# pennucci/PulsePortraiture

Hardware: AMD Instinct MI355X
Metric: subint_fits_per_sec (higher is better)
Workload: dtype f64

## Files before the change

pulseportraiture_amd/csrc/pp_common.h:

```cpp
#pragma once
#include <hip/hip_runtime.h>
#include <stdint.h>
#include <type_traits>

namespace pp {

#define PP_DCONST 4149.377593360996
#define PP_TWO_PI 6.283185307179586476925286766559
#define PP_LN10 2.302585092994045684017991454684

typedef double2 cplx;

__device__ __forceinline__ cplx cmul(cplx a, cplx b) {
    return make_double2(fma(a.x, b.x, -a.y * b.y), fma(a.x, b.y, a.y * b.x));
}
__device__ __forceinline__ cplx cmulc(cplx a, cplx b) {
    return make_double2(fma(a.x, b.x, a.y * b.y), fma(a.y, b.x, -a.x * b.y));
}
__device__ __forceinline__ cplx cadd(cplx a, cplx b) { return make_double2(a.x + b.x, a.y + b.y); }
__device__ __forceinline__ cplx csub(cplx a, cplx b) { return make_double2(a.x - b.x, a.y - b.y); }
__device__ __forceinline__ cplx cmul_mi(cplx a) { return make_double2(a.y, -a.x); }
__device__ __forceinline__ double cnorm(cplx a) { return fma(a.x, a.x, a.y * a.y); }

template <typename T>
__device__ __forceinline__ const T* as_global(const T* p) {
    typedef const T __attribute__((address_space(1)))* gp_t;
    return (const T*)(gp_t)(uintptr_t)p;
}

template <typename T>
__device__ __forceinline__ T load_uniform(const T* p) {
    typedef const T __attribute__((address_space(4)))* cp_t;
    return *(cp_t)(uintptr_t)p;
}

__device__ __forceinline__ double rn_pin(double r) { asm volatile("" : "+v"(r)); return r; }
__device__ __forceinline__ double mul_rn(double a, double b) { return rn_pin(a * b); }
__device__ __forceinline__ double add_rn(double a, double b) { return rn_pin(a + b); }
__device__ __forceinline__ double sub_rn(double a, double b) { return rn_pin(a - b); }

__device__ __forceinline__ double recip_ge1(double x) {
    double y = __builtin_amdgcn_rcp(x);
    y = fma(fma(-x, y, 1.0), y, y);
    y = fma(fma(-x, y, 1.0), y, y);
    return (x < 1e300) ? y : 0.0;
}

template <bool SC>
__device__ __forceinline__ double kconst(double v) {
    if (SC) asm volatile("" : "+s"(v));
    return v;
}
template <bool SC = false, bool ISGN = false>
__device__ __forceinline__ void sincos_turns(double t, double* sn, double* cs) {
    const double q = rint(4.0 * t);
    const double y = fma(-0.25, q, t);
    const double u = y * y;
    double ps = kconst<SC>(0x1.aaec32af93359p-4);
    ps = fma(ps, u, kconst<SC>(-0x1.6fadb9f155744p-1));
    ps = fma(ps, u, kconst<SC>(0x1.e8f434d018d63p+1));
    ps = fma(ps, u, kconst<SC>(-0x1.e3074fde8871fp+3));
    ps = fma(ps, u, kconst<SC>(0x1.50783487ee782p+5));
    ps = fma(ps, u, kconst<SC>(-0x1.32d2cce62bd86p+6));
    ps = fma(ps, u, kconst<SC>(0x1.466bc6775aae2p+6));
    ps = fma(ps, u, kconst<SC>(-0x1.4abbce625be53p+5));
    ps = fma(ps, u, kconst<SC>(0x1.921fb54442d18p+2));
    const double s0 = ps * y;
    double pc = kconst<SC>(0x1.20c62c2f2d7f5p-2);
    pc = fma(pc, u, kconst<SC>(-0x1.b6e24f44b128fp+0));
    pc = fma(pc, u, kconst<SC>(0x1.f9d38a3763cc3p+2));
    pc = fma(pc, u, kconst<SC>(-0x1.a6d1f2a204a8cp+4));
    pc = fma(pc, u, kconst<SC>(0x1.e1f506891babbp+5));
    pc = fma(pc, u, kconst<SC>(-0x1.55d3c7e3cbffap+6));
    pc = fma(pc, u, kconst<SC>(0x1.03c1f081b5ac4p+6));
    pc = fma(pc, u, kconst<SC>(-0x1.3bd3cc9be45dep+4));
    const double c0 = fma(pc, u, 1.0);
    const int qi = (int)q;
    const bool odd = qi & 1;
    const double so = odd ? c0 : s0, co = odd ? s0 : c0;
    if (ISGN) {
        const unsigned uq = (unsigned)qi;
        *sn = __hiloint2double((int)((unsigned)__double2hiint(so) + ((uq >> 1) << 31)), __double2loint(so));
        *cs = __hiloint2double((int)((unsigned)__double2hiint(co) + (((uq + 1u) >> 1) << 31)), __double2loint(co));
        return;
    }
    *sn = (qi & 2) ? -so : so;
    *cs = ((qi + 1) & 2) ? -co : co;
}

template <bool SC = false, bool ISGN = false>
__device__ __forceinline__ cplx unit_phasor(double k, double phi) {
    double pfrac = phi - rint(phi);
    double prod = k * pfrac;
    double err = fma(k, pfrac, -prod);
    double r = (prod - rint(prod)) + err;
    double s, c;
    sincos_turns<SC, ISGN>(r, &s, &c);
    return make_double2(c, s);
}

template <int W>
__device__ __forceinline__ double group_sum(double v) {
#pragma unroll
    for (int o = W / 2; o > 0; o >>= 1) v += __shfl_xor(v, o, 64);
    return v;
}
template <int W>
__device__ __forceinline__ double group_max(double v) {
#pragma unroll
    for (int o = W / 2; o > 0; o >>= 1) v = fmax(v, __shfl_xor(v, o, 64));
    return v;
}

__device__ __forceinline__ int wave_reduce16_index(int lane) { return (lane >> 2) & 15; }
template <int NS>
__device__ __forceinline__ double wave_reduce16(const double (&s)[NS], int lane) {
    double t8[8], t4[4], t2[2];
    const bool b5 = lane & 32, b4 = lane & 16, b3 = lane & 8, b2 = lane & 4;
#pragma unroll
    for (int j = 0; j < 8; ++j) {
        const double hi = (j + 8 < NS) ? s[j + 8] : 0.0;
        const double keep = b5 ? hi : s[j], send = b5 ? s[j] : hi;
        t8[j] = keep + __shfl_xor(send, 32, 64);
    }
#pragma unroll
    for (int j = 0; j < 4; ++j) {
        const double keep = b4 ? t8[j + 4] : t8[j], send = b4 ? t8[j] : t8[j + 4];
        t4[j] = keep + __shfl_xor(send, 16, 64);
    }
#pragma unroll
    for (int j = 0; j < 2; ++j) {
        const double keep = b3 ? t4[j + 2] : t4[j], send = b3 ? t4[j] : t4[j + 2];
        t2[j] = keep + __shfl_xor(send, 8, 64);
    }
    const double keep = b2 ? t2[1] : t2[0], send = b2 ? t2[0] : t2[1];
    double v = keep + __shfl_xor(send, 4, 64);
    v += __shfl_xor(v, 2, 64);
    v += __shfl_xor(v, 1, 64);
    return v;
}

template <int X>
__device__ __forceinline__ double quad_xor(double v) {
    static_assert(X == 1 || X == 2, "inside a quad");
    constexpr int ctrl = X == 1 ? 0xB1 : 0x4E;
    int lo = __double2loint(v), hi = __double2hiint(v);
    lo = __builtin_amdgcn_mov_dpp(lo, ctrl, 0xF, 0xF, false);
    hi = __builtin_amdgcn_mov_dpp(hi, ctrl, 0xF, 0xF, false);
    return __hiloint2double(hi, lo);
}
template <int NS, bool LEAN = false>
__device__ __forceinline__ double wave_reduce_lds(const double (&s)[NS], int lane, double* buf) {
    static_assert(NS <= 16, "one value per lane quad");
    const unsigned l = (unsigned)lane & 63u;
    const int wpos = LEAN ? (int)(l + (l >> 4)) : (lane >> 4) * 17 + (lane & 15);
#pragma unroll
    for (int q = 0; q < NS; ++q) buf[q * 68 + wpos] = s[q];
    const int q = min(lane >> 2, NS - 1), part = lane & 3;
    const double* src = LEAN ? buf + 17u * (4u * min(l >> 2, (unsigned)(NS - 1)) + (l & 3u)) : buf + q * 68 + part * 17;
    double v = 0.0;
#pragma unroll
    for (int t = 0; t < 16; ++t) v += src[t];
    if (LEAN) {
        v += quad_xor<1>(v);
        v += quad_xor<2>(v);
    } else {
        v += __shfl_xor(v, 1, 64);
        v += __shfl_xor(v, 2, 64);
    }
    return v;
}
#define PP_WRED_DOUBLES(NS) ((NS) * 68)

template <int NV>
__device__ inline void block_sum(double (&v)[NV], double* scratch) {
    const int lane = threadIdx.x & 63, wid = threadIdx.x >> 6, nw = blockDim.x >> 6;
#pragma unroll
    for (int i = 0; i < NV; ++i) v[i] = group_sum<64>(v[i]);
    __syncthreads();
    if (lane == 0) {
#pragma unroll
        for (int i = 0; i < NV; ++i) scratch[wid * NV + i] = v[i];
    }
    __syncthreads();
#pragma unroll
    for (int i = 0; i < NV; ++i) {
        double s = 0.0;
        for (int w = 0; w < nw; ++w) s += scratch[w * NV + i];
        v[i] = s;
    }
}

template <int NV, int C0>
__device__ __forceinline__ void wave_totals_to(const double (&v)[NV], int lane, double* dst) {
    constexpr int n = (NV - C0) < 16 ? (NV - C0) : 16;
    double part[n];
#pragma unroll
    for (int j = 0; j < n; ++j) part[j] = v[C0 + j];
    const double tot = wave_reduce16<n>(part, lane);
    if ((lane & 3) == 0 && (lane >> 2) < n) dst[C0 + (lane >> 2)] = tot;
    if constexpr (C0 + 16 < NV) wave_totals_to<NV, C0 + 16>(v, lane, dst);
}
#define PP_BSUM_DOUBLES(NW, NVMAX) (2 * (NW) * ((NVMAX) + 1))
template <int NV, int NVMAX>
__device__ __forceinline__ void block_sum_t(double (&v)[NV], double* scratch, int& flip, double* mx = nullptr) {
    static_assert(NV <= NVMAX, "scratch sized for NVMAX values");
    const int lane = threadIdx.x & 63, wid = threadIdx.x >> 6, nw = blockDim.x >> 6;
    double* buf = scratch + flip * nw * (NVMAX + 1);
    flip ^= 1;
    wave_totals_to<NV, 0>(v, lane, buf + wid * (NV + 1));
    if (mx) {
        const double m = group_max<64>(*mx);
        if (lane == 0) buf[wid * (NV + 1) + NV] = m;
    }
    __syncthreads();
#pragma unroll
    for (int i = 0; i < NV; ++i) {
        double s = 0.0;
        for (int w = 0; w < nw; ++w) s += buf[w * (NV + 1) + i];
        v[i] = s;
    }
    if (mx) {
        double m = buf[NV];
        for (int w = 1; w < nw; ++w) m = fmax(m, buf[w * (NV + 1) + NV]);
        *mx = m;
    }
}

struct SubState {
    double x[5];
    double xe[5];
    double f;
    double g[5];
    double H[25];
    double f0, g0[5], H0[25];
    double radius;
    double pred_red;
    int hits_boundary;
    int iter, nfev, status, done, cur;
    int npass;
    double xl[5], fl, gl[5], Hl[25];
    int fresh;
    int recentred;
    int nmodel;
    int model;
    double xprev[5];
    double geo[4];
};

#define PP_NACC 21
constexpr int PP_CHUNK_CHANNELS = 256;
#define PP_NCS 9
#define PP_TJ 10
#define PP_TSTRIDE (PP_TJ + 2)
#define PP_TAY_PAIR_STRIDE 2
__device__ __forceinline__ size_t tay_idx(size_t row, int q) { return row * PP_TSTRIDE + (size_t)q; }

}
```

pulseportraiture_amd/csrc/pp_extra.h:

```cpp
#pragma once
#include "pp_kernels.h"

namespace pp {

__device__ __forceinline__ void philox4x32_10(uint32_t (&c)[4], uint32_t k0, uint32_t k1) {
#pragma unroll
    for (int r = 0; r < 10; ++r) {
        const uint32_t hi0 = __umulhi(0xD2511F53u, c[0]), lo0 = 0xD2511F53u * c[0];
        const uint32_t hi1 = __umulhi(0xCD9E8D57u, c[2]), lo1 = 0xCD9E8D57u * c[2];
        const uint32_t n0 = hi1 ^ c[1] ^ k0, n2 = hi0 ^ c[3] ^ k1;
        c[0] = n0; c[1] = lo1; c[2] = n2; c[3] = lo0;
        k0 += 0x9E3779B9u; k1 += 0xBB67AE85u;
    }
}

__device__ __forceinline__ void normal_pair(uint64_t seed, int64_t sub, int chan, int pair, double& z0, double& z1) {
    uint32_t c[4] = {(uint32_t)pair, (uint32_t)chan, (uint32_t)((uint64_t)sub & 0xffffffffu),
                     (uint32_t)((uint64_t)sub >> 32)};
    philox4x32_10(c, (uint32_t)(seed & 0xffffffffu), (uint32_t)(seed >> 32));
    const uint64_t a = ((uint64_t)c[0] << 32) | c[1], b = ((uint64_t)c[2] << 32) | c[3];
    const double u1 = ((double)(a >> 11) + 0.5) * (1.0 / 9007199254740992.0);
    const double u2 = ((double)(b >> 11) + 0.5) * (1.0 / 9007199254740992.0);
    const double r = sqrt(-2.0 * log(u1));
    double s, co;
// ... 621 lines not shown
    const double* par;
    const double* w;
    const cplx* twB;
    cplx* acc;
    double* totw;
    const int* off;
    const int2* pairs;
    int npol, nchan, nchan_model;
};

__device__ __forceinline__ void align_add_totw(const AlignListArgs& a, int m) {
    double t = a.totw[m];
    for (int q = a.off[m]; q < a.off[m + 1]; ++q) t += a.w[(size_t)a.pairs[q].x * a.nchan + a.pairs[q].y];
    a.totw[m] = t;
}

template <int M, typename Tio>
__global__ __launch_bounds__(FftPlan<M>::T) void k_align_add(AlignListArgs a) {
    constexpr int T = FftPlan<M>::T;
    __shared__ cplx lds[FftPlan<M>::LDS_ELEMS];
    __shared__ cplx zin[M];
    const int tid = threadIdx.x;
    const int ipol = blockIdx.x / a.nchan_model, m = blockIdx.x % a.nchan_model;
    const int q0 = a.off[m], q1 = a.off[m + 1];
    if (q0 == q1) return;
    cplx* arow = a.acc + ((size_t)ipol * a.nchan_model + m) * M;
    for (int k = tid; k < M; k += T) zin[k] = arow[k];
    for (int q = q0; q < q1; ++q) {
        const int i = a.pairs[q].x, n = a.pairs[q].y;
        const double w = a.w[(size_t)i * a.nchan + n];
        const double phin = align_phase(a.par[i * 3], a.par[i * 3 + 1], a.par[i * 3 + 2],
                                        a.freqs[(size_t)i * a.freqs_stride + n], a.P[i]);
        align_add_row<M, Tio>(lds, zin, reinterpret_cast<const Tio*>(a.src) + (((size_t)i * a.npol + ipol) * a.nchan + n) * (2 * M),
                              a.twB, w, phin, tid);
        __syncthreads();
    }
    for (int k = tid; k < M; k += T) arow[k] = zin[k];
    if (ipol == 0 && tid == 0) align_add_totw(a, m);
}

struct ChanChi2Args {
    const void* src;
    const cplx* const* mft; const double* const* mdc; const int* slot;
    const double* freqs; long long freqs_stride;
    const double* P;
    const double* par;
    const double* nuref;
    const double* scales;
    const double* errs;
    const cplx* twB;
    double* out;
    int nsub, nchan;
};

template <int M, typename Tio>
__global__ __launch_bounds__(FftPlan<M>::T) void k_chan_chi2(ChanChi2Args a) {
    constexpr int T = FftPlan<M>::T;
    __shared__ cplx lds[FftPlan<M>::LDS_ELEMS];
    __shared__ double scratch[(T / 64) + 1];
    const int tid = threadIdx.x;
    const long long nrows = (long long)a.nsub * a.nchan;
    for (long long row = blockIdx.x; row < nrows; row += gridDim.x) {
        const int i = (int)(row / a.nchan), n = (int)(row % a.nchan);
        const double nu = a.freqs[(size_t)i * a.freqs_stride + n], P = a.P[i];
        const double* pr = a.par + (size_t)i * 5;
        const double nuDM = a.nuref[i * 3], nuGM = a.nuref[i * 3 + 1], nutau = a.nuref[i * 3 + 2];
        const double a2 = 1.0 / (nu * nu);
        const double iDM = (nuDM == INFINITY) ? 0.0 : 1.0 / (nuDM * nuDM);
        const double iGM = (nuGM == INFINITY) ? 0.0 : 1.0 / (nuGM * nuGM * nuGM * nuGM);
        const double phin = pr[0] + PP_DCONST * pr[1] * (a2 - iDM) / P +
                            PP_DCONST * PP_DCONST * pr[2] * (a2 * a2 - iGM) / P;
        const double taun = (pr[3] != 0.0) ? pr[3] * pow(nu / nutau, pr[4]) : 0.0;
        const int sl = a.slot ? a.slot[i] : 0;
        const cplx* mrow = as_global(a.mft[sl]) + (size_t)n * M;
        const double m0 = as_global(a.mdc[sl])[n];
        const double sc = a.scales[(size_t)i * a.nchan + n], sg = a.errs[(size_t)i * a.nchan + n];
        fft_row<M, Tio>(lds, reinterpret_cast<const Tio*>(a.src) + (size_t)row * (2 * M), a.twB, tid);
        const cplx z0 = lds[0];
        double sum = 0.0;
        for (int k = tid; k <= M; k += T) {
            double wgt = 2.0;
            cplx d, m;
            if (k == 0) { d = make_double2(z0.x + z0.y, 0.0); m = make_double2(m0, 0.0); wgt = 1.0; }
            else {
                d = (k == M) ? make_double2(z0.x - z0.y, 0.0) : rfft_harmonic<M>(lds, a.twB, k);
                d = cmul(d, unit_phasor((double)k, phin));
                m = mrow[k - 1];
                if (taun != 0.0) {
                    const double x = PP_TWO_PI * (double)k * taun, den = 1.0 / (1.0 + x * x);
                    m = cmul(m, make_double2(den, -x * den));
                }
            }
            cplx r = make_double2(d.x - sc * m.x, d.y - sc * m.y);
            if (k == M) { r.y = 0.0; wgt = 1.0; }
            sum = fma(wgt, cnorm(r), sum);
        }
        sum = group_sum<64>(sum);
        if ((tid & 63) == 0) scratch[tid >> 6] = sum;
        __syncthreads();
        if (tid == 0) {
            double tot = 0.0;
            for (int wv = 0; wv < T / 64; ++wv) tot += scratch[wv];
            a.out[row] = tot / (2.0 * M) / (sg * sg) / (double)(2 * M - 2);
        }
        __syncthreads();
    }
}

struct FpsArgs {
    const cplx* spec;
    const double* noise;
    double* out7;
    double lo, hi;
    int Ns, M, nprof;
    int finish;
    const cplx* specm;
    int mstride;
};

__device__ __forceinline__ void fps_sums(const cplx* X, int M, double phi, int tid, int nt, double& s0,
                                         double& s1, double& s2) {
    s0 = s1 = s2 = 0.0;
    if (tid >= M) return;
    cplx e = unit_phasor((double)(tid + 1), phi);
    const cplx w = unit_phasor((double)nt, phi);
    for (int j = tid; j < M; j += nt) {
        const cplx z = cmul(X[j], e);
        const double k = (double)(j + 1);
        s0 += z.x;
        s1 = fma(k, z.y, s1);
        s2 = fma(k * k, z.x, s2);
        e = cmul(e, w);
    }
}

__device__ inline int block_argmin256(double v, int j, double* shv, int* shj) {
#pragma unroll
    for (int o = 32; o > 0; o >>= 1) {
        const double ov = __shfl_xor(v, o, 64);
        const int oj = __shfl_xor(j, o, 64);
        if (ov < v || (ov == v && oj < j)) { v = ov; j = oj; }
    }
    __syncthreads();
    if ((threadIdx.x & 63) == 0) { shv[threadIdx.x >> 6] = v; shj[threadIdx.x >> 6] = j; }
    __syncthreads();
    v = shv[0]; j = shj[0];
    for (int w = 1; w < 4; ++w)
        if (shv[w] < v || (shv[w] == v && shj[w] < j)) { v = shv[w]; j = shj[w]; }
    __syncthreads();
    return j;
}

#define PP_FPS_LDS 2048
template <int NV, int NVW, typename F>
__device__ __forceinline__ void fps_bsum(double (&out)[NV], double* scratch, int tid, F&& part) {
    if constexpr (NVW == 1) {
        part(tid, out);
        block_sum<NV>(out, scratch);
        __syncthreads();
    } else {
        const int lane = tid & 63;
#pragma unroll 1
        for (int vw = 0; vw < NVW; ++vw) {
            double v[NV];
            part(lane + 64 * vw, v);
#pragma unroll
            for (int q = 0; q < NV; ++q) v[q] = group_sum<64>(v[q]);
            if (lane == 0) {
#pragma unroll
                for (int q = 0; q < NV; ++q) scratch[vw * NV + q] = v[q];
            }
        }
        __syncthreads();
#pragma unroll
        for (int q = 0; q < NV; ++q) {
            double t = 0.0;
            for (int w = 0; w < NVW; ++w) t += scratch[w * NV + q];
            out[q] = t;
        }
        __syncthreads();
    }
}

template <typename F>
__device__ __forceinline__ double nelder_mead_1d(const double x0, F&& feval, double& f0, int& fcalls) {
    double sim0 = x0, sim1 = (x0 != 0.0) ? mul_rn(1.05, x0) : 0.00025;
    f0 = feval(sim0);
    double f1 = feval(sim1);
    fcalls = 2;
    int iterations = 1;
    auto order = [&]() {
        if (f1 < f0) { const double t = sim0; sim0 = sim1; sim1 = t; const double u = f0; f0 = f1; f1 = u; }
    };
    order();
    while (fcalls < 200 && iterations < 200) {
        if (fabs(sim1 - sim0) <= 1e-4 && fabs(f0 - f1) <= 1e-4) break;
        const double xbar = sim0;
        const double xr = sub_rn(mul_rn(2.0, xbar), sim1);
        const double fxr = feval(xr); ++fcalls;
        bool shrink = false;
        if (fxr < f0) {
            const double xe = sub_rn(mul_rn(3.0, xbar), mul_rn(2.0, sim1));
            const double fxe = feval(xe); ++fcalls;
            if (fxe < fxr) { sim1 = xe; f1 = fxe; } else { sim1 = xr; f1 = fxr; }
        } else if (fxr < f1) {
            const double xc = sub_rn(mul_rn(1.5, xbar), mul_rn(0.5, sim1));
            const double fxc = feval(xc); ++fcalls;
            if (fxc <= fxr) { sim1 = xc; f1 = fxc; } else shrink = true;
        } else {
            const double xcc = add_rn(mul_rn(0.5, xbar), mul_rn(0.5, sim1));
            const double fxcc = feval(xcc); ++fcalls;
            if (fxcc < f1) { sim1 = xcc; f1 = fxcc; } else shrink = true;
        }
        if (shrink) {
            sim1 = add_rn(sim0, mul_rn(0.5, sub_rn(sim1, sim0)));
            f1 = feval(sim1); ++fcalls;
        }
        ++iterations;
        order();
    }
    return sim0;
}

template <int NVW, typename DF>
__device__ __forceinline__ void fps_body(const FpsArgs& a, const int i, const int tid, const int M, DF&& dspec,
                                         const cplx* m, cplx* X, double* scratch, double* shv, int* shj) {
    constexpr int RT = 256 / NVW;
    const int H = M + 1, kc = (int)(0.75 * H);
    double v[3];
    fps_bsum<3, NVW>(v, scratch, tid, [&](const int vt, double (&u)[3]) __attribute__((always_inline)) {
        u[0] = u[1] = u[2] = 0.0;
        for (int k = 1 + vt; k <= M; k += 256) {
            const cplx dk = dspec(k), mk = m[k];
            X[k - 1] = cmulc(dk, mk);
            const double pd = cnorm(dk);
            u[0] += pd; u[1] += cnorm(mk);
            if (k >= kc) u[2] += pd;
        }
    });
    const double B = 2.0 * M;
    double sig = a.noise ? a.noise[i] : NAN;
    if (!(sig >= 0.0)) sig = sqrt(v[2] / B / (double)(H - kc));
    const double err2 = sig * sig * (0.5 * B);
    const double dd = v[0] / err2, pp_ = v[1] / err2;
    const int Ns = a.Ns;
    double bestv = INFINITY;
    int bestj = 0x7fffffff;
    const double h = (Ns > 1) ? (a.hi - a.lo) / (double)(Ns - 1) : 0.5;
    for (int j = tid; j < Ns; j += RT) {
        const double phi = (Ns > 1) ? add_rn(mul_rn((double)j, h), a.lo) : a.lo;
        double s0, s1, s2;
        fps_sums(X, M, phi, 0, 1, s0, s1, s2);
        const double vv = -s0 / err2;
        if (vv < bestv) { bestv = vv; bestj = j; }
    }
    int best;
    if constexpr (NVW == 1) best = min(block_argmin256(bestv, bestj, shv, shj), Ns - 1);
    else {
#pragma unroll
        for (int o = 32; o > 0; o >>= 1) {
            const double ov = __shfl_xor(bestv, o, 64);
            const int oj = __shfl_xor(bestj, o, 64);
            if (ov < bestv || (ov == bestv && oj < bestj)) { bestv = ov; bestj = oj; }
        }
        best = min(bestj, Ns - 1);
    }
    double phi = (Ns > 1) ? add_rn(mul_rn((double)best, h), a.lo) : a.lo;
    double f = 0.0, f2 = 0.0;
    auto sums_at = [&](double x, double (&s)[3]) __attribute__((always_inline)) {
        fps_bsum<3, NVW>(s, scratch, tid, [&](const int vt, double (&u)[3]) __attribute__((always_inline)) {
            fps_sums(X, M, x, vt, 256, u[0], u[1], u[2]);
        });
    };
    auto feval = [&](double x) -> double {
        double s[3];
        sums_at(x, s);
        return -s[0] / err2;
    };
    if (a.finish == 1) {
        double f0_;
        int fcalls_;
        phi = nelder_mead_1d(phi, feval, f0_, fcalls_);
    } else {
    double lo = phi - h, hi = phi + h;
    for (int it = 0; it < 60; ++it) {
        double s[3];
        sums_at(phi, s);
        f = -s[0] / err2;
        const double f1 = PP_TWO_PI * s[1] / err2;
        f2 = PP_TWO_PI * PP_TWO_PI * s[2] / err2;
        if (f1 > 0.0) hi = phi; else lo = phi;
        double nxt = (f2 > 0.0) ? phi - f1 / f2 : 0.5 * (lo + hi);
        if (!(nxt > lo && nxt < hi)) nxt = 0.5 * (lo + hi);
        const double step = fabs(nxt - phi);
        phi = nxt;
        if (step < 1e-15) break;
    }
    }
    double s[3];
    sums_at(phi, s);
    f = -s[0] / err2;
    f2 = PP_TWO_PI * PP_TWO_PI * s[2] / err2;
    if (tid == 0) {
        const double scale = -f / pp_;
        double* o = a.out7 + (size_t)i * 7;
        o[0] = phi;
        o[1] = 1.0 / sqrt(scale * f2);
        o[2] = scale;
        o[3] = 1.0 / sqrt(pp_);
        o[4] = sqrt(scale * scale * pp_);
        o[5] = (dd - f * f / pp_) / (B - 2.0);
        o[6] = 0.0;
    }
}

__global__ __launch_bounds__(256) void k_fps(FpsArgs a, cplx* xwork) {
    const int i = blockIdx.x, tid = threadIdx.x, M = a.M;
    __shared__ double scratch[4 * 4];
    __shared__ double shv[4];
    __shared__ int shj[4];
    const cplx* d = a.specm ? a.spec + (size_t)i * (M + 1) : a.spec + (size_t)(2 * i) * (M + 1);
    const cplx* m = a.specm ? a.specm + (size_t)i * a.mstride : a.spec + (size_t)(2 * i + 1) * (M + 1);
    __shared__ cplx Xs[PP_FPS_LDS];
    auto dv = [&](const int k) __attribute__((always_inline)) { return d[k]; };
    if (M <= PP_FPS_LDS) fps_body<1>(a, i, tid, M, dv, m, Xs, scratch, shv, shj);
    else fps_body<1>(a, i, tid, M, dv, m, xwork + (size_t)i * M, scratch, shv, shj);
}

__global__ void k_seed_dm_pick(const int* act, int nact, const double* pk, int ntrial, double step,
                               const double* xbase, double* xout) {
    const int j = blockIdx.x * blockDim.x + threadIdx.x;
    if (j >= nact) return;
    const int i = sub_of(act, j);
    const double* p = pk + (size_t)i * ntrial;
    int b = 0;
    for (int t = 1; t < ntrial; ++t) if (p[t] > p[b]) b = t;
    double frac = 0.0;
    if (b > 0 && b < ntrial - 1) {
        const double den = p[b - 1] - 2.0 * p[b] + p[b + 1];
        if (den < 0.0) frac = fmin(0.5, fmax(-0.5, 0.5 * (p[b - 1] - p[b + 1]) / den));
    }
    for (int q = 0; q < 5; ++q) xout[i * 5 + q] = xbase[i * 5 + q];
    xout[i * 5 + 1] = xbase[i * 5 + 1] + ((double)(b - (ntrial - 1) / 2) + frac) * step;
}

__global__ __launch_bounds__(256) void k_list_active(const SubState* st, const double* seedq, double qmin, int nsub,
                                                     int* act, int* count) {
    __shared__ int offs[257];
    const int tid = threadIdx.x;
    const int per = (nsub + 255) / 256, lo = min(nsub, tid * per), hi = min(nsub, lo + per);
    auto want = [&](int i) { return seedq ? !(seedq[i] >= qmin) : (st[i].done == 0); };
    int c = 0;
    for (int i = lo; i < hi; ++i) c += want(i) ? 1 : 0;
    offs[tid + 1] = c;
    if (tid == 0) offs[0] = 0;
    __syncthreads();
    if (tid == 0) for (int t = 1; t <= 256; ++t) offs[t] += offs[t - 1];
    __syncthreads();
    int o = offs[tid];
    for (int i = lo; i < hi; ++i) if (want(i)) act[o++] = i;
    if (tid == 0) *count = offs[256];
}

#define PP_SEED_KPT 16
__global__ __launch_bounds__(256) void k_seed_accum(FitArgs a, cplx* ypart, int Ks, const double* xbase,
                                                    double dm_off) {
    const int jx = blockIdx.x, i = sub_of(a.act, jx), chunk = blockIdx.y, tid = threadIdx.x;
    const int lane = tid & 63, wave = tid >> 6;
    __shared__ cplx ysh[3 * 64 * PP_SEED_KPT / 4];
    const double P = a.P[i];
    const double nuDM = a.nu_fit[i * 3], nuGM = a.nu_fit[i * 3 + 1];
    const double DM = xbase[i * 5 + 1] + dm_off, GM = xbase[i * 5 + 2];
    const double* freqs = a.freqs + (size_t)i * a.freqs_stride;
    const double* wts = a.wts + (size_t)i * a.nchan;
    const int* ktv = a.ktab ? a.ktab[a.slot ? a.slot[i] : 0] : nullptr;
    cplx y[PP_SEED_KPT];
#pragma unroll
    for (int j = 0; j < PP_SEED_KPT; ++j) y[j] = make_double2(0.0, 0.0);
    const int n0 = chunk * a.cpc, n1 = min(n0 + a.cpc, a.nchan_x);
    for (int nn = n0 + wave; nn < n1; nn += 4) {
        const int n = a.coff + nn * a.cstep;
        const double w = wts[n];
        if (w == 0.0) continue;
        double p1, p2;
        phase_geom(freqs[n], P, nuDM, nuGM, p1, p2);
        const double phin = DM * p1 + GM * p2;
        cplx e = unit_phasor((double)(lane + 1), phin);
        const cplx wst = make_double2(__shfl(e.x, 63, 64), __shfl(e.y, 63, 64));
        const cplx* xrow = a.X + ((size_t)jx * a.nchan_x + nn) * a.Xs;
        const int ktn = min(ktv ? ktv[n] : a.Kt, Ks);
        cplx xv[PP_SEED_KPT];
#pragma unroll
        for (int j = 0; j < PP_SEED_KPT; ++j) {
            const int k = lane + 1 + 64 * j;
            xv[j] = (k <= ktn) ? xrow[k - 1] : make_double2(0.0, 0.0);
        }
#pragma unroll
        for (int j = 0; j < PP_SEED_KPT; ++j) {
            if (64 * j < ktn) {
                const cplx z = cmul(xv[j], e);
                y[j].x = fma(w, z.x, y[j].x);
                y[j].y = fma(w, z.y, y[j].y);
                e = cmul(e, wst);
            }
        }
    }
    cplx* yo = ypart + ((size_t)jx * a.nchunk + chunk) * Ks;
#pragma unroll
    for (int q = 0; q < 4; ++q) {
        __syncthreads();
        if (wave > 0) {
#pragma unroll
            for (int j = 0; j < PP_SEED_KPT / 4; ++j)
                ysh[((wave - 1) * (PP_SEED_KPT / 4) + j) * 64 + lane] = y[q * (PP_SEED_KPT / 4) + j];
        }
        __syncthreads();
        if (wave == 0) {
#pragma unroll
            for (int j = 0; j < PP_SEED_KPT / 4; ++j) {
                const int jj = q * (PP_SEED_KPT / 4) + j;
                cplx s = y[jj];
                for (int ww = 0; ww < 3; ++ww) {
                    const cplx v = ysh[(ww * (PP_SEED_KPT / 4) + j) * 64 + lane];
// ... 97 lines not shown
```

pulseportraiture_amd/csrc/pp_fftq.h:

```cpp
#pragma once
#include "pp_fft.h"

namespace pp {

__device__ __forceinline__ void lane_swap32(double& a, double& b) {
    unsigned alo = (unsigned)__double2loint(a), ahi = (unsigned)__double2hiint(a);
    unsigned blo = (unsigned)__double2loint(b), bhi = (unsigned)__double2hiint(b);
    auto r0 = __builtin_amdgcn_permlane32_swap(alo, blo, false, false);
    auto r1 = __builtin_amdgcn_permlane32_swap(ahi, bhi, false, false);
    a = __hiloint2double((int)r1[0], (int)r0[0]);
    b = __hiloint2double((int)r1[1], (int)r0[1]);
}
__device__ __forceinline__ void lane_swap16(double& a, double& b) {
    unsigned alo = (unsigned)__double2loint(a), ahi = (unsigned)__double2hiint(a);
    unsigned blo = (unsigned)__double2loint(b), bhi = (unsigned)__double2hiint(b);
    auto r0 = __builtin_amdgcn_permlane16_swap(alo, blo, false, false);
    auto r1 = __builtin_amdgcn_permlane16_swap(ahi, bhi, false, false);
    a = __hiloint2double((int)r1[0], (int)r0[0]);
    b = __hiloint2double((int)r1[1], (int)r0[1]);
}

__device__ __forceinline__ int fftq_lambda(int t) { return 4 * (t >> 4) + (t & 3) + 16 * ((t >> 2) & 3); }
__device__ __forceinline__ int fftq_lane_of(int lam) { return 16 * ((lam >> 2) & 3) + (lam & 3) + 4 * ((lam >> 4) & 3); }

constexpr int FFTQ_LDS_ELEMS = 4 * 272;

template <int WHEN = 0, bool LEAN = false, typename T1, typename T2, typename Mid>
__device__ __forceinline__ void fftq1024_from(cplx (&v)[16], cplx* lds, T1 get_t1, T2 get_t2, int tid,
                                              double* power, Mid mid) {
    dft16_first(v);
    if (WHEN == 0) mid();
    const cplx t1 = get_t1();
    dft16_second(v);
    {
        cplx wq[16];
        wq[1] = t1;
#pragma unroll
        for (int j = 2; j < 16; ++j) {
            if (j % 2 == 0) {
                const cplx h = wq[j / 2];
                wq[j] = make_double2(fma(h.x, h.x, -h.y * h.y), 2.0 * h.x * h.y);
            } else wq[j] = cmul(wq[j - 1], wq[1]);
        }
#pragma unroll
        for (int j = 1; j < 16; ++j) v[j] = cmul(v[j], wq[j]);
    }
    if (WHEN == 1) mid();
    const cplx t2 = get_t2();
#pragma unroll
    for (int j = 0; j < 8; ++j) {
        lane_swap32(v[j].x, v[j + 8].x);
        lane_swap32(v[j].y, v[j + 8].y);
    }
#pragma unroll
    for (int j = 0; j < 16; ++j) {
        if (j & 4) continue;
        lane_swap16(v[j].x, v[j + 4].x);
        lane_swap16(v[j].y, v[j + 4].y);
    }
    if (WHEN == 2) mid();
    dft16_first(v);
    {
        const cplx w2 = make_double2(fma(t2.x, t2.x, -t2.y * t2.y), 2.0 * t2.x * t2.y);
        const cplx w3 = cmul(w2, t2);
#pragma unroll
        for (int c = 0; c < 4; ++c) {
            v[4 + c] = cmul(v[4 + c], t2);
            v[8 + c] = cmul(v[8 + c], w2);
            v[12 + c] = cmul(v[12 + c], w3);
        }
    }
    {
        cplx* wbase = LEAN ? lds + 17u * ((unsigned)tid & 63u) : lds + (tid >> 4) * 272 + 17 * (tid & 15);
#pragma unroll
        for (int j = 0; j < 16; ++j) wbase[j] = v[j];
        lds_sync<64>();
        const cplx* rbase = LEAN ? wbase - 16u * ((unsigned)tid & 15u) : lds + (tid >> 4) * 272 + (tid & 15);
#pragma unroll
        for (int j = 0; j < 16; ++j) v[j] = rbase[17 * j];
        lds_sync<64>();
    }
    if (WHEN == 3) mid();
    dft_reg<16>(v);
    if (power) {
        double acc = 0.0;
#pragma unroll
        for (int j = 0; j < 16; ++j) {
            if (j == 0 && tid == 0) { const double dM = v[0].x - v[0].y; acc += dM * dM; }
            else acc += cnorm(v[j]);
        }
        *power += acc;
    }
}

template <int WHEN = 0, typename Mid>
__device__ __forceinline__ void fftq1024(cplx (&v)[16], cplx* lds, const cplx t1, const cplx t2, int tid,
                                         double* power, Mid mid) {
    fftq1024_from<WHEN>(v, lds, [&]() { return t1; }, [&]() { return t2; }, tid, power, mid);
}

__device__ __forceinline__ int fftq512_lambda(int t) {
    return 4 * ((t >> 5) & 1) + 2 * ((t >> 4) & 1) + 32 * ((t >> 3) & 1) + 16 * ((t >> 2) & 1) + 8 * ((t >> 1) & 1) + (t & 1);
}
__device__ __forceinline__ int fftq512_lane_of(int lam) {
    return 32 * ((lam >> 2) & 1) + 16 * ((lam >> 1) & 1) + 8 * ((lam >> 5) & 1) + 4 * ((lam >> 4) & 1) + 2 * ((lam >> 3) & 1) + (lam & 1);
}
constexpr int FFTQ512_LDS_ELEMS = 8 * 72;

__device__ __forceinline__ double lane_xor8(double v) {
    int lo = __double2loint(v), hi = __double2hiint(v);
    lo = __builtin_amdgcn_update_dpp(lo, lo, 0x128, 0xF, 0xF, false);
    hi = __builtin_amdgcn_update_dpp(hi, hi, 0x128, 0xF, 0xF, false);
    return __hiloint2double(hi, lo);
}

template <int WHEN = 0, typename Mid>
__device__ __forceinline__ void fftq512(cplx (&v)[8], cplx* lds, const cplx t1, const cplx t2, const cplx t3, int tid,
                                        double* power, Mid mid) {
    dft_reg<8>(v);
    if (WHEN == 0) mid();
    {
        cplx wq[8];
        wq[1] = t1;
#pragma unroll
        for (int j = 2; j < 8; ++j) {
            if (j % 2 == 0) {
                const cplx h = wq[j / 2];
                wq[j] = make_double2(fma(h.x, h.x, -h.y * h.y), 2.0 * h.x * h.y);
            } else wq[j] = cmul(wq[j - 1], wq[1]);
        }
#pragma unroll
        for (int j = 1; j < 8; ++j) v[j] = cmul(v[j], wq[j]);
    }
#pragma unroll
    for (int j = 0; j < 4; ++j) {
        lane_swap32(v[j].x, v[j + 4].x);
        lane_swap32(v[j].y, v[j + 4].y);
    }
#pragma unroll
    for (int j = 0; j < 8; ++j) {
        if (j & 2) continue;
        lane_swap16(v[j].x, v[j + 2].x);
        lane_swap16(v[j].y, v[j + 2].y);
    }
    dft4(v[0], v[2], v[4], v[6]);
    dft4(v[1], v[3], v[5], v[7]);
    {
        const cplx w2 = make_double2(fma(t2.x, t2.x, -t2.y * t2.y), 2.0 * t2.x * t2.y);
        const cplx w3 = cmul(w2, t2);
#pragma unroll
        for (int c = 0; c < 2; ++c) {
            v[2 + c] = cmul(v[2 + c], t2);
            v[4 + c] = cmul(v[4 + c], w2);
            v[6 + c] = cmul(v[6 + c], w3);
        }
    }
    {
        const bool up = (tid & 8) != 0;
        const double sg = up ? -1.0 : 1.0;
        const cplx w = up ? t3 : make_double2(1.0, 0.0);
#pragma unroll
        for (int j = 0; j < 8; ++j) {
            const cplx p = make_double2(lane_xor8(v[j].x), lane_xor8(v[j].y));
            const cplx d = make_double2(fma(sg, v[j].x, p.x), fma(sg, v[j].y, p.y));
            v[j] = cmul(d, w);
        }
    }
    {
        cplx* wbase = lds + (tid >> 3) * 72 + 9 * (tid & 7);
#pragma unroll
        for (int j = 0; j < 8; ++j) wbase[j] = v[j];
        lds_sync<64>();
        const cplx* rbase = lds + (tid >> 3) * 72 + (tid & 7);
#pragma unroll
        for (int j = 0; j < 8; ++j) v[j] = rbase[9 * j];
        lds_sync<64>();
    }
    if (WHEN == 3) mid();
    dft_reg<8>(v);
    if (power) {
        double acc = 0.0;
#pragma unroll
        for (int j = 0; j < 8; ++j) {
            if (j == 0 && tid == 0) { const double dM = v[0].x - v[0].y; acc += dM * dM; }
            else acc += cnorm(v[j]);
        }
        *power += acc;
    }
}

template <int M> struct FftQ;
template <> struct FftQ<1024> {
    static constexpr int R = 16, LDS_ELEMS = FFTQ_LDS_ELEMS;
    static __device__ __forceinline__ int lambda(int t) { return fftq_lambda(t); }
    static __device__ __forceinline__ int lane_of(int lam) { return fftq_lane_of(lam); }
    template <int WHEN, typename Mid>
    static __device__ __forceinline__ void run(cplx (&v)[16], cplx* lds, const cplx* twB, int tid, double* power, Mid mid) {
        const cplx t1 = twB[2 * tid], t2 = twB[32 * (tid & 15)];
// ... 83 lines not shown
```

pulseportraiture_amd/csrc/pp_kernels.h:

```cpp
#pragma once
#include "pp_fft.h"

namespace pp {

struct ModelFftArgs {
    const void* port;
    cplx* mft;
    double* msum;
    double* mmax;
    double* mdc;
    double* msq;
    const cplx* twB;
    int nchan;
};

struct TailArgs;
#define PP_TAIL_LDS_DOUBLES 2176
#define PP_TAIL_CACHE ((PP_TAIL_LDS_DOUBLES - 536) / 4)
__device__ void tail_work(const TailArgs* t, double* lds, int nlds, int tid, int max_tickets);

struct XspecArgs {
    const void* data;
    const cplx* const* mft;
    const cplx* mft0;
    const int* const* ktab;
    const int* kt0;
    const int* slot;
    cplx* X;
    double* sdraw;
    double* noise;
    const cplx* twB;
    int nsub, nchan, Kt;
    int Xs;
    const double* x0;
    const double* P;
    const double* nu_fit;
    const double* freqs; long long freqs_stride;
    double* csum0;
    double* tay;
    const double* ph0;
    const int* act;
    int cstep, coff, nchan_full;
    unsigned* ticket;
    unsigned ticket_base;
    int x_f32;
    const unsigned* mwords;
    const TailArgs* tail;
    int tail_nsub;
};

__device__ __forceinline__ void store_x(const XspecArgs& a, size_t row, int k, const cplx& x) {
    if (a.x_f32) reinterpret_cast<float2*>(a.X)[row * a.Xs + (k - 1)] = make_float2((float)x.x, (float)x.y);
    else a.X[row * a.Xs + (k - 1)] = x;
}

struct FitArgs {
    int nsub, nchan, nbin, M, Kt;
    int Xs;
    int flags[5];
    int log10_tau, option, is_toa, max_iter, scat;
    int method;
    const cplx* X;
    const cplx* const* mft;
    const double* const* msq;
    const double* const* msum;
    const int* const* ktab;
    const int* slot;
    const double* freqs; long long freqs_stride;
    const double* wts;
    const double* sdraw;
    const double* P;
    const double* nu_fit;
    const double* nu_out;
    const double* x0;
    SubState* st;
    double* csum;
    int ncs;
    double* tay;
    double* partial;
    int nchunk, cpc;
    int* nactive;
    double* o_params; double* o_errs; double* o_nu; double* o_cov;
    double* o_chi2; double* o_rchi2; double* o_snr; int* o_nfev; int* o_rc; int* o_npass;
    double* o_scales; double* o_scale_errs; double* o_csnr;
    double* o_f0; double* o_g0; double* o_H0;
    double* o_rec;
    const int* act;
    int nact, nchan_x, cstep, coff;
    double* mdl;
    int use_model;
    double model_tol;
    int model_bet;
    int recentre;
    double* x0w;
    int x_f32;
    const double* xstart;
    int nfev_shadow;
    int solve_cache;
    int tail_fused;
    int x_full;
};

__device__ __forceinline__ int sub_of(const int* act, int j) { return act ? act[j] : j; }

template <typename P>
__device__ __forceinline__ const P* uniform_ptr(const P* p) {
    const unsigned long long u = reinterpret_cast<unsigned long long>(p);
    const unsigned lo = (unsigned)__builtin_amdgcn_readfirstlane((int)(unsigned)u);
    const unsigned hi = (unsigned)__builtin_amdgcn_readfirstlane((int)(unsigned)(u >> 32));
    return as_global(reinterpret_cast<const P*>(((unsigned long long)hi << 32) | (unsigned long long)lo));
}

__device__ __forceinline__ bool channel_lookup(const XspecArgs& a, int ia, int n, int ne, int M, int& n_held,
                                               const cplx*& mrow, int& ktn) {
    if (!a.slot && n == n_held) return false;
    const cplx* m = as_global(a.slot ? a.mft[a.slot[ia]] : a.mft0) + (size_t)ne * M;
    const int k = a.ktab ? as_global(a.slot ? a.ktab[a.slot[ia]] : a.kt0)[ne] : a.Kt;
    mrow = uniform_ptr(m);
    ktn = __builtin_amdgcn_readfirstlane(k);
    n_held = n;
    return true;
}

template <int M, typename Tin>
__global__ __launch_bounds__(FftPlan<M>::T) void k_model_fft(ModelFftArgs a) {
    constexpr int T = FftPlan<M>::T;
    __shared__ cplx lds[FftPlan<M>::LDS_ELEMS];
    __shared__ double red[2 * (T / 64) + 2];
    const int tid = threadIdx.x;
    for (int n = blockIdx.x; n < a.nchan; n += gridDim.x) {
        const Tin* grow = reinterpret_cast<const Tin*>(a.port) + (size_t)n * (2 * M);
        fft_row<M, Tin>(lds, grow, a.twB, tid);
        double s = 0.0, mx = 0.0;
        for (int k = 1 + tid; k <= M; k += T) {
            const cplx d = rfft_harmonic<M>(lds, a.twB, k);
            a.mft[(size_t)n * M + (k - 1)] = d;
            const double p = cnorm(d);
            a.msq[(size_t)n * M + (k - 1)] = p;
            s += p;
            mx = fmax(mx, p);
        }
        s = group_sum<64>(s);
        mx = group_max<64>(mx);
        if (T > 64) {
            if ((tid & 63) == 0) { red[2 * (tid >> 6)] = s; red[2 * (tid >> 6) + 1] = mx; }
            __syncthreads();
            if (tid == 0) {
                s = 0.0; mx = 0.0;
                for (int w = 0; w < T / 64; ++w) { s += red[2 * w]; mx = fmax(mx, red[2 * w + 1]); }
            }
        }
        if (tid == 0) {
            a.msum[n] = s; a.mmax[n] = mx;
            const cplx z0 = lds[0];
            a.mdc[n] = z0.x + z0.y;
        }
        __syncthreads();
    }
}

__global__ void k_model_kcut(const cplx* mft, const double* mmax, int , int M, double eps2,
                             int* kt, int* kmax) {
    const int n = blockIdx.x;
    const double thr = eps2 * mmax[n];
    int last = 0;
    for (int k = 1 + threadIdx.x; k <= M; k += blockDim.x)
        if (cnorm(mft[(size_t)n * M + k - 1]) > thr) last = k;
    for (int o = 32; o > 0; o >>= 1) last = max(last, __shfl_xor(last, o, 64));
    if ((threadIdx.x & 63) == 0) {
        const int v = min(M, max(64, ((last + 63) / 64) * 64));
        kt[n] = v;
        atomicMax(kmax, v);
    }
}

constexpr int PP_ROW_CHUNK = 32;
template <bool DYN>
struct RowWalk {
    unsigned row, row_nx;
    unsigned bits;
    unsigned wnx, cnx;
    unsigned tick;
    unsigned more, more_nx;
    unsigned fresh, have_wnx;
    static __device__ __forceinline__ unsigned word_of(const unsigned* mw, unsigned c, unsigned nrows) {
        const unsigned r0 = c * PP_ROW_CHUNK;
        if (r0 >= nrows) return 0u;
        if (mw) return as_global(mw)[c];
        const unsigned rem = nrows - r0;
        return rem >= 32u ? 0xffffffffu : ((1u << rem) - 1u);
    }
    static __device__ __forceinline__ unsigned chunk_after(unsigned c, unsigned* ticket, unsigned base) {
        if (DYN) {
            unsigned t = 0;
            if (threadIdx.x == 0) t = atomicAdd(ticket, 1u);
            return gridDim.x + (__builtin_amdgcn_readfirstlane(t) - base);
        }
        return c + gridDim.x;
    }
    __device__ __forceinline__ void enter(unsigned c, unsigned w, unsigned nrows) {
        more_nx = (c * PP_ROW_CHUNK < nrows) ? 1u : 0u;
        row_nx = c * PP_ROW_CHUNK + (w ? (unsigned)__builtin_ctz(w) : 0u);
        bits = w & (w - 1u);
    }
    __device__ __forceinline__ void start(long long nrows_, const unsigned* mw = nullptr, unsigned* ticket = nullptr,
                                          unsigned base = 0) {
        static_assert(PP_ROW_CHUNK == 32, "one 32-bit word per chunk");
        const unsigned nrows = (unsigned)nrows_;
        wnx = 0; cnx = 0; have_wnx = 0u;
        unsigned c = blockIdx.x;
        unsigned w = word_of(mw, c, nrows);
        while (w == 0u && c * PP_ROW_CHUNK < nrows) {
            c = chunk_after(c, ticket, base);
            w = word_of(mw, c, nrows);
        }
        enter(c, __builtin_amdgcn_readfirstlane(w), nrows);
        row = row_nx; more = more_nx;
        tick = threadIdx.x;
        fresh = 1u;
    }
    __device__ __forceinline__ void draw(unsigned* ticket) {
        if (DYN && fresh && threadIdx.x == 0) tick = atomicAdd(ticket, 1u);
    }
    __device__ __forceinline__ void peek(long long nrows_, unsigned base, const unsigned* mw) {
        if (mw && !fresh && !have_wnx) {
            cnx = DYN ? gridDim.x + (__builtin_amdgcn_readfirstlane(tick) - base) : (row >> 5) + gridDim.x;
            wnx = word_of(mw, cnx, (unsigned)nrows_);
            have_wnx = 1u;
        }
    }
    __device__ __forceinline__ void next(int i, int n, int& i_nx, int& n_nx, long long nrows_, int nsub,
                                         unsigned base, unsigned* ticket = nullptr, const unsigned* mw = nullptr) {
        const unsigned nrows = (unsigned)nrows_;
        if (bits) {
            const unsigned b = (unsigned)__builtin_ctz(bits);
            bits &= bits - 1u;
            row_nx = (row & ~(unsigned)(PP_ROW_CHUNK - 1)) + b;
            i_nx = i + (int)(row_nx - row); n_nx = n;
            while (i_nx >= nsub) { i_nx -= nsub; ++n_nx; }
            more_nx = 1u;
            return;
        }
        unsigned c, w;
        if (have_wnx) { c = cnx; w = wnx; have_wnx = 0u; }
        else {
            c = DYN ? gridDim.x + (__builtin_amdgcn_readfirstlane(tick) - base) : (row >> 5) + gridDim.x;
            w = word_of(mw, c, nrows);
        }
        while (w == 0u && c * PP_ROW_CHUNK < nrows) {
            c = chunk_after(c, ticket, base);
            w = word_of(mw, c, nrows);
        }
        enter(c, __builtin_amdgcn_readfirstlane(w), nrows);
        if (more_nx) {
            n_nx = __builtin_amdgcn_readfirstlane((int)(row_nx / (unsigned)nsub));
            i_nx = __builtin_amdgcn_readfirstlane((int)(row_nx % (unsigned)nsub));
        }
    }
    __device__ __forceinline__ void next_row(long long nrows_, unsigned base, unsigned* ticket, const unsigned* mw) {
        const unsigned nrows = (unsigned)nrows_;
        if (bits) {
            const unsigned b = (unsigned)__builtin_ctz(bits);
            bits &= bits - 1u;
            row_nx = (row & ~(unsigned)(PP_ROW_CHUNK - 1)) + b;
            more_nx = 1u;
            return;
        }
        unsigned c = DYN ? gridDim.x + (__builtin_amdgcn_readfirstlane(tick) - base) : (row >> 5) + gridDim.x;
        unsigned w = word_of(mw, c, nrows);
        while (w == 0u && c * PP_ROW_CHUNK < nrows) {
            c = chunk_after(c, ticket, base);
            w = word_of(mw, c, nrows);
        }
        enter(c, __builtin_amdgcn_readfirstlane(w), nrows);
    }
    __device__ __forceinline__ void advance() {
        fresh = (((row_nx ^ row) >> 5) != 0u) ? 1u : 0u;
        row = row_nx; more = more_nx;
    }
};

constexpr int PP_SPLIT_U = 4;
template <int M, typename Tin, bool TAIL, int MODE>
__global__ __launch_bounds__(FftPlan<M>::T, (FftPlan<M>::T >= 256 ? 1 : 2)) void k_xspec(XspecArgs a) {
    constexpr bool FUSE = (MODE != 0);
    constexpr bool M2 = (MODE == 2 || MODE == 3), PAIR = (MODE == 3);
    constexpr int T = FftPlan<M>::T, R1 = FftPlan<M>::R1, PER1 = FftPlan<M>::PER1;
    constexpr int PL = FftPlan<M>::PADLOG;
    constexpr int NW = T / 64;
    typedef typename RawOf<Tin>::type Raw;
    constexpr bool RIDE = M2 && NW == 1;
    constexpr int NRED = RIDE ? PP_TSTRIDE + (TAIL ? 2 : 1) : PP_TSTRIDE;
    static_assert(NRED <= 16, "wave_reduce_lds takes 16 values");
    constexpr int WRED = PP_WRED_DOUBLES(NRED) / 2;
    constexpr int LDSN = (M2 && NW * WRED > FftPlan<M>::LDS_ELEMS) ? NW * WRED : FftPlan<M>::LDS_ELEMS;
    __shared__ cplx lds[LDSN];
    __shared__ double red[(M2 ? 16 : 5) * NW + 4];
    int tid = threadIdx.x;
    const long long nrows = (long long)a.nsub * a.nchan;
    const int H = M + 1;
    const int kc = (int)(0.75 * H);
    Raw cur[PER1][R1];
    RowTwiddles<M> tw;
    load_row_twiddles<M>(tw, a.twB, tid);
    cplx wb0 = a.twB[min(tid + 1, M)];
    const cplx wbT = a.twB[min(T, M)];
    RowWalk<(NW == 1)> rw;
    rw.start(nrows, a.mwords, a.ticket, a.ticket_base);
    long long row = rw.row;
    int n = 0, i = 0;
    if (rw.more) {
        n = __builtin_amdgcn_readfirstlane((int)(row / a.nsub));
        i = __builtin_amdgcn_readfirstlane((int)(row % a.nsub));
        const size_t rc = (size_t)sub_of(a.act, i) * a.nchan_full + (a.coff + n * a.cstep);
        stage_load_global<M, T, R1>(cur, reinterpret_cast<const Tin*>(a.data) + rc * (2 * M), tid);
    }
    constexpr int KPT = (M / 2 + T - 1) / T;
    cplx mv2[KPT];
    constexpr bool CRES = PAIR && M != 1024;
    cplx mc2[CRES ? KPT : 1];
    const cplx* mheld = nullptr;
    const cplx* mrow = nullptr;
    int n_held = -1, ktn = 0;
    int i_nx = i, n_nx = n;
    for (; rw.more; rw.advance(), row = rw.row, i = i_nx, n = n_nx) {
        rw.draw(a.ticket);
        rw.peek(nrows, a.ticket_base, a.mwords);
        if (M2) {
            asm volatile("" : "+v"(tid));
            opaque_twiddles<M>(tw);
            asm volatile("" : "+v"(wb0.x), "+v"(wb0.y));
        }
        const int ia = sub_of(a.act, i), ne = a.coff + n * a.cstep;
        const size_t rc = (size_t)ia * a.nchan_full + ne;
        const size_t rx = (size_t)i * a.nchan + n;
        const bool looked = channel_lookup(a, ia, n, ne, M, n_held, mrow, ktn);
        if (M2 && looked && mrow != mheld) {
#pragma unroll
            for (int j = 0; j < KPT; ++j) {
                const int k = tid + 1 + j * T;
                mv2[j] = mrow[min(k, M) - 1];
                if (CRES) mc2[j] = mrow[max(M - k, 1) - 1];
            }
            mheld = mrow;
        }
        double phin = 0.0;
        if (FUSE) phin = a.ph0[rc];
        {
            cplx v[PER1][R1];
#pragma unroll
            for (int ii = 0; ii < PER1; ++ii)
#pragma unroll
                for (int k = 0; k < R1; ++k) v[ii][k] = to_cplx(cur[ii][k]);
            rw.next(i, n, i_nx, n_nx, nrows, a.nsub, a.ticket_base, a.ticket, a.mwords);
            const size_t rn = rw.more_nx
                ? (size_t)sub_of(a.act, i_nx) * a.nchan_full + (a.coff + n_nx * a.cstep) : rc;
            const Tin* const nxrow = reinterpret_cast<const Tin*>(a.data) + rn * (2 * M);
            auto prefetch = [&]() {
                __builtin_amdgcn_sched_barrier(0);
                stage_load_global<M, T, R1>(cur, nxrow, tid);
                __builtin_amdgcn_sched_barrier(0);
            };
            fft_first_stage<M, M2>(lds, v, tw, tid, prefetch);
        }
        double sd = 0.0, tail = 0.0;
        fft_later_stages<M>(lds, tw, tid, &sd);
        __builtin_amdgcn_sched_barrier(0);
        if (TAIL) {
            for (int k = kc + tid; k <= M; k += T) tail += cnorm(rfft_harmonic<M>(lds, a.twB, k));
        }
        __builtin_amdgcn_sched_barrier(0);
        double s0 = 0.0, s1 = 0.0, s2 = 0.0;
        cplx e = make_double2(1.0, 0.0), wst = make_double2(1.0, 0.0);
        auto setup_phasors = [&]() {
            const cplx el = unit_phasor<true>((double)((tid & 63) + 1), phin);
            const cplx w64 = make_double2(__shfl(el.x, 63, 64), __shfl(el.y, 63, 64));
            e = el;
            for (int q = 0; q < (tid >> 6); ++q) e = cmul(e, w64);
            wst = w64;
#pragma unroll
            for (int q = 1; q < NW; q <<= 1) wst = cmul(wst, wst);
        };
        if (MODE == 1) setup_phasors();
        cplx wb = wb0;
        double tm[PP_TSTRIDE];
        if (M2) {
            static_assert(T % (1 << PL) == 0, "padding period must divide the block size");
            static_assert(PP_TJ == 10, "power ladder written for order 10");
            constexpr int JS = T + (T >> PL);
            const cplx* pk = lds + lds_pad<PL>(tid + 1);
            const cplx* pc = lds + lds_pad<PL>(M - 1 - tid);
            setup_phasors();
            constexpr bool UNI = (T == 64) && (M >= 64) && !PAIR;
            const int ktu = UNI ? __builtin_amdgcn_readfirstlane(ktn) : 0;
            const double kap0 = PP_TWO_PI * (double)(tid + 1);
            if (!UNI) {
#pragma unroll
                for (int j = 0; j < PP_TSTRIDE; ++j) tm[j] = 0.0;
            }
            auto taylor_sums = [&](const cplx& x, const cplx& z, double kap, bool first) {
                const double p2 = kap * kap, p4 = p2 * p2, p6 = p4 * p2, p8 = p4 * p4, p10 = p8 * p2;
                const double ui = z.y * kap;
                const double ax = fabs(x.x) + fabs(x.y);
                if (first) {
                    tm[0] = z.x;
                    tm[1] = ui;
                    tm[2] = p2 * z.x;
                    tm[3] = p2 * ui;
                    tm[4] = p4 * z.x;
                    tm[5] = p4 * ui;
                    tm[6] = p6 * z.x;
                    tm[7] = p6 * ui;
                    tm[8] = p8 * z.x;
                    tm[9] = p8 * ui;
                    tm[10] = p10 * z.x;
                    tm[11] = (p10 * kap) * ax;
                    return;
                }
                tm[0] += z.x;
                tm[1] += ui;
                tm[2] = fma(p2, z.x, tm[2]);
// ... 771 lines not shown
    return rho > 0.15;
}

#define PP_FOR_N3(n_, EXPR)           \
    switch (n_) {                     \
        case 1: { constexpr int N_ = 1; EXPR; } break; \
        case 2: { constexpr int N_ = 2; EXPR; } break; \
        default: { constexpr int N_ = 3; EXPR; } break; \
    }
__device__ __forceinline__ double sel3(double v0, double v1, double v2, int k) { return k == 0 ? v0 : (k == 1 ? v1 : v2); }
template <int N>
__device__ __forceinline__ void gather_sub3(const double (&g)[3], const double (&H)[9], const int (&ix)[3], double (&gs)[N],
                                            double (&Hs)[N * N]) {
#pragma unroll
    for (int r = 0; r < N; ++r) {
        const int k = ix[r];
        gs[r] = sel3(g[0], g[1], g[2], k);
        const double r0 = sel3(H[0], H[3], H[6], k), r1 = sel3(H[1], H[4], H[7], k), r2 = sel3(H[2], H[5], H[8], k);
#pragma unroll
        for (int c = 0; c < N; ++c) Hs[r * N + c] = sel3(r0, r1, r2, ix[c]);
    }
}
template <int N>
__device__ __forceinline__ void scatter_sub3(const double (&p)[N], const int (&ix)[3], double (&p3)[3]) {
#pragma unroll
    for (int j = 0; j < 3; ++j) {
        p3[j] = 0.0;
#pragma unroll
        for (int r = 0; r < N; ++r) if (ix[r] == j) p3[j] = p[r];
    }
}
template <int N>
__device__ __forceinline__ void tr_propose_scipy3(double f, const double (&g)[3], const double (&H)[9], const int (&ix)[3],
                                                  double radius, double (&p3)[3], int& hits, double& pred) {
    double gs[N], Hs[N * N], p[N];
    gather_sub3<N>(g, H, ix, gs, Hs);
    tr_cg_steihaug_scipy<N>(f, gs, Hs, radius, p, &hits);
    pred = f - tr_model_value<N>(f, gs, Hs, p);
    scatter_sub3<N>(p, ix, p3);
}
template <int N>
__device__ __forceinline__ bool newton_propose3(const double (&g)[3], const double (&H)[9], const int (&ix)[3], double (&p3)[3],
                                                double& pred) {
    double gs[N], Hs[N * N], p[N], mg[N], Hp[N];
    gather_sub3<N>(g, H, ix, gs, Hs);
#pragma unroll
    for (int r = 0; r < N; ++r) mg[r] = -gs[r];
    if (!chol_solve<N>(Hs, mg, p)) return false;
#pragma unroll
    for (int r = 0; r < N; ++r) Hp[r] = vdot<N>(Hs + r * N, p);
    pred = -(vdot<N>(gs, p) + 0.5 * vdot<N>(p, Hp));
    scatter_sub3<N>(p, ix, p3);
    return true;
}

__global__ __launch_bounds__(256) void k_eval_moments(FitArgs a) {
    constexpr int LPC = 16;
    const int jx = blockIdx.x, i = sub_of(a.act, jx), chunk = blockIdx.y;
    const SubState& st = a.st[i];
    const int tid = threadIdx.x, g = tid / LPC, l = tid % LPC;
    const double phi = st.xe[0], DM = st.xe[1], GM = st.xe[2];
    const double P = a.P[i];
    const double nuDM = a.nu_fit[i * 3], nuGM = a.nu_fit[i * 3 + 1];
    const double* freqs = a.freqs + (size_t)i * a.freqs_stride;
    const double* wts = a.wts + (size_t)i * a.nchan;
    const int* ktv = a.ktab ? as_global(a.ktab[a.slot ? a.slot[i] : 0]) : nullptr;
    double* tay = a.tay;
    const size_t row0 = (size_t)i * a.nchan;
    const int n0 = chunk * a.cpc, n1 = min(n0 + a.cpc, a.nchan_x);
    const int src = ((tid & 63) & ~(LPC - 1)) | (LPC - 1);
    for (int nn = n0 + g; nn < n1; nn += 256 / LPC) {
        const int n = a.coff + nn * a.cstep;
        const double w = wts[n];
        double p1, p2;
        phase_geom(freqs[n], P, nuDM, nuGM, p1, p2);
        const double phin = phi + DM * p1 + GM * p2;
        cplx e0 = unit_phasor((double)(l + 1), phin);
        const cplx w1 = make_double2(__shfl(e0.x, src, 64), __shfl(e0.y, src, 64));
        const cplx w2 = cmul(w1, w1), w3 = cmul(w2, w1), w4 = cmul(w2, w2);
        const cplx* xrow = a.X + ((size_t)jx * a.nchan_x + nn) * a.Xs;
        const int ktn = ktv ? ktv[n] : a.Kt;
        double s[PP_TSTRIDE];
#pragma unroll
        for (int j = 0; j < PP_TSTRIDE; ++j) s[j] = 0.0;
        double k = (double)(l + 1);
        if (w != 0.0) {
#pragma unroll 1
            for (int jj = l; jj < ktn; jj += 4 * LPC) {
                const cplx zero = make_double2(0.0, 0.0);
                cplx xv[4];
                xv[0] = xrow[jj];
                xv[1] = (jj + LPC < ktn) ? xrow[jj + LPC] : zero;
                xv[2] = (jj + 2 * LPC < ktn) ? xrow[jj + 2 * LPC] : zero;
                xv[3] = (jj + 3 * LPC < ktn) ? xrow[jj + 3 * LPC] : zero;
                cplx ev[4];
                ev[0] = e0; ev[1] = cmul(e0, w1); ev[2] = cmul(e0, w2); ev[3] = cmul(e0, w3);
#pragma unroll
                for (int q = 0; q < 4; ++q) {
                    const cplx z = cmul(xv[q], ev[q]);
                    const double kap = PP_TWO_PI * (k + (double)(q * LPC));
                    const double kap2 = kap * kap;
                    double ur = z.x, ui = z.y * kap;
#pragma unroll
                    for (int j = 0; j <= PP_TJ; j += 2) {
                        s[j] += ur;
                        ur *= kap2;
                        if (j + 1 <= PP_TJ) { s[j + 1] += ui; ui *= kap2; }
                    }
                    static_assert(PP_TJ % 2 == 0, "PP_TJ must be even");
                    double pw = kap;
#pragma unroll
                    for (int j = 0; j < PP_TJ / 2; ++j) pw *= kap2;
                    s[PP_TJ + 1] = fma(pw, fabs(xv[q].x) + fabs(xv[q].y), s[PP_TJ + 1]);
                }
                e0 = cmul(e0, w4);
                k += 4.0 * LPC;
            }
        }
#pragma unroll
        for (int j = 0; j < PP_TSTRIDE; ++j) {
            double v = group_sum<LPC>(s[j]);
            if (j <= PP_TJ && ((j & 3) == 1 || (j & 3) == 2)) v = -v;
            if (l == (j % LPC)) tay[tay_idx(row0 + n, j)] = v;
        }
    }
}

__device__ __forceinline__ void taylor_load(const double* tay, size_t row, double (&t)[PP_TSTRIDE]) {
    static_assert(PP_TSTRIDE % 2 == 0, "rows of the Taylor model are read in pairs");
    const double* tg = tay + tay_idx(row, 0);
#pragma unroll
    for (int j = 0; j < PP_TSTRIDE / 2; ++j) {
        const double2 v = *reinterpret_cast<const double2*>(tg + j * PP_TAY_PAIR_STRIDE);
        t[2 * j] = v.x; t[2 * j + 1] = v.y;
    }
}
__device__ __forceinline__ void taylor_shift_reg(const double (&t)[PP_TSTRIDE], double d, double& A0, double& A1,
                                                 double& A2);
__device__ __forceinline__ void taylor_shift_reg(const double (&t)[PP_TSTRIDE], double d, double& A0, double& A1,
                                                 double& A2) {
    double a0 = 0.0, a1 = 0.0, a2 = 0.0;
#pragma unroll
    for (int j = PP_TJ; j >= 0; --j) {
        a0 = fma(a0, d * (1.0 / (double)(j + 1)), t[j]);
        if (j >= 1) a1 = fma(a1, d * (1.0 / (double)j), t[j]);
        if (j >= 2) a2 = fma(a2, d * (1.0 / (double)(j - 1)), t[j]);
    }
    A0 = a0; A1 = a1; A2 = a2;
}

#define PP_SOLVE_CACHE_MAX 4096
constexpr int PP_SOLVE_PF = 2;
constexpr int PP_TAYLOR_WAVES = 2;
template <int NV, int NVMAX, int NT, int NVW, typename F>
__device__ __forceinline__ void vblock_sum(double (&out)[NV], double* scratch, int& flip, double* mx, int tid, F&& accumulate) {
    static_assert(NV <= NVMAX, "scratch sized for NVMAX values");
    constexpr int NWV = NT / 64, RT = NT / NVW;
    const int lane = tid & 63, rw = tid >> 6;
    double* buf = scratch + flip * NWV * (NVMAX + 1);
    flip ^= 1;
    auto one_wave = [&](const int vw) __attribute__((always_inline)) {
#pragma unroll
        for (int j = 0; j < NV; ++j) out[j] = 0.0;
        double m = 0.0;
        accumulate(lane + 64 * vw, out, m);
        wave_totals_to<NV, 0>(out, lane, buf + vw * (NV + 1));
        if (mx) {
            m = group_max<64>(m);
            if (lane == 0) buf[vw * (NV + 1) + NV] = m;
        }
    };
    if constexpr (NVW == 1) one_wave(rw);
    else {
#pragma unroll 1
        for (int k = 0; k < NVW; ++k) one_wave(rw + (RT / 64) * k);
    }
    __syncthreads();
#pragma unroll
    for (int i = 0; i < NV; ++i) out[i] = 0.0;
#pragma unroll 1
    for (int w = 0; w < NWV; ++w) {
#pragma unroll
        for (int i = 0; i < NV; ++i) out[i] += buf[w * (NV + 1) + i];
    }
    if (mx) {
        double m = buf[NV];
#pragma unroll 1
        for (int w = 1; w < NWV; ++w) m = fmax(m, buf[w * (NV + 1) + NV]);
        *mx = m;
    }
}

template <int NT, int PF, int NVW>
__device__ __forceinline__ void taylor_solve_body(const FitArgs& a, const int i, const int tid, double* scratch, double* inv_lds) {
    constexpr int RT = NT / NVW;
    static_assert(NT % 64 == 0 && RT % 64 == 0 && NT % RT == 0, "whole waves");
    SubState& st = a.st[i];
    if (st.done) return;
    int flip = 0;
    const double P = a.P[i];
    const double nuDM = a.nu_fit[i * 3], nuGM = a.nu_fit[i * 3 + 1];
    const double* freqs = a.freqs + (size_t)i * a.freqs_stride;
    const double* wts = a.wts + (size_t)i * a.nchan;
    const double* msum = as_global(a.msum[a.slot ? a.slot[i] : 0]);
    const double* tay = a.tay;
    const size_t row0 = (size_t)i * a.nchan;
    const int* fl = a.flags;
    int ix[3] = {0, 0, 0}, nf = 0;
#pragma unroll
    for (int j = 0; j < 3; ++j)
        if (fl[j]) {
            if (nf == 0) ix[0] = j; else if (nf == 1) ix[1] = j; else ix[2] = j;
            ++nf;
        }
    const int ncache = a.solve_cache;
    double *inv_w = inv_lds, *inv_p1 = inv_lds + ncache, *inv_p2 = inv_lds + 2 * ncache, *inv_S = inv_lds + 3 * ncache;
    {
        const int nc = min(a.nchan, ncache);
#pragma unroll 4
        for (int n = tid; n < nc; n += RT) {
            double p1, p2;
            phase_geom(freqs[n], P, nuDM, nuGM, p1, p2);
            inv_w[n] = wts[n]; inv_p1[n] = p1; inv_p2[n] = p2; inv_S[n] = msum[n];
        }
        __syncthreads();
    }
    auto chan_inv = [&](int n, double& w, double& p1, double& p2, double& S0) {
        if (n < ncache) { w = inv_w[n]; p1 = inv_p1[n]; p2 = inv_p2[n]; S0 = inv_S[n]; }
        else { w = wts[n]; phase_geom(freqs[n], P, nuDM, nuGM, p1, p2); S0 = msum[n]; }
    };
    auto for_channels = [&](const int vt, auto&& body) {
        if constexpr (PF == 0) {
            for (int n = vt; n < a.nchan; n += NT) {
                double t[PP_TSTRIDE];
                taylor_load(tay, row0 + n, t);
                body(n, t);
            }
        } else {
            double buf[PF ? PF : 1][PP_TSTRIDE];
#pragma unroll
            for (int d = 0; d < PF; ++d)
                if (vt + d * NT < a.nchan) taylor_load(tay, row0 + vt + d * NT, buf[d]);
            for (int n0 = vt; n0 < a.nchan; n0 += PF * NT) {
#pragma unroll
                for (int d = 0; d < PF; ++d) {
                    const int n = n0 + d * NT;
                    if (n < a.nchan) {
                        double t[PP_TSTRIDE];
#pragma unroll
                        for (int j = 0; j < PP_TSTRIDE; ++j) t[j] = buf[d][j];
                        if (n + PF * NT < a.nchan) taylor_load(tay, row0 + n + PF * NT, buf[d]);
                        body(n, t);
                    }
                }
            }
        }
    };
    auto for_channels_at_origin = [&](const int vt, auto&& body) {
        constexpr int U = 4;
        for (int n0 = vt; n0 < a.nchan; n0 += U * NT) {
            double2 h[U][2];
#pragma unroll
            for (int d = 0; d < U; ++d)
                if (n0 + d * NT < a.nchan) {
                    const double* tg = tay + tay_idx(row0 + n0 + d * NT, 0);
                    h[d][0] = *reinterpret_cast<const double2*>(tg);
                    h[d][1] = *reinterpret_cast<const double2*>(tg + PP_TAY_PAIR_STRIDE);
                }
#pragma unroll
            for (int d = 0; d < U; ++d)
                if (n0 + d * NT < a.nchan) body(n0 + d * NT, h[d][0].x, h[d][0].y, h[d][1].x);
        }
    };
    auto evalm = [&](const double* dx, double& f, double* g, double* H, bool at_origin = false) -> double {
        double acc[10];
        double dmax = 0.0;
        vblock_sum<10, 10, NT, NVW>(acc, scratch, flip, &dmax, tid, [&](const int vt, double (&ac)[10], double& dm) __attribute__((always_inline)) {
            auto add = [&](double w, double p1, double p2, double S0, double A0, double A1, double A2) {
                const bool in = (w != 0.0);
                const double r = A0 / S0;
                const double F = in ? -w * A0 * r : 0.0, Gp = in ? -2.0 * w * r * A1 : 0.0;
                const double Lpp = in ? -2.0 * w * (A1 * A1 / S0 + r * A2) : 0.0;
                ac[0] += F;
                ac[1] += Gp; ac[2] += Gp * p1; ac[3] += Gp * p2;
                ac[4] += Lpp; ac[5] += Lpp * p1; ac[6] += Lpp * p2;
                ac[7] += Lpp * p1 * p1; ac[8] += Lpp * p1 * p2; ac[9] += Lpp * p2 * p2;
            };
            if (at_origin)
                for_channels_at_origin(vt, [&](int n, double A0, double A1, double A2) {
                    double w, p1, p2, S0;
                    chan_inv(n, w, p1, p2, S0);
                    add(w, p1, p2, S0, A0, A1, A2);
                });
            else
                for_channels(vt, [&](int n, const double (&t)[PP_TSTRIDE]) {
                    double w, p1, p2, S0;
                    chan_inv(n, w, p1, p2, S0);
                    const double d = dx[0] + dx[1] * p1 + dx[2] * p2;
                    dm = fmax(dm, (w != 0.0) ? fabs(d) : 0.0);
                    double A0, A1, A2;
                    taylor_shift_reg(t, d, A0, A1, A2);
                    add(w, p1, p2, S0, A0, A1, A2);
                });
        });
        f = acc[0];
        g[0] = fl[0] ? acc[1] : 0.0; g[1] = fl[1] ? acc[2] : 0.0; g[2] = fl[2] ? acc[3] : 0.0;
        const double hh[3][3] = {{acc[4], acc[5], acc[6]}, {acc[5], acc[7], acc[8]}, {acc[6], acc[8], acc[9]}};
#pragma unroll
        for (int r_ = 0; r_ < 3; ++r_)
#pragma unroll
            for (int c_ = 0; c_ < 3; ++c_) H[r_ * 3 + c_] = (fl[r_] && fl[c_]) ? hh[r_][c_] : 0.0;
        return dmax;
    };
    double dx[3] = {0.0, 0.0, 0.0};
    const bool off_centre = (a.xstart != nullptr) && st.recentred == 0;
    if (off_centre)
#pragma unroll
        for (int j = 0; j < 3; ++j) dx[j] = fl[j] ? a.xstart[i * 5 + j] - st.xe[j] : 0.0;
    const double dx0[3] = {dx[0], dx[1], dx[2]};
    double f, g[3], H[9];
    bool ok = true;
    int it = 0, nfev = 1;
    double dpath = evalm(dx, f, g, H, !off_centre);
    if (tid == 0 && st.recentred == 0) {
        st.f0 = f;
#pragma unroll
        for (int j = 0; j < 5; ++j) st.g0[j] = j < 3 ? g[j] : 0.0;
#pragma unroll
        for (int r_ = 0; r_ < 5; ++r_)
#pragma unroll
            for (int c_ = 0; c_ < 5; ++c_) st.H0[r_ * 5 + c_] = (r_ < 3 && c_ < 3) ? H[r_ * 3 + c_] : 0.0;
    }
    if (!isfinite(f)) ok = false;
    if (ok && a.method == 0) {
        double radius = 1.0;
        double xa[3], xla[3], xld[3] = {dx0[0], dx0[1], dx0[2]};
#pragma unroll
        for (int j = 0; j < 3; ++j) { xa[j] = off_centre ? (fl[j] ? a.xstart[i * 5 + j] : st.xe[j]) : st.xe[j]; xla[j] = xa[j]; }
        double f2 = f, g2[3] = {g[0], g[1], g[2]}, H2[9];
#pragma unroll
        for (int j = 0; j < 9; ++j) H2[j] = H[j];
        for (;;) {
            double p3[3], pred = 0.0;
            int hits = 0;
            PP_FOR_N3(nf, (tr_propose_scipy3<N_>(f, g, H, ix, radius, p3, hits, pred)));
            double xta[3], xt[3];
#pragma unroll
            for (int j = 0; j < 3; ++j) { xta[j] = fl[j] ? xa[j] + p3[j] : xa[j]; xt[j] = fl[j] ? dx[j] + p3[j] : dx[j]; }
            if (a.nfev_shadow >= 2)
#pragma unroll
                for (int j = 0; j < 3; ++j) xt[j] = xta[j] - st.xe[j];
            const bool shadow = a.nfev_shadow > 0 || (a.nfev_shadow < 0 && nf == 1);
            const bool cached = shadow ? (xta[0] == xla[0] && xta[1] == xla[1] && xta[2] == xla[2])
                                              : (xt[0] == xld[0] && xt[1] == xld[1] && xt[2] == xld[2]);
            if (!(pred > 0.0)) {
                if (!cached) ++nfev;
                break;
            }
            if (!cached) {
                dpath = fmax(dpath, evalm(xt, f2, g2, H2));
#pragma unroll
                for (int j = 0; j < 3; ++j) { xla[j] = xta[j]; xld[j] = xt[j]; }
                ++nfev;
            }
            bool finite = isfinite(f2);
#pragma unroll
            for (int j = 0; j < 3; ++j) finite = finite && isfinite(g2[j]);
#if defined(PP_TAYLOR_TRACE) && PP_TAYLOR_TRACE >= 3
            if (tid == 0)
                printf("tay it %2d f %.17g f_new %.17g actual %.3e pred %.3e rho %.3f radius %.3e hits %d cached %d\n", it, f, f2,
                       f - f2, pred, (f - f2) / pred, radius, hits, (int)cached);
#endif
            if (tr_scipy_accept(f, f2, pred, hits, finite, &radius)) {
#pragma unroll
                for (int j = 0; j < 3; ++j) { dx[j] = xt[j]; xa[j] = xta[j]; }
                f = f2;
#pragma unroll
                for (int j = 0; j < 3; ++j) g[j] = g2[j];
#pragma unroll
                for (int j = 0; j < 9; ++j) H[j] = H2[j];
            }
            ++it;
            if (it >= a.max_iter || !(radius > 1e-300)) {
#ifdef PP_TAYLOR_TRACE
                if (tid == 0) printf("taylor %d: iteration limit it %d radius %.3e\n", i, it, radius);
#endif
                ok = false; break;
            }
        }
    } else if (ok) {
        double fprev = INFINITY;
        for (it = 0; it < 24; ++it) {
            if (it > 0) { dpath = fmax(dpath, evalm(dx, f, g, H)); ++nfev; }
            if (!isfinite(f)) { ok = false; break; }
            double p3[3], pred = 0.0;
            bool solved = false;
            PP_FOR_N3(nf, (solved = newton_propose3<N_>(g, H, ix, p3, pred)));
            if (!solved) { ok = false; break; }
            if (f > fprev + 1e-9 * fabs(fprev)) { ok = false; break; }
            fprev = f;
#pragma unroll
            for (int j = 0; j < 3; ++j) if (fl[j]) dx[j] += p3[j];
            if (!(pred > 64.0 * 2.220446049250313e-16 * fabs(f))) break;
        }
        if (it >= 24) ok = false;
    }
    const int buf = 1 - st.cur;
    if (ok) {
        double* csum = a.csum + ((size_t)buf * a.nsub + i) * a.nchan * a.ncs;
        double ev[4];
        double jf = 1.0;
        for (int j = 2; j <= PP_TJ; ++j) jf *= (double)j;
        vblock_sum<4, 10, NT, NVW>(ev, scratch, flip, nullptr, tid, [&](const int vt, double (&e4)[4], double&) __attribute__((always_inline)) {
            for_channels(vt, [&](int n, const double (&t)[PP_TSTRIDE]) {
                double w, p1, p2, S0;
                chan_inv(n, w, p1, p2, S0);
                const double d = dx[0] + dx[1] * p1 + dx[2] * p2;
                double A0, A1, A2;
                taylor_shift_reg(t, d, A0, A1, A2);
                csum[(size_t)n * 3] = A0; csum[(size_t)n * 3 + 1] = A1; csum[(size_t)n * 3 + 2] = A2;
                if (w == 0.0) return;
                e4[3] += -w * A0 * A0 / S0;
                const double d2 = d * d, d4 = d2 * d2, d10 = d4 * d4 * d2;
                static_assert(PP_TJ == 10, "remainder power written for order 10");
                const double e1 = t[PP_TJ + 1] * d10 / jf;
                const double r = fabs(t[0] / S0) + 1e-300;
                const double ge = 2.0 * w * r * e1 * 1.5;
                e4[0] += ge; e4[1] += ge * fabs(p1); e4[2] += ge * fabs(p2);
            });
        });
        const double tol[3] = {1e-13, 1e-11, 1e-8};
#pragma unroll
        for (int j = 0; j < 3; ++j)
            if (fl[j]) {
                const double hjj = fabs(H[j * 3 + j]);
#if defined(PP_TAYLOR_TRACE) && PP_TAYLOR_TRACE >= 2
                if (tid == 0 && j == 0) printf("tmargin %d %.4e %.4e\n", i, ev[j] / (tol[j] * hjj), dpath);
#endif
                if (!(ev[j] <= tol[j] * hjj)) {
#ifdef PP_TAYLOR_TRACE
                    if (tid == 0) printf("taylor %d: certificate %d: err %.3e > tol %.3e (dpath %.3e, it %d) x0 %.9f %.9f dx %.3e %.3e f %.10e\n", i, j, ev[j], tol[j] * hjj, dpath, it, st.xe[0], st.xe[1], dx[0], dx[1], f);
#endif
                    ok = false;
                }
            }
        if (!(dpath < 0.02)) {
#ifdef PP_TAYLOR_TRACE
            if (tid == 0) printf("taylor %d: path %.3e left the model's range (it %d)\n", i, dpath, it);
#endif
            ok = false;
        }
        if (ok && tid == 0) {
#pragma unroll
            for (int j = 0; j < 3; ++j) st.x[j] = st.xe[j] + dx[j];
            st.x[3] = st.xe[3]; st.x[4] = st.xe[4];
            st.f = ev[3];
#pragma unroll
            for (int j = 0; j < 5; ++j) st.g[j] = j < 3 ? g[j] : 0.0;
#pragma unroll
            for (int r_ = 0; r_ < 5; ++r_)
#pragma unroll
                for (int c_ = 0; c_ < 5; ++c_) st.H[r_ * 5 + c_] = (r_ < 3 && c_ < 3) ? H[r_ * 3 + c_] : 0.0;
            st.cur = buf; st.nfev += nfev; st.npass = 1 + st.recentred; st.iter = it; st.status = PP_RC_STALL; st.done = 1; st.fresh = 0;
            atomicSub(a.nactive, 1);
        }
    }
    if (!ok && tid == 0) {
        bool fin = isfinite(dpath) && dpath < 0.02;
#pragma unroll
        for (int j = 0; j < 3; ++j) fin = fin && isfinite(dx[j]);
        if (off_centre) {
#pragma unroll
            for (int j = 0; j < 5; ++j) { st.xe[j] = a.xstart[i * 5 + j]; st.x[j] = st.xe[j]; a.x0w[i * 5 + j] = st.xe[j]; }
            st.recentred = 1;
        } else if (st.recentred < a.recentre && fin) {
            st.nfev += nfev;
#pragma unroll
            for (int j = 0; j < 3; ++j) st.xe[j] += dx[j];
#pragma unroll
            for (int j = 0; j < 5; ++j) { st.x[j] = st.xe[j]; a.x0w[i * 5 + j] = st.xe[j]; }
            st.recentred += 1;
        } else { st.recentred = a.recentre + 1; st.nfev = 0; }
        st.fresh = 1;
    }
}

template <int NT, int PF = PP_SOLVE_PF>
__global__ __launch_bounds__(NT, PP_TAYLOR_WAVES) void k_taylor_solve(FitArgs a) {
    __shared__ double scratch[PP_BSUM_DOUBLES(NT / 64, 10)];
    extern __shared__ double inv_lds[];
    taylor_solve_body<NT, PF, 1>(a, blockIdx.x, threadIdx.x, scratch, inv_lds);
}
template <int NT, int PF = PP_SOLVE_PF>
__global__ __launch_bounds__(64, PP_TAYLOR_WAVES) void k_taylor_solve_v(FitArgs a) {
    __shared__ double scratch[PP_BSUM_DOUBLES(NT / 64, 10)];
    extern __shared__ double inv_lds[];
    taylor_solve_body<NT, PF, NT / 64>(a, blockIdx.x, threadIdx.x, scratch, inv_lds);
}

__device__ inline void unpack_acc(const double* acc, const int* flags, double& f, double* g, double* H) {
    f = acc[0];
    for (int j = 0; j < 5; ++j) g[j] = flags[j] ? acc[1 + j] : 0.0;
    int c = 6;
    for (int i = 0; i < 5; ++i)
        for (int j = i; j < 5; ++j) {
            const double v = (flags[i] && flags[j]) ? acc[c] : 0.0;
            H[i * 5 + j] = v;
            H[j * 5 + i] = v;
            ++c;
        }
}

template <int n>
__device__ inline bool step_propose(const FitArgs& a, SubState& s, const int* idx) {
    bool done = false;
        double gs[n], Hs[n * n], p[n];
        for (int r = 0; r < n; ++r) {
            gs[r] = s.g[idx[r]];
            for (int c = 0; c < n; ++c) Hs[r * n + c] = s.H[idx[r] * 5 + idx[c]];
        }
        int hits = 0;
        if (a.method == 0) {
            tr_cg_steihaug_scipy<n>(s.f, gs, Hs, s.radius, p, &hits);
            const double pred = s.f - tr_model_value<n>(s.f, gs, Hs, p);
            if (!(pred > 0.0)) {
                bool cached = true;
                for (int j = 0; j < 5; ++j) {
                    double xp = s.x[j];
                    for (int r = 0; r < n; ++r) if (idx[r] == j) xp = s.x[j] + p[r];
                    cached = cached && (xp == s.xl[j]);
                }
                if (!cached) s.nfev += 1;
                s.status = PP_RC_STALL; done = true;
            } else {
                for (int j = 0; j < 5; ++j) s.xe[j] = s.x[j];
                for (int r = 0; r < n; ++r) s.xe[idx[r]] = s.x[idx[r]] + p[r];
                s.pred_red = pred;
                s.hits_boundary = hits;
            }
        } else {
        tr_subproblem<n>(gs, Hs, s.radius, p, &hits);
        double Hp[n];
        for (int r = 0; r < n; ++r) Hp[r] = vdot<n>(Hs + r * n, p);
        const double pred = -(vdot<n>(gs, p) + 0.5 * vdot<n>(p, Hp));
        const double fpred = s.f - pred;
        const double noise = 2.220446049250313e-16 * fabs(s.f);
        if (!(pred > 0.0) || !(fpred < s.f) || pred <= 64.0 * noise) {
            double pn[n], Hpn[n];
            int hn = 0;
            tr_subproblem<n>(gs, Hs, 1e150, pn, &hn);
            for (int r = 0; r < n; ++r) Hpn[r] = vdot<n>(Hs + r * n, pn);
            const double predn = -(vdot<n>(gs, pn) + 0.5 * vdot<n>(pn, Hpn));
            if (!hn && predn >= 0.0 && predn <= 4096.0 * noise && s.iter + 1 < a.max_iter) {
                for (int j = 0; j < 5; ++j) s.xe[j] = s.x[j];
                for (int r = 0; r < n; ++r) s.xe[idx[r]] = s.x[idx[r]] + pn[r];
                s.fresh = 2;
            } else {
                s.status = PP_RC_STALL; done = true;
            }
        } else {
            for (int j = 0; j < 5; ++j) s.xe[j] = s.x[j];
            for (int r = 0; r < n; ++r) s.xe[idx[r]] = s.x[idx[r]] + p[r];
            s.pred_red = pred;
            s.hits_boundary = hits;
        }
        }
// ... 17 lines not shown
            s.f = f;
            s.cur = 1 - s.cur;
        }
        s.status = PP_RC_STALL; done = true;
    } else if (first) {
        s.f = f;
        for (int j = 0; j < 5; ++j) s.g[j] = g[j];
        for (int j = 0; j < 25; ++j) s.H[j] = H[j];
        if (s.recentred == 0) {
            s.f0 = f;
            for (int j = 0; j < 5; ++j) s.g0[j] = g[j];
            for (int j = 0; j < 25; ++j) s.H0[j] = H[j];
        }
        s.cur = 1 - s.cur;
        if (!finite) { s.status = PP_RC_NAN; done = true; }
        if (a.max_iter <= 0) { s.status = PP_RC_MAXITER; done = true; }
    } else {
        const double actual = s.f - f;
        const double rho = finite ? actual / s.pred_red : -1.0;
#ifdef PP_STEP_TRACE
        if (&s == &a.st[PP_STEP_TRACE])
            printf("dev it %2d f %.17g f_new %.17g actual %.3e pred %.3e rho %.3f radius %.3e hits %d\n", s.iter, s.f, f,
                   actual, s.pred_red, rho, s.radius, s.hits_boundary);
#endif
        if (rho < 0.25) s.radius *= 0.25;
        else if (rho > 0.75 && s.hits_boundary) s.radius = fmin(2.0 * s.radius, 1000.0);
        if (rho > 0.15) {
            for (int j = 0; j < 5; ++j) { s.xprev[j] = s.x[j]; s.x[j] = s.xe[j]; s.g[j] = g[j]; }
            for (int j = 0; j < 25; ++j) s.H[j] = H[j];
            s.f = f;
            s.cur = 1 - s.cur;
        }
        s.iter += 1;
        if (s.iter >= a.max_iter) { s.status = PP_RC_MAXITER; done = true; }
        if (!(s.radius > 1e-300)) { s.status = PP_RC_NAN; done = true; }
    }
    if (!done) {
        int idx[5], n = 0;
        for (int j = 0; j < 5; ++j) if (a.flags[j]) idx[n++] = j;
        PP_FOR_N(n, done = step_propose<N_>(a, s, idx));
    }
    return done;
}

__device__ inline bool step_logic(const FitArgs& a, SubState& s, double f, const double* g, const double* H, bool is_pass) {
    for (int j = 0; j < 5; ++j) { s.xl[j] = s.xe[j]; s.gl[j] = g[j]; }
    for (int j = 0; j < 25; ++j) s.Hl[j] = H[j];
    s.fl = f;
    bool done = step_decide(a, s, f, g, H, true, is_pass);
    while (!done && s.fresh == 0) {
        bool same = true;
        for (int j = 0; j < 5; ++j) same = same && (s.xe[j] == s.xl[j]);
        if (!same) break;
        done = step_decide(a, s, s.fl, s.gl, s.Hl, false, false);
    }
    return done;
}

#include "pp_evalscat.h"
#include "pp_scatmodel.h"

__global__ __launch_bounds__(64) void k_step(FitArgs a) {
    const int i = sub_of(a.act, blockIdx.x), tid = threadIdx.x;
    SubState& s = a.st[i];
    if (s.done || s.model == 1) return;
    if (s.model >= 4) {
        if (tid == 0) s.model = (s.model == 4) ? 0 : 3;
        return;
    }
    __shared__ double acc[PP_NACC];
    if (tid < PP_NACC) {
        double v = 0.0;
        for (int c = 0; c < a.nchunk; ++c) v += a.partial[((size_t)i * a.nchunk + c) * PP_NACC + tid];
        acc[tid] = v;
    }
    __syncthreads();
    if (s.fresh == 1 && a.scat && a.use_model) scat_model_geometry(a, i, s);
    if (tid != 0) return;
    double f, g[5], H[25];
    unpack_acc(acc, a.flags, f, g, H);
    const bool done = step_logic(a, s, f, g, H, true);
    if (done) {
        s.done = 1;
        atomicSub(a.nactive, 1);
    } else if (a.scat && a.use_model && s.model == 0) {
        scat_model_request(a, s);
    }
}

__device__ inline double pick_poly_root(const double* cin, int deg, double target, bool take_sqrt) {
    double c[7];
    int n = deg, off = 0;
    while (n > 0 && cin[off] == 0.0) { ++off; --n; }
    while (n > 0 && cin[off + n] == 0.0) --n;
    for (int j = 0; j <= n; ++j) c[j] = cin[off + j] / cin[off];
    if (n <= 0) return NAN;
    double rad = 0.0;
    for (int j = 1; j <= n; ++j) rad = fmax(rad, pow(fabs(c[j]), 1.0 / (double)j));
    rad *= 2.0;
    double zr[6], zi[6];
    for (int j = 0; j < n; ++j) {
        double s, co;
        sincos(PP_TWO_PI * j / n + 0.4, &s, &co);
        zr[j] = 0.5 * rad * co; zi[j] = 0.5 * rad * s;
    }
    for (int it = 0; it < 200; ++it) {
        double maxstep = 0.0;
        for (int j = 0; j < n; ++j) {
            double pr = 1.0, pi = 0.0, dr = 0.0, di = 0.0;
            for (int m = 1; m <= n; ++m) {
                const double ndr = dr * zr[j] - di * zi[j] + pr, ndi = dr * zi[j] + di * zr[j] + pi;
                dr = ndr; di = ndi;
                const double npr = pr * zr[j] - pi * zi[j] + c[m], npi = pr * zi[j] + pi * zr[j];
                pr = npr; pi = npi;
            }
            const double dn = dr * dr + di * di;
            if (dn == 0.0) continue;
            double wr = (pr * dr + pi * di) / dn, wi = (pi * dr - pr * di) / dn;
            double sr = 0.0, si = 0.0;
            for (int m = 0; m < n; ++m)
                if (m != j) {
                    const double er = zr[j] - zr[m], ei = zi[j] - zi[m], en = er * er + ei * ei;
                    if (en > 0.0) { sr += er / en; si -= ei / en; }
                }
            const double qr = 1.0 - (wr * sr - wi * si), qi = -(wr * si + wi * sr), qn = qr * qr + qi * qi;
            const double stx = (wr * qr + wi * qi) / qn, sty = (wi * qr - wr * qi) / qn;
            zr[j] -= stx; zi[j] -= sty;
            maxstep = fmax(maxstep, (fabs(stx) + fabs(sty)) / (fabs(zr[j]) + fabs(zi[j]) + 1e-10 * rad));
        }
        if (maxstep < 8e-16) break;
    }
    double best = NAN, bestd = INFINITY;
    for (int j = 0; j < n; ++j) {
        if (fabs(zi[j]) > 1e-9 * fabs(zr[j]) || !(zr[j] > 0.0)) continue;
        double x = zr[j];
        for (int it = 0; it < 4; ++it) {
            double pv = 1.0, dv = 0.0;
            for (int m = 1; m <= n; ++m) { dv = dv * x + pv; pv = pv * x + c[m]; }
            if (dv != 0.0) x -= pv / dv;
        }
        if (!(x > 0.0)) continue;
        const double v = take_sqrt ? sqrt(x) : x;
        if (fabs(target - v) < bestd) { bestd = fabs(target - v); best = v; }
    }
    return best;
}

__device__ __forceinline__ double py_wrap_half(double x) {
    if (fabs(x) >= 0.5) { x = fmod(x, 1.0); if (x < 0.0) x += 1.0; }
    if (x >= 0.5) x -= 1.0;
    return x;
}

template <int CPT, int NT, int NVW>
__device__ __forceinline__ void finalize_body(const FitArgs& a, const int i, const int tid, double* scratch, double* sh) {
    static_assert(NVW == 1 || CPT == 0, "channels held in registers belong to real threads");
    constexpr int RT = NT / NVW;
    const SubState& s = a.st[i];
    int flip = 0;
    const double P = a.P[i];
    const double* freqs = a.freqs + (size_t)i * a.freqs_stride;
    const double* wts = a.wts + (size_t)i * a.nchan;
    const double* csum = a.csum + ((size_t)s.cur * a.nsub + i) * a.nchan * a.ncs;
    const int slot = a.slot ? a.slot[i] : 0;
    const double* msum = as_global(a.msum[slot]);
    const int* fl = a.flags;
    const double phi = s.x[0], DM = s.x[1], GM = s.x[2], alpha = s.x[4];
    const double taup = s.x[3];
    const double tau = a.log10_tau ? pow(10.0, taup) : taup;
    const bool scat_on = a.scat && (tau != 0.0);
    const double nfDM = a.nu_fit[i * 3], nfGM = a.nu_fit[i * 3 + 1], nftau = a.nu_fit[i * 3 + 2];
    double noDM = a.nu_out ? a.nu_out[i * 3] : NAN, noGM = a.nu_out ? a.nu_out[i * 3 + 1] : NAN,
           notau = a.nu_out ? a.nu_out[i * 3 + 2] : NAN;
    double rw[CPT ? CPT : 1], rf[CPT ? CPT : 1], rc0[CPT ? CPT : 1], rc1[CPT ? CPT : 1], rc2[CPT ? CPT : 1],
           rS[CPT ? CPT : 1], rd[CPT ? CPT : 1];
    if constexpr (CPT > 0) {
#pragma unroll
        for (int q = 0; q < CPT; ++q) {
            const int n = tid + NT * q;
            const bool in = n < a.nchan;
            rw[q] = in ? wts[n] : 0.0;
            rf[q] = in ? freqs[n] : 0.0;
            rc0[q] = in ? csum[(size_t)n * 3] : 0.0; rc1[q] = in ? csum[(size_t)n * 3 + 1] : 0.0;
            rc2[q] = in ? csum[(size_t)n * 3 + 2] : 0.0;
            rS[q] = in ? msum[n] : 0.0;
            rd[q] = in ? a.sdraw[(size_t)i * a.nchan + n] : 0.0;
        }
    }
    auto for_channels = [&](const int vt, auto&& body) {
        if constexpr (CPT > 0) {
#pragma unroll
            for (int q = 0; q < CPT; ++q) {
                const int n = vt + NT * q;
                if (n < a.nchan) body(n, q);
            }
        } else {
            for (int n = vt; n < a.nchan; n += NT) body(n, 0);
        }
    };
    auto wt_of = [&](int n, int q) { if constexpr (CPT > 0) return rw[q]; else return wts[n]; };
    auto nu_of = [&](int n, int q) { if constexpr (CPT > 0) return rf[q]; else return freqs[n]; };
    auto load_cs = [&](int n, int q, double* cs) {
        if constexpr (CPT > 0) {
            cs[0] = rc0[q]; cs[1] = rc1[q]; cs[2] = rc2[q];
            cs[3] = cs[4] = cs[5] = 0.0; cs[6] = rS[q]; cs[7] = cs[8] = 0.0;
        } else if (a.ncs == 3) {
            cs[0] = csum[(size_t)n * 3]; cs[1] = csum[(size_t)n * 3 + 1]; cs[2] = csum[(size_t)n * 3 + 2];
            cs[3] = cs[4] = cs[5] = 0.0; cs[6] = msum[n]; cs[7] = cs[8] = 0.0;
        } else {
            for (int j = 0; j < PP_NCS; ++j) cs[j] = csum[(size_t)n * PP_NCS + j];
        }
    };
    double v3[3];
    vblock_sum<3, 31, NT, NVW>(v3, scratch, flip, nullptr, tid, [&](const int vt, double (&u3)[3], double&) __attribute__((always_inline)) {
        for_channels(vt, [&](int n, int q) {
            const double w = wt_of(n, q);
            double sd;
            if constexpr (CPT > 0) sd = rd[q]; else sd = (w != 0.0) ? a.sdraw[(size_t)i * a.nchan + n] : 0.0;
            if (w != 0.0) { u3[0] += w * sd; u3[1] += nu_of(n, q); u3[2] += 1.0; }
        });
    });
    const double Sd = v3[0], nused = v3[2], fmean = v3[1] / v3[2];
    int pat = 0;
    for (int j = 0; j < 5; ++j) pat = pat * 2 + (fl[j] ? 1 : 0);
    if (pat == 0x1F) pat = 0x1B;
    int efl[5];
    for (int j = 0; j < 5; ++j) efl[j] = fl[j];
    if ((fl[0] && fl[1] && fl[2] && fl[3] && fl[4])) efl[2] = 0;
    const bool need_zero = isnan(noDM) || isnan(noGM) || isnan(notau);
    double nzDM = nfDM, nzGM = nfGM, nztau = nftau;
    if (need_zero) {
        double v[20];
        vblock_sum<20, 31, NT, NVW>(v, scratch, flip, nullptr, tid, [&](const int vt, double (&v)[20], double&) __attribute__((always_inline)) {
        for_channels(vt, [&](int n, int q) {
            const double w = wt_of(n, q);
            if (w == 0.0) return;
            double cs[PP_NCS];
            load_cs(n, q, cs);
            const Local L = local_terms(cs, w);
            ChanGeom cg;
            const double nu = nu_of(n, q);
            chan_geom(nu, P, nfDM, nfGM, nftau, tau, alpha, a.log10_tau, scat_on, cg);
            const double a2 = 1.0 / (nu * nu), a4 = a2 * a2, lf = scat_on ? log(nu) : 0.0;
            const double h = L.Lpp;
            const double q2p = cg.taun;
            const double q12p = a.log10_tau ? PP_LN10 * cg.taun : (scat_on ? cg.taun / tau : 0.0);
            const double Htt = L.Ltt * cg.q1 * cg.q1 + L.Gt * cg.q11;
            const double Hta = L.Ltt * cg.q1 * cg.q2 + L.Gt * cg.q12;
            const double Haa = L.Ltt * cg.q2 * cg.q2 + L.Gt * cg.q22;
            const double Hta_l = L.Ltt * cg.q1 * q2p + L.Gt * q12p;
            switch (pat) {
            case 0x18:
                v[0] += a2 * h; v[1] += h; break;
            case 0x14:
                v[0] += a4 * h; v[1] += h; break;
            case 0x03:
                v[0] += lf * Hta_l; v[1] += Hta_l; break;
            case 0x1A: {
                const double H23 = L.Lpt * cg.q1;
                v[0] += H23;
                v[1] += Htt;
                v[2] += a2 * H23; v[3] += a2 * h; v[4] += h;
                break; }
            case 0x1C: {
                const double pj = (a.option == 1) ? cg.p1 : cg.p2;
                v[0] += h * a4; v[1] += h;
                v[2] += h * pj * a2; v[3] += h * pj;
                v[4] += h * pj * a4;
                v[5] += h * a2;
                break; }
            case 0x1B: {
                const double H23 = L.Lpt * cg.q1, H24 = L.Lpt * cg.q2;
                const double H41 = L.Lpt * q2p, H42 = L.Lpt * cg.p1 * q2p, H43 = Hta_l;
                v[0] += h; v[1] += h * cg.p1 * cg.p1; v[2] += Htt; v[3] += Haa;
                v[4] += h * cg.p1; v[5] += H23; v[6] += H24;
                v[7] += H23 * cg.p1; v[8] += H24 * cg.p1; v[9] += Hta;
                v[10] += a2 * h; v[11] += a2 * H23; v[12] += a2 * H24;
                v[13] += lf * H41; v[14] += lf * H42; v[15] += lf * H43;
                v[16] += H41; v[17] += H42; v[18] += H43;
                break; }
            case 0x1E: {
                const double k1 = PP_DCONST / P, k2 = PP_DCONST * PP_DCONST / P;
                const double Hpt = L.Lpt * cg.q1;
                v[0] += Hpt; v[1] += Htt;
                if (a.option == 0) {
                    const double H21 = h * k1, H23 = h * cg.p2 * k1, H24 = Hpt * k1;
                    const double H31 = h * k2, H33 = h * cg.p2 * k2, H34 = Hpt * k2;
                    v[2] += a4 * H34; v[3] += H34; v[4] += a2 * H21; v[5] += H21;
                    v[6] += a4 * H31; v[7] += H31; v[8] += a2 * H23; v[9] += H23;
                    v[10] += a4 * H33; v[11] += H33; v[12] += a2 * H24; v[13] += H24;
                } else {
                    const double H21 = h * k1, H22 = h * cg.p1 * k1, H24 = Hpt * k1;
                    const double H31 = h * k2, H32 = h * cg.p1 * k2, H34 = Hpt * k2;
                    v[2] += a2 * H24; v[3] += H24; v[4] += a4 * H31; v[5] += H31;
                    v[6] += a2 * H21; v[7] += H21; v[8] += a4 * H32; v[9] += H32;
                    v[10] += a2 * H22; v[11] += H22; v[12] += a4 * H34; v[13] += H34;
                }
                break; }
            default: break;
            }
        });
        });
        switch (pat) {
        case 0x18: nzDM = 1.0 / sqrt(v[0] / v[1]); break;
        case 0x14: nzGM = pow(v[0] / v[1], -0.25); break;
        case 0x03: nztau = exp(v[0] / v[1]); break;
        case 0x1A: {
            const double numer = v[0] * v[2] - v[1] * v[3], denom = v[0] * v[0] - v[1] * v[4];
            nzDM = 1.0 / sqrt(numer / denom);
            break; }
        case 0x1C:
            if (a.option == 0 || a.option == 1) {
                const double A = v[0], B = v[1], C = v[2], D = v[3], E = v[4], F = v[3], G = v[5], Hh = v[1];
                double co[4] = {A * C - E * G, E * Hh - A * D, F * G - B * C, B * D - F * Hh};
                if (tid == 0) sh[0] = pick_poly_root(co, 3, fmean, true);
                __syncthreads();
                nzDM = nzGM = sh[0];
                __syncthreads();
            }
            break;
        case 0x1B: {
            const double H11 = v[0], H22 = v[1], H33 = v[2], H44 = v[3], H12 = v[4], H13 = v[5], H14 = v[6];
            const double H23 = v[7], H34 = v[9];
            const double c1 = H34 * H34 - H33 * H44, c2 = H13 * H44 - H14 * H34, c3 = H14 * H33 - H13 * H34;
            nzDM = 1.0 / sqrt((c1 * v[10] + c2 * v[11] + c3 * v[12]) / (c1 * v[0] + c2 * v[5] + c3 * v[6]));
            const double e1 = H13 * H22 - H12 * H23, e2 = H11 * H23 - H12 * H13, e3 = H12 * H12 - H11 * H22;
            nztau = exp((e1 * v[13] + e2 * v[14] + e3 * v[15]) / (e1 * v[16] + e2 * v[17] + e3 * v[18]));
            break; }
        case 0x1E:
            if (a.option == 0 || a.option == 1) {
                const double H14 = v[0], H44 = v[1];
                const double A = v[2], aa = v[3], B = v[4], b = v[5], C = v[6], c = v[7], D = v[8], d = v[9];
                const double E = v[10], e = v[11], F = v[12], f = v[13];
                double co[6];
                int deg;
                if (a.option == 0) {
                    co[0] = A * A * B + H44 * C * D + H14 * E * F - H44 * B * E - A * C * F - H14 * A * D;
                    co[1] = -A * A * b - H44 * C * d - H14 * E * f + H44 * b * E + A * C * f + H14 * A * d;
                    co[2] = -2 * A * aa * B - H44 * c * D - H14 * e * F + H44 * B * e + (A * c + aa * C) * F + H14 * aa * D;
                    co[3] = 2 * A * aa * b + H44 * c * d + H14 * e * f - H44 * b * e - (A * c + aa * C) * f - H14 * aa * d;
                    co[4] = aa * aa * B - aa * c * F;
                    co[5] = -aa * aa * b + aa * c * f;
                    deg = 5;
                } else {
                    co[0] = A * A * B + H44 * C * D + H14 * E * F - H44 * B * E - A * C * F - H14 * A * D;
                    co[1] = -2 * A * aa * B - H44 * c * D - H14 * e * F + H44 * B * e + (A * c + aa * C) * F + H14 * aa * D;
                    co[2] = -(A * A * b - aa * aa * B) - H44 * C * d - H14 * E * f + H44 * b * E + (A * C * f - aa * c * F) + H14 * A * d;
                    co[3] = 2 * A * aa * b + H44 * c * d + H14 * e * f - H44 * b * e - (A * c + aa * C) * f - H14 * aa * d;
                    co[4] = -aa * aa * b + aa * c * f;
                    deg = 4;
                }
                if (tid == 0) sh[0] = pick_poly_root(co, deg, fmean, true);
                __syncthreads();
                nzDM = nzGM = sh[0];
                __syncthreads();
            }
            break;
        default: break;
        }
    }
    if (isnan(noDM)) noDM = nzDM;
    if (isnan(noGM)) noGM = nzGM;
    if (isnan(notau)) notau = nztau;
    if (a.is_toa) {
        if (fl[1]) noGM = noDM;
        else if (fl[2]) noDM = noGM;
    }
    const double k1 = PP_DCONST / P, k2 = PP_DCONST * PP_DCONST / P;
    const double inv2 = (nfDM == INFINITY) ? 0.0 : 1.0 / (nfDM * nfDM);
    const double inv4 = (nfGM == INFINITY) ? 0.0 : 1.0 / (nfGM * nfGM * nfGM * nfGM);
    const double phi_inf = phi + PP_DCONST * DM * (0.0 - inv2) / P + PP_DCONST * PP_DCONST * GM * (0.0 - inv4) / P;
    const double phi_out = py_wrap_half(phi_inf + k1 * DM / (noDM * noDM) + k2 * GM / (noGM * noGM * noGM * noGM));
    const double tau_out = tau * pow(notau / nftau, alpha);
    double m[31];
    vblock_sum<31, 31, NT, NVW>(m, scratch, flip, nullptr, tid, [&](const int vt, double (&m)[31], double&) __attribute__((always_inline)) {
    for_channels(vt, [&](int n, int q) {
        const double w = wt_of(n, q);
        if (w == 0.0) return;
        double cs[PP_NCS];
        load_cs(n, q, cs);
        ChanGeom cg;
        chan_geom(nu_of(n, q), P, noDM, noGM, notau, tau_out, alpha, a.log10_tau, scat_on, cg);
        const double A0 = cs[0], A1 = cs[1], A2 = cs[2], T1 = cs[3], T2 = cs[4], A1T = cs[5];
        const double S0 = cs[6], S1 = cs[7], S2 = cs[8];
        const double r = A0 / S0;
        const double Lpp = -2.0 * w * r * A2, Lpt = -2.0 * w * r * A1T;
        const double Ltt = -2.0 * w * (r * T2 - 0.5 * r * r * S2);
        const double Gt = -2.0 * w * (r * T1 - 0.5 * r * r * S1);
        const double J[5] = {1.0, cg.p1, cg.p2, cg.q1, cg.q2};
        const double up = -2.0 * w * A1, ut = -2.0 * w * (T1 - r * S1);
        const double U[5] = {up, up * cg.p1, up * cg.p2, ut * cg.q1, ut * cg.q2};
        const double cinv = 1.0 / (2.0 * w * S0);
        int c = 0;
        for (int ii = 0; ii < 5; ++ii)
            for (int jj = ii; jj < 5; ++jj) {
                double hij;
                if (jj < 3) hij = Lpp * J[ii] * J[jj];
                else if (ii < 3) hij = Lpt * J[ii] * J[jj];
                else hij = Ltt * J[ii] * J[jj] + Gt * (ii == 3 ? (jj == 3 ? cg.q11 : cg.q12) : cg.q22);
                m[c] += hij;
                m[15 + c] += U[ii] * U[jj] * cinv;
                ++c;
            }
        m[30] += w * A0 * r;
    });
    });
    int ix[5] = {0, 0, 0, 0, 0}, nfit = 0;
#pragma unroll
    for (int j = 0; j < 5; ++j)
        if (fl[j]) {
            if (nfit == 0) ix[0] = j; else if (nfit == 1) ix[1] = j; else if (nfit == 2) ix[2] = j;
            else if (nfit == 3) ix[3] = j; else ix[4] = j;
            ++nfit;
        }
    double full[25];
    {
        int c = 0;
#pragma unroll
        for (int ii = 0; ii < 5; ++ii)
#pragma unroll
            for (int jj = ii; jj < 5; ++jj) {
                const double vv = (fl[ii] && fl[jj]) ? (m[c] - m[15 + c]) : 0.0;
                full[ii * 5 + jj] = vv; full[jj * 5 + ii] = vv;
                ++c;
            }
    }
    auto sel5 = [](double v0, double v1, double v2, double v3, double v4, int k) {
        return k == 0 ? v0 : k == 1 ? v1 : k == 2 ? v2 : k == 3 ? v3 : v4;
    };
    auto on_subspace = [&](auto NC) {
        constexpr int N = decltype(NC)::value;
        double Xs[N * N];
#pragma unroll
        for (int r = 0; r < N; ++r) {
            const int k = ix[r];
            double row[5];
#pragma unroll
            for (int jj = 0; jj < 5; ++jj) row[jj] = sel5(full[jj], full[5 + jj], full[10 + jj], full[15 + jj], full[20 + jj], k);
#pragma unroll
            for (int c2 = 0; c2 < N; ++c2) Xs[r * N + c2] = sel5(row[0], row[1], row[2], row[3], row[4], ix[c2]);
        }
        const bool inv_ok = mat_inverse<N>(Xs);
#pragma unroll 1
        for (int kv = 0; kv < NVW; ++kv)
        for_channels(tid + RT * kv, [&](int n, int q) {
            const double w = wt_of(n, q);
            double sc = 0.0, se = 0.0, sn = 0.0;
            if (w != 0.0) {
                double cs[PP_NCS];
                load_cs(n, q, cs);
                ChanGeom cg;
                chan_geom(nu_of(n, q), P, noDM, noGM, notau, tau_out, alpha, a.log10_tau, scat_on, cg);
                const double r = cs[0] / cs[6];
                const double up = -2.0 * w * cs[1], ut = -2.0 * w * (cs[3] - r * cs[7]);
                const double U[5] = {up, up * cg.p1, up * cg.p2, ut * cg.q1, ut * cg.q2};
                double Us[N];
#pragma unroll
                for (int r1 = 0; r1 < N; ++r1) Us[r1] = sel5(U[0], U[1], U[2], U[3], U[4], ix[r1]);
                const double cinv = 1.0 / (2.0 * w * cs[6]);
                double uXu = 0.0;
#pragma unroll
                for (int r1 = 0; r1 < N; ++r1)
#pragma unroll
                    for (int c1 = 0; c1 < N; ++c1) uXu += Us[r1] * Xs[r1 * N + c1] * Us[c1];
                sc = r;
                se = sqrt(2.0 * (cinv + cinv * cinv * uXu));
                sn = r * sqrt(w * cs[6]);
            }
            if (a.o_scales) a.o_scales[(size_t)i * a.nchan + n] = sc;
            if (a.o_scale_errs) a.o_scale_errs[(size_t)i * a.nchan + n] = se;
            if (a.o_csnr) a.o_csnr[(size_t)i * a.nchan + n] = sn;
        });
        if (tid == 0) {
            double* oe = a.o_errs + (size_t)i * 5;
            double* oc = a.o_cov + (size_t)i * 25;
            for (int j = 0; j < 5; ++j) oe[j] = 0.0;
            for (int j = 0; j < 25; ++j) oc[j] = 0.0;
#pragma unroll
            for (int r = 0; r < N; ++r) {
                if (r >= nfit) break;
#pragma unroll
                for (int c = 0; c < N; ++c) if (c < nfit) oc[ix[r] * 5 + ix[c]] = inv_ok ? 2.0 * Xs[r * N + c] : NAN;
                oe[ix[r]] = inv_ok ? sqrt(2.0 * Xs[r * N + r]) : NAN;
            }
        }
    };
    if constexpr (CPT > 0) { PP_FOR_N3(nfit, on_subspace(std::integral_constant<int, N_>{})); }
    else { PP_FOR_N(nfit, on_subspace(std::integral_constant<int, N_>{})); }
    if (tid == 0) {
        double* op = a.o_params + (size_t)i * 5;
        op[0] = phi_out; op[1] = DM; op[2] = GM;
        op[3] = a.log10_tau ? log10(tau_out) : tau_out;
        op[4] = alpha;
        const double* oe = a.o_errs + (size_t)i * 5;
        a.o_nu[(size_t)i * 3] = noDM; a.o_nu[(size_t)i * 3 + 1] = noGM; a.o_nu[(size_t)i * 3 + 2] = notau;
        const double chi2 = Sd + s.f;
        const double dof = nused * a.nbin - (nfit + nused);
        a.o_chi2[i] = chi2;
        a.o_rchi2[i] = chi2 / dof;
        a.o_snr[i] = sqrt(m[30]);
        a.o_nfev[i] = s.nfev;
        a.o_rc[i] = s.status;
        a.o_npass[i] = s.npass;
        if (i == 0 && !a.tail_fused) a.o_npass[a.nsub] = *a.nactive;
        if (a.o_rec) {
            double* rec = a.o_rec + (size_t)i * PP_RECORD_WIDTH;
            for (int j = 0; j < 5; ++j) { rec[j] = op[j]; rec[5 + j] = oe[j]; }
            rec[10] = noDM; rec[11] = noGM; rec[12] = notau;
            rec[13] = chi2; rec[14] = chi2 / dof; rec[15] = sqrt(m[30]);
            rec[16] = (double)s.nfev; rec[17] = (double)s.status;
        }
        if (a.o_f0) a.o_f0[i] = s.f0;
        if (a.o_g0) for (int j = 0; j < 5; ++j) a.o_g0[(size_t)i * 5 + j] = s.g0[j];
        if (a.o_H0) for (int j = 0; j < 25; ++j) a.o_H0[(size_t)i * 25 + j] = s.H0[j];
    }
}

template <int CPT, int NT>
__global__ __launch_bounds__(NT) void k_finalize(FitArgs a) {
    __shared__ double scratch[PP_BSUM_DOUBLES(NT / 64, 31)];
    __shared__ double sh[2];
    finalize_body<CPT, NT, 1>(a, blockIdx.x, threadIdx.x, scratch, sh);
}
template <int NT>
__global__ __launch_bounds__(64) void k_finalize_v(FitArgs a) {
    __shared__ double scratch[PP_BSUM_DOUBLES(NT / 64, 31)];
    __shared__ double sh[2];
    finalize_body<0, NT, NT / 64>(a, blockIdx.x, threadIdx.x, scratch, sh);
// ... 4 lines not shown
```

pulseportraiture_amd/csrc/pp_tail.h:

```cpp
#pragma once
#include "pp_kernels.h"
#include "pp_extra.h"
#include "pp_xspec1024r.h"

namespace pp {

struct RefTailArgs {
    int on;
    int ncc;
    const cplx* part;
    const double* delta;
    const double* wsum;
    const unsigned* mws;
    const cplx* mspec;
    int mstride;
    FpsArgs fps;
    double* xs;
    double* seed_phase;
};
struct TailArgs {
    FitArgs fa;
    unsigned ticket, done;
    int nsub;
    int solve_nt, solve_pf;
    int fin_nt;
    RefTailArgs rs;
};

__device__ __forceinline__ void refseed_ticket(const RefTailArgs& r, const int nsub, const int i, const int tid, double* lds) {
    constexpr int M = 1024;
    static_assert(128 + 2 * M <= PP_TAIL_LDS_DOUBLES, "the fit's cross-spectrum in the carrying kernel's image");
    cplx* X = reinterpret_cast<cplx*>(lds + 128);
    {
        const double delta_i = r.delta[i], wsum_i = r.wsum[i];
        const double inv = wsum_i > 0.0 ? 1.0 / wsum_i : 0.0;
        cplx s[RS_NACC];
#pragma unroll
        for (int q = 0; q < RS_NACC; ++q) s[q] = make_double2(0.0, 0.0);
        const cplx* base = r.part + (size_t)i * r.ncc * RS_NACC * 64 + tid;
#pragma unroll 2
        for (int cc = 0; cc < r.ncc; ++cc) {
            if (r.mws && r.mws[(size_t)cc * nsub + i] == 0u) continue;
            cplx v[RS_NACC];
#pragma unroll
            for (int q = 0; q < RS_NACC; ++q)
                v[q] = (q < RS_NREG || tid == 0) ? base[((size_t)cc * RS_NACC + q) * 64] : make_double2(0.0, 0.0);
#pragma unroll
            for (int q = 0; q < RS_NACC; ++q) { s[q].x += v[q].x; s[q].y += v[q].y; }
        }
        const int lam = fftq_lambda(tid);
        auto put = [&](const int k, cplx t) __attribute__((always_inline)) {
            const cplx rot = unit_phasor((double)k, -delta_i);
            t = cmul(t, rot);
            t.x *= inv; t.y *= inv;
            if (k == M) t.y = 0.0;
            X[k - 1] = t;
        };
#pragma unroll
        for (int q = 0; q < 7; ++q) put(lam != 0 ? lam + 64 * q : 64 * (q + 1), s[q]);
#pragma unroll
        for (int q = 7; q < RS_NREG; ++q) put(lam + 64 * (12 + q - 7), s[q]);
        if (lam == 0) put(M, s[RS_NREG]);
#pragma unroll
        for (int kd = 7; kd < 12; ++kd) {
            const int k = lam + 64 * kd;
            if (k > 448) X[k - 1] = make_double2(0.0, 0.0);
        }
    }
    __syncthreads();
    const cplx* m = r.mspec + (size_t)i * r.mstride;
    auto dv = [&](const int k) __attribute__((always_inline)) { return X[k - 1]; };
    fps_body<4>(r.fps, i, tid, M, dv, m, X, lds, nullptr, nullptr);
    __syncthreads();
    if (tid == 0) refseed_start_one(r.fps.out7, i, r.xs, r.seed_phase);
    __syncthreads();
}

__device__ __noinline__ void tail_work(const TailArgs* t, double* lds, int nlds, int tid, int max_tickets) {
    TailArgs* tw = const_cast<TailArgs*>(t);
    const int nsub = t->nsub;
    for (int round = 0; round < max_tickets; ++round) {
        unsigned tk = 0;
        if (tid == 0) tk = atomicAdd(&tw->ticket, 1u);
        tk = (unsigned)__builtin_amdgcn_readfirstlane((int)tk);
        if (tk >= (unsigned)nsub) return;
        const FitArgs& a = t->fa;
        const int i = (int)tk;
        double* scratch = lds;
        double* sh = lds + 528;
        double* inv = lds + 536;
        (void)nlds;
        if (t->rs.on) refseed_ticket(t->rs, nsub, i, tid, lds);
        const int snt = t->solve_nt, spf = t->solve_pf, fnt = t->fin_nt;
        if (snt == 64) taylor_solve_body<64, PP_SOLVE_PF, 1>(a, i, tid, scratch, inv);
        else if (snt == 128) taylor_solve_body<128, PP_SOLVE_PF, 2>(a, i, tid, scratch, inv);
        else if (snt == 512) taylor_solve_body<512, PP_SOLVE_PF, 8>(a, i, tid, scratch, inv);
        else if (spf == 0) taylor_solve_body<256, 0, 4>(a, i, tid, scratch, inv);
        else taylor_solve_body<256, PP_SOLVE_PF, 4>(a, i, tid, scratch, inv);
        __syncthreads();
        if (fnt == 64) finalize_body<8, 64, 1>(a, i, tid, scratch, sh);
        else if (fnt == 128) finalize_body<0, 128, 2>(a, i, tid, scratch, sh);
        else if (fnt == 512) finalize_body<0, 512, 8>(a, i, tid, scratch, sh);
        else finalize_body<0, 256, 4>(a, i, tid, scratch, sh);
        __syncthreads();
        if (tid == 0) {
            __threadfence();
            const unsigned d = atomicAdd(&tw->done, 1u);
            if (d + 1u == (unsigned)nsub) {
                __threadfence();
                a.o_npass[a.nsub] = atomicAdd(a.nactive, 0);
            }
        }
    }
}

}
```

pulseportraiture_amd/csrc/pp_toas.hip:

```cpp
#include "../../include/pp_toas.h"

#include <hip/hip_runtime.h>

#include <algorithm>
#include <cmath>
#include <complex>
#include <deque>
#include <cstdarg>
#include <cstdio>
#include <climits>
#include <cstdint>
#include <cstring>
#include <map>
#include <atomic>
#include <string>
#include <thread>
#include <type_traits>
#include <vector>

#include "pp_kernels.h"
#include "pp_extra.h"
#include "pp_scrunch.h"
#include "pp_xspec1024r.h"
#include "pp_tail.h"
// ... 11 lines not shown
    va_start(ap, fmt);
    vsnprintf(buf, sizeof buf, fmt, ap);
    va_end(ap);
    g_err = buf;
    return code;
}

struct pp_ctx;
static int ctx_busy(pp_ctx* c, const char* who);

#define HIP_TRY(expr)                                                                        \
    do {                                                                                     \
        hipError_t e_ = (expr);                                                              \
        if (e_ != hipSuccess)                                                                \
            return fail(e_ == hipErrorOutOfMemory ? PP_ENOMEM : PP_EHIP, "%s: %s (%s:%d)",   \
                        #expr, hipGetErrorString(e_), __FILE__, __LINE__);                   \
    } while (0)

struct DevBuf {
    void* p = nullptr;
    size_t cap = 0;
    int reserve(size_t bytes) {
        if (bytes <= cap) return PP_OK;
        if (p) (void)hipFree(p);
        p = nullptr; cap = 0;
        hipError_t e = hipMalloc(&p, bytes);
        if (e != hipSuccess) {
            p = nullptr;
            return fail(PP_ENOMEM, "hipMalloc(%zu bytes): %s", bytes, hipGetErrorString(e));
        }
        cap = bytes;
        return PP_OK;
    }
    void release() { if (p) (void)hipFree(p); p = nullptr; cap = 0; }
    template <typename T> T* as() const { return reinterpret_cast<T*>(p); }
};

struct ModelSlot {
    bool set = false;
    int nchan = 0, nbin = 0, Kt = 0;
    int Mp = 0;
    DevBuf mft, msum, mmax, mdc, kt, msq;
};

__global__ void k_copy_words(unsigned long long* dst, const unsigned long long* src, size_t n) {
    for (size_t j = (size_t)blockIdx.x * blockDim.x + threadIdx.x; j < n; j += (size_t)gridDim.x * blockDim.x) dst[j] = src[j];
}
static int staged_copy(pp_ctx* c, void* dst, const void* src, size_t bytes, hipMemcpyKind kind, hipStream_t st = nullptr);
__global__ void k_publish_int(int* host_dst, const int* dev_src) { *host_dst = *dev_src; }
static int publish_int(pp_ctx* c, int* host_dst, const int* dev_src);
enum KernelFamily { KF_MODEL = 0, KF_XSPEC, KF_PREP, KF_SEED, KF_ACCUM, KF_EVAL, KF_TAYLOR, KF_STEP, KF_FINAL, KF_SYNTH, KF_FPS, KF_SCATMODEL, KF_PCA, KF_GAUSSRES, KF_GAUSSNORM, KF_NBSFFT, KF_NBSFIT, KF_SCRUNCH, KF_COUNT };
static const char* kFamilyNames[KF_COUNT] = {"model_fft", "xspec", "prep", "seed", "accum", "eval", "taylor_solve", "step", "finalize",
                                            "synth", "fit_phase_shift", "scat_model", "pca_gram", "gauss_resid", "gauss_normal", "nbscat_fft", "nbscat_fit", "scrunch"};

#define PP_NSTAGE 3
struct pp_ctx {
    int device = 0;
    hipStream_t stream = nullptr;
    std::map<int, DevBuf> twiddles;
    struct AnyPlan { int L = 0; DevBuf chirp, bft; };
    std::map<int, AnyPlan> anyplans;
    ModelSlot slots[PP_MAX_SLOTS];
    DevBuf mft_table, msum_table, kt_table, mdc_table, msq_table;
    DevBuf data, X, sdraw, noise, wts, freqs, errs, mask, P, x0, nufit, slot, csum, o_params, misc, seedbuf, seedq, xbase;
    std::map<const void*, int> occ_cache;
    DevBuf ticket;
    unsigned ticket_base = 0;
    void release_buffers() {
        for (DevBuf* b : {&mft_table, &msum_table, &kt_table, &mdc_table, &msq_table, &data, &X, &sdraw, &noise, &wts, &freqs, &errs,
                          &mask, &P, &x0, &nufit, &slot, &csum, &o_params, &misc, &seedbuf, &seedq, &xbase, &ticket}) b->release();
    }
    int ncu = 0;
    struct WorkSet {
        DevBuf inpack, sdraw, noise, wts, state, csum, partial, tay, mdl, ph0, misc, act, o_pack, o_f0, o_g0, o_H0,
            o_scales, o_serrs, o_csnr, refbuf,
            mwords;
        hipEvent_t xdone = nullptr;
        void release() {
            DevBuf* b[] = {&inpack, &sdraw, &noise, &wts, &state, &csum, &partial, &tay, &mdl, &ph0, &misc, &act, &o_pack,
                           &o_f0, &o_g0, &o_H0, &o_scales, &o_serrs, &o_csnr, &refbuf, &mwords};
            for (DevBuf* q : b) q->release();
            if (xdone) (void)hipEventDestroy(xdone);
            xdone = nullptr;
        }
    };
    WorkSet work[PP_NSTAGE];
    hipStream_t stream2 = nullptr;
    hipStream_t last_post = nullptr;
    int overlap_post = 0;
    struct Pca {
        DevBuf w, vec, part, D, S, G, U, B, small, idx, proj;
        int nchan = 0, nbin = 0, dual = 0, pitch = 0, nvec = 0;
        double fact = 0.0;
        void release() { for (DevBuf* b : {&w, &vec, &part, &D, &S, &G, &U, &B, &small, &idx, &proj}) b->release(); }
    } pca;
    struct Align {
        DevBuf acc, totw, off, pairs, harm, out;
        int npol = 0, nchan = 0, nbin = 0;
        bool open = false;
        void release() { for (DevBuf* b : {&acc, &totw, &off, &pairs, &harm, &out}) b->release(); open = false; }
    } align;
    struct GaussFit {
        DevBuf data, isig, freqs, R, part, gram, h, band;
        int nchan = 0, nbin = 0;
        int njoin = 0;
        double P = 1.0;
        int nsets = 0;
        long long nrow = 0;
        bool open = false;
        void release() { for (DevBuf* b : {&data, &isig, &freqs, &R, &part, &gram, &h, &band}) b->release(); open = false; nsets = 0; nrow = 0; njoin = 0; }
    } gfit;
    struct Wl {
        DevBuf x64, coef, med, noise, live, srow, out, small, fgrid, lev, par, idx;
        void release() { for (DevBuf* b : {&x64, &coef, &med, &noise, &live, &srow, &out, &small, &fgrid, &lev, &par, &idx}) b->release(); }
    } wl;
    struct Stage { void* in_host = nullptr; size_t in_cap = 0; void* o_host = nullptr; size_t o_cap = 0;
                   hipEvent_t t0 = nullptr, done = nullptr; };
    Stage stage[PP_NSTAGE];
    int cur_stage = 0;
    struct PendingTail {
        bool valid = false;
        int stage = 0;
        FitArgs fa;
        int ns = 0, C = 0, solve_nt = 0, solve_pf0 = 0, fin_nt = 0;
        pp_fit_out out; int s0 = 0; bool chan_dev = false; size_t copy_bytes = 0;
        RefTailArgs rs;
        cplx* rs_dspec = nullptr;
        cplx* rs_xwork = nullptr;
    } ptail;
    DevBuf tailbuf[PP_NSTAGE];
    void* tail_host[PP_NSTAGE] = {nullptr, nullptr, nullptr};
    int fuse_tail = 1;
    struct Deferred { pp_fit_in in; pp_fit_out out; int stage; bool queued; int rc; std::string err; size_t span_end = 0; };
    std::deque<Deferred> pending;
    int* nactive_h = nullptr;
    double harm_eps = 8.8817841970012523e-16;
    int max_iter = 64;
    int profile = 0;
    int check_every = 1;
    int check_from = 2;
    int use_taylor = 1;
    int moments_in_xspec = 1;
    int scat_model = 1;
    double scat_model_tol = 1e-10;
    int scat_model_bet = 1;
    int x_pad = 0;
    int fuse_scat = 1;
    int x_f32 = 0;
    int taylor_recentre = 1;
    int debug_poison = 0;
    int fps_finish = 0;
    int paired_split = 1;
    int one_exchange = 1;
    int seed_chan_stride = 16;
    int tail_virtual = 0;
    int refseed_stride = 0;
    double seed_min_snr = 8.0;
    int seed_ndm = 1;
    double seed_dm_step = 0.0;
    double max_work_bytes = 96e9;
    bool solve_lds_attr = false;
    int solve_cache = -1;
    int solve_prefetch = 0;
    int solve_threads = 0;
    int copy_kernels = 1;
    int finalize_regs = 1;
    int eager_flush = 1;
    int coarse_newton = 1;
    int nfev_shadow = -1;
    int skip_masked = 1;
    struct Span { int fam; hipEvent_t a, b; };
    std::vector<Span> spans;
    std::vector<hipEvent_t> ev_pool;
    std::map<int, double> known_ok;
    int max_lds_bytes = 0;
    double fam_sec[KF_COUNT] = {0};
    long long fam_n[KF_COUNT] = {0};
    hipEvent_t ev0 = nullptr, ev1 = nullptr;
    hipEvent_t evq[2] = {nullptr, nullptr};
    int lagged_check = 1;
    std::thread job;
    bool job_active = false;
    std::atomic<int> job_done{0};
    int job_rc = 0;
    std::string job_err;
    pp_fit_in job_in;
    pp_fit_out job_out;
};

static hipEvent_t prof_event(pp_ctx* c) {
    if (!c->ev_pool.empty()) { hipEvent_t e = c->ev_pool.back(); c->ev_pool.pop_back(); return e; }
    hipEvent_t e = nullptr;
    (void)hipEventCreate(&e);
    return e;
}

struct Prof {
    pp_ctx* c; int fam; hipStream_t st; hipEvent_t a = nullptr, b = nullptr;
    Prof(pp_ctx* c_, int fam_, hipStream_t st_ = nullptr) : c(c_), fam(fam_), st(st_ ? st_ : c_->stream) {
        if (c->profile) {
            a = prof_event(c); b = prof_event(c);
            (void)hipEventRecord(a, st);
        }
    }
    ~Prof() {
        if (c->profile) {
            (void)hipEventRecord(b, st);
            c->spans.push_back({fam, a, b});
        }
    }
};

static void resolve_spans(pp_ctx* c, size_t upto = (size_t)-1) {
    upto = std::min(upto, c->spans.size());
    for (size_t q = 0; q < upto; ++q) {
        auto& s = c->spans[q];
        float ms = 0.f;
        if (hipEventSynchronize(s.b) == hipSuccess && hipEventElapsedTime(&ms, s.a, s.b) == hipSuccess) {
            c->fam_sec[s.fam] += 1e-3 * ms;
            c->fam_n[s.fam] += 1;
        }
        c->ev_pool.push_back(s.a); c->ev_pool.push_back(s.b);
    }
    c->spans.erase(c->spans.begin(), c->spans.begin() + upto);
    for (auto& q : c->pending) q.span_end = q.span_end > upto ? q.span_end - upto : 0;
}

static void drain_spans(pp_ctx* c) {
    (void)hipStreamSynchronize(c->stream);
    if (c->stream2) (void)hipStreamSynchronize(c->stream2);
    resolve_spans(c);
}

static int ctx_busy(pp_ctx* c, const char* who) {
    if (!c) return PP_OK;
    if (c->job_active && t_worker_of != c)
        return fail(PP_ESTATE, "%s: a submitted fit is pending on this context (pp_fit_wait first)", who);
    if (!c->pending.empty())
        return fail(PP_ESTATE, "%s: %zu enqueued batch(es) not collected yet (pp_fit_collect first)", who, c->pending.size());
    return PP_OK;
}

extern "C" int pp_abi_version(void) { return PP_ABI_VERSION; }
extern "C" const char* pp_last_error(void) { return g_err.c_str(); }

static int ctx_init(pp_ctx* c) {
    HIP_TRY(hipStreamCreateWithFlags(&c->stream, hipStreamNonBlocking));
    {
        int prio_lo = 0, prio_hi = 0;
        (void)hipDeviceGetStreamPriorityRange(&prio_lo, &prio_hi);
        if (hipStreamCreateWithPriority(&c->stream2, hipStreamNonBlocking, prio_hi) != hipSuccess) {
            (void)hipGetLastError();
            HIP_TRY(hipStreamCreateWithFlags(&c->stream2, hipStreamNonBlocking));
        }
        for (auto& w : c->work) HIP_TRY(hipEventCreateWithFlags(&w.xdone, hipEventDisableTiming));
    }
    HIP_TRY(hipHostMalloc((void**)&c->nactive_h, sizeof(int) * 4, hipHostMallocDefault));
    HIP_TRY(hipEventCreate(&c->ev0));
    HIP_TRY(hipEventCreate(&c->ev1));
    for (auto& e : c->evq) HIP_TRY(hipEventCreateWithFlags(&e, hipEventDisableTiming));
    for (auto& sg : c->stage) { HIP_TRY(hipEventCreate(&sg.t0)); HIP_TRY(hipEventCreate(&sg.done)); }
    DevBuf* tables[] = {&c->mft_table, &c->msum_table, &c->kt_table, &c->mdc_table, &c->msq_table};
    for (DevBuf* t : tables) {
        int rc = t->reserve(sizeof(void*) * PP_MAX_SLOTS);
        if (rc) return rc;
        HIP_TRY(hipMemset(t->p, 0, sizeof(void*) * PP_MAX_SLOTS));
    }
    int rc = c->ticket.reserve(64);
    if (rc) return rc;
    HIP_TRY(hipMemset(c->ticket.p, 0, 64));
    return PP_OK;
}

extern "C" int pp_destroy(pp_ctx* c);

extern "C" int pp_create(int device_id, pp_ctx** out) {
    if (!out) return fail(PP_EINVAL, "pp_create: out is NULL");
    *out = nullptr;
    int ndev = 0;
    HIP_TRY(hipGetDeviceCount(&ndev));
    if (device_id < 0 || device_id >= ndev) return fail(PP_EINVAL, "pp_create: device %d of %d", device_id, ndev);
    HIP_TRY(hipSetDevice(device_id));
    pp_ctx* c = new pp_ctx();
    c->device = device_id;
    const int rc = ctx_init(c);
    if (rc) {
        const std::string keep = g_err;
        (void)pp_destroy(c);
        g_err = keep;
        return rc;
    }
    *out = c;
    return PP_OK;
}

extern "C" int pp_destroy(pp_ctx* c) {
    if (!c) return PP_OK;
    if (c->job_active) { c->job.join(); c->job_active = false; }
    (void)hipSetDevice(c->device);
    drain_spans(c);
    for (auto& w : c->work) w.release();
    for (auto& b : c->tailbuf) b.release();
    for (void*& h : c->tail_host) { if (h) (void)hipHostFree(h); h = nullptr; }
    for (auto& kv : c->twiddles) kv.second.release();
    for (auto& kv : c->anyplans) { kv.second.chirp.release(); kv.second.bft.release(); }
    for (auto& s : c->slots) { s.mft.release(); s.msum.release(); s.mmax.release(); s.mdc.release(); s.kt.release(); s.msq.release(); }
    for (auto& sg : c->stage) {
        if (sg.o_host) (void)hipHostFree(sg.o_host);
        if (sg.in_host) (void)hipHostFree(sg.in_host);
        if (sg.t0) (void)hipEventDestroy(sg.t0);
        if (sg.done) (void)hipEventDestroy(sg.done);
    }
    c->pca.release();
    c->align.release();
    c->gfit.release();
    c->wl.release();
    c->release_buffers();
    if (c->nactive_h) (void)hipHostFree(c->nactive_h);
    for (hipEvent_t e : c->ev_pool) (void)hipEventDestroy(e);
    c->ev_pool.clear();
    if (c->ev0) (void)hipEventDestroy(c->ev0);
    if (c->ev1) (void)hipEventDestroy(c->ev1);
    for (auto& e : c->evq) if (e) (void)hipEventDestroy(e);
    if (c->stream) (void)hipStreamDestroy(c->stream);
    if (c->stream2) (void)hipStreamDestroy(c->stream2);
    delete c;
    return PP_OK;
}

static int flush_tail(pp_ctx* c);
extern "C" int pp_synchronize(pp_ctx* c) {
    if (!c) return fail(PP_EINVAL, "null context");
    if (int rc = flush_tail(c)) return rc;
    HIP_TRY(hipStreamSynchronize(c->stream));
    HIP_TRY(hipStreamSynchronize(c->stream2));
    return PP_OK;
}

extern "C" void* pp_stream(pp_ctx* c) { return c ? (void*)c->stream : nullptr; }

namespace {
struct OptRef { const char* name; char kind; void* p; int imin; };
}
static bool option_ref(pp_ctx* c, const std::string& n, OptRef* out) {
    const OptRef tab[] = {
        {"harm_eps", 'd', &c->harm_eps, 0}, {"max_iter", 'i', &c->max_iter, INT32_MIN},
        {"profile", 'i', &c->profile, INT32_MIN}, {"check_every", 'i', &c->check_every, 1}, {"check_from", 'i', &c->check_from, 2},
        {"lagged_check", 'i', &c->lagged_check, INT32_MIN}, {"max_work_bytes", 'd', &c->max_work_bytes, 0},
        {"taylor", 'i', &c->use_taylor, INT32_MIN}, {"moments_in_xspec", 'i', &c->moments_in_xspec, INT32_MIN},
        {"paired_split", 'i', &c->paired_split, INT32_MIN}, {"one_exchange", 'i', &c->one_exchange, INT32_MIN},
        {"scat_model", 'i', &c->scat_model, INT32_MIN}, {"scat_model_tol", 'd', &c->scat_model_tol, 0},
        {"scat_model_bet", 'i', &c->scat_model_bet, INT32_MIN}, {"x_f32", 'i', &c->x_f32, INT32_MIN},
        {"fuse_scat", 'i', &c->fuse_scat, INT32_MIN}, {"x_pad", 'i', &c->x_pad, INT32_MIN},
        {"fps_finish", 'i', &c->fps_finish, INT32_MIN}, {"debug_poison", 'i', &c->debug_poison, INT32_MIN},
        {"taylor_recentre", 'i', &c->taylor_recentre, INT32_MIN}, {"seed_chan_stride", 'i', &c->seed_chan_stride, 1},
        {"seed_min_snr", 'd', &c->seed_min_snr, 0}, {"seed_ndm", 'i', &c->seed_ndm, 1},
        {"seed_dm_step", 'd', &c->seed_dm_step, 0}, {"skip_masked", 'i', &c->skip_masked, INT32_MIN},
        {"nfev_shadow", 'i', &c->nfev_shadow, INT32_MIN}, {"coarse_newton", 'i', &c->coarse_newton, INT32_MIN},
        {"eager_flush", 'i', &c->eager_flush, INT32_MIN},
        {"finalize_regs", 'i', &c->finalize_regs, INT32_MIN}, {"solve_cache", 'i', &c->solve_cache, -1},
        {"solve_threads", 'i', &c->solve_threads, 0}, {"copy_kernels", 'i', &c->copy_kernels, INT32_MIN},
        {"solve_prefetch", 'i', &c->solve_prefetch, INT32_MIN}, {"overlap_post", 'i', &c->overlap_post, INT32_MIN},
        {"refseed_stride", 'i', &c->refseed_stride, 0}, {"tail_virtual", 'i', &c->tail_virtual, INT32_MIN},
        {"fuse_tail", 'i', &c->fuse_tail, INT32_MIN},
    };
    for (const OptRef& o : tab)
        if (n == o.name) { *out = o; return true; }
    return false;
}

extern "C" int pp_set_option(pp_ctx* c, const char* name, double value) {
    if (!c || !name) return fail(PP_EINVAL, "pp_set_option: null argument");
    OptRef o;
    if (!option_ref(c, name, &o)) return fail(PP_EINVAL, "pp_set_option: unknown option '%s'", name);
    if (o.kind == 'd') *static_cast<double*>(o.p) = value;
    else *static_cast<int*>(o.p) = std::max(o.imin, (int)value);
    return PP_OK;
}

extern "C" int pp_get_option(pp_ctx* c, const char* name, double* value) {
    if (!c || !name || !value) return fail(PP_EINVAL, "pp_get_option: null argument");
    OptRef o;
    if (!option_ref(c, name, &o)) return fail(PP_EINVAL, "pp_get_option: unknown option '%s'", name);
    *value = o.kind == 'd' ? *static_cast<double*>(o.p) : (double)*static_cast<int*>(o.p);
    return PP_OK;
}

extern "C" int pp_kernel_times(pp_ctx* c, int cap, const char** names, double* seconds, int64_t* launches) {
    if (!c) return fail(PP_EINVAL, "null context");
    drain_spans(c);
    int n = std::min(cap, (int)KF_COUNT);
    for (int i = 0; i < n; ++i) {
        if (names) names[i] = kFamilyNames[i];
        if (seconds) seconds[i] = c->fam_sec[i];
        if (launches) launches[i] = c->fam_n[i];
    }
    return n;
}

extern "C" int pp_kernel_times_reset(pp_ctx* c) {
    if (!c) return fail(PP_EINVAL, "null context");
    drain_spans(c);
    for (int i = 0; i < KF_COUNT; ++i) { c->fam_sec[i] = 0; c->fam_n[i] = 0; }
    return PP_OK;
}

static int get_twiddles(pp_ctx* c, int nbin, const cplx** out) {
    auto it = c->twiddles.find(nbin);
    if (it != c->twiddles.end()) { *out = it->second.as<cplx>(); return PP_OK; }
    const int M = nbin / 2;
    std::vector<double> h(2 * (size_t)(M + 1));
    const long double two_pi = 6.283185307179586476925286766559005768L;
    for (int k = 0; k <= M; ++k) {
        long double ang = two_pi * (long double)k / (long double)nbin;
        h[2 * k] = (double)cosl(ang);
        h[2 * k + 1] = (double)(-sinl(ang));
    }
    h[0] = 1.0; h[1] = 0.0;
    if (M % 2 == 0) { h[2 * (M / 2)] = 0.0; h[2 * (M / 2) + 1] = -1.0; }
    h[2 * M] = -1.0; h[2 * M + 1] = 0.0;
    DevBuf b;
    int rc = b.reserve(h.size() * sizeof(double));
    if (rc) return rc;
    HIP_TRY(hipMemcpy(b.p, h.data(), h.size() * sizeof(double), hipMemcpyHostToDevice));
    c->twiddles[nbin] = b;
    *out = b.as<cplx>();
    return PP_OK;
}

static int staged_copy(pp_ctx* c, void* dst, const void* src, size_t bytes, hipMemcpyKind kind, hipStream_t st) {
    if (!st) st = c->stream;
    if (c->copy_kernels && bytes % 8 == 0 && bytes <= ((size_t)64 << 20)) {
        const size_t n = bytes / 8;
        const unsigned nb = (unsigned)std::min<size_t>((n + 255) / 256, 256);
        hipLaunchKernelGGL(k_copy_words, dim3(nb ? nb : 1), dim3(256), 0, st, (unsigned long long*)dst,
                           (const unsigned long long*)src, n);
        return hipGetLastError() == hipSuccess ? PP_OK : PP_EHIP;
    }
    return hipMemcpyAsync(dst, src, bytes, kind, st) == hipSuccess ? PP_OK : PP_EHIP;
}
static int publish_int(pp_ctx* c, int* host_dst, const int* dev_src) {
    if (c->copy_kernels) {
        hipLaunchKernelGGL(k_publish_int, dim3(1), dim3(1), 0, c->stream, host_dst, dev_src);
        return hipGetLastError() == hipSuccess ? PP_OK : PP_EHIP;
    }
    return hipMemcpyAsync(host_dst, dev_src, sizeof(int), hipMemcpyDeviceToHost, c->stream) == hipSuccess ? PP_OK : PP_EHIP;
}
static bool nbin_ok(int nbin) { return nbin >= 32 && nbin <= 8192 && (nbin & (nbin - 1)) == 0; }
static bool nbin_any_ok(int nbin) { return nbin_ok(nbin) || (nbin >= 8 && nbin <= 4096 && nbin % 2 == 0); }
static int fail(int code, const char* fmt, ...);
static int nbin_refuse(const char* who, int nbin) {
    return fail(PP_EINVAL, "%s: nbin %d must be a power of two in [32, 8192] or an even number in [8, 4096]", who, nbin);
}

static int get_twiddles(pp_ctx* c, int nbin, const cplx** out);
static int get_any_plan(pp_ctx* c, int nbin, pp_ctx::AnyPlan** out) {
    auto it = c->anyplans.find(nbin);
    if (it != c->anyplans.end()) { *out = &it->second; return PP_OK; }
    const int M = nbin / 2;
    int L = 16;
    while (L < 2 * M - 1) L <<= 1;
    const int sizes[4] = {64, 256, 1024, 4096};
    for (int sz : sizes) if (L <= sz) { L = sz; break; }
    const long double pi = 3.141592653589793238462643383279502884L;
    std::vector<double> w(2 * (size_t)M);
    std::vector<std::complex<long double>> b((size_t)L, std::complex<long double>(0.0L, 0.0L));
    for (int j = 0; j < M; ++j) {
        const long long q = ((long long)j * j) % (2LL * M);
        const long double ang = pi * (long double)q / (long double)M;
        const long double cs = cosl(ang), sn = sinl(ang);
        w[2 * (size_t)j] = (double)cs; w[2 * (size_t)j + 1] = (double)(-sn);
        b[j] = std::complex<long double>(cs, sn);
        if (j) b[L - j] = b[j];
    }
    {
        for (int i = 1, j = 0; i < L; ++i) {
            int bit = L >> 1;
            for (; j & bit; bit >>= 1) j ^= bit;
            j ^= bit;
            if (i < j) std::swap(b[i], b[j]);
        }
        for (int len = 2; len <= L; len <<= 1) {
            for (int i = 0; i < L; i += len)
                for (int k = 0; k < len / 2; ++k) {
                    const long double ang = -2.0L * pi * (long double)k / (long double)len;
                    const std::complex<long double> tw(cosl(ang), sinl(ang));
                    const std::complex<long double> u = b[i + k], v = b[i + k + len / 2] * tw;
                    b[i + k] = u + v; b[i + k + len / 2] = u - v;
                }
        }
    }
    std::vector<double> bf(2 * (size_t)L);
    for (int k = 0; k < L; ++k) { bf[2 * (size_t)k] = (double)b[k].real(); bf[2 * (size_t)k + 1] = (double)b[k].imag(); }
    pp_ctx::AnyPlan pl;
    pl.L = L;
    int rc;
    if ((rc = pl.chirp.reserve(w.size() * 8))) return rc;
    if ((rc = pl.bft.reserve(bf.size() * 8))) return rc;
    HIP_TRY(hipMemcpy(pl.chirp.p, w.data(), w.size() * 8, hipMemcpyHostToDevice));
    HIP_TRY(hipMemcpy(pl.bft.p, bf.data(), bf.size() * 8, hipMemcpyHostToDevice));
    c->anyplans[nbin] = pl;
    *out = &c->anyplans[nbin];
    return PP_OK;
}

static int fft_grid(int T, long long nrows) {
    long long g = 256LL * (T <= 128 ? 8 : (T == 256 ? 4 : 2));
    return (int)std::max(1LL, std::min(nrows, g));
}

template <typename F>
static void with_flag(bool b, F f) { if (b) f(std::true_type{}); else f(std::false_type{}); }
template <int MAX, typename F>
static void with_mode(int mode, F f) {
    if constexpr (MAX > 0) {
        if (mode == MAX) f(std::integral_constant<int, MAX>{});
        else with_mode<MAX - 1>(mode, f);
// ... 49 lines not shown
    return launch_any(c, xa, nbin, dtype, -1, false, hout, nullptr);
}

#define PP_DISPATCH_M(M_, ...)         \
    switch (M_) {                      \
        case 16: { constexpr int MM = 16; __VA_ARGS__; break; }     \
        case 32: { constexpr int MM = 32; __VA_ARGS__; break; }     \
        case 64: { constexpr int MM = 64; __VA_ARGS__; break; }     \
        case 128: { constexpr int MM = 128; __VA_ARGS__; break; }   \
        case 256: { constexpr int MM = 256; __VA_ARGS__; break; }   \
        case 512: { constexpr int MM = 512; __VA_ARGS__; break; }   \
        case 1024: { constexpr int MM = 1024; __VA_ARGS__; break; } \
        case 2048: { constexpr int MM = 2048; __VA_ARGS__; break; } \
        case 4096: { constexpr int MM = 4096; __VA_ARGS__; break; } \
        default: return fail(PP_EINVAL, "unsupported nbin %d", 2 * (M_)); \
    }

static int model_publish(pp_ctx* c, int slot) {
    ModelSlot& s = c->slots[slot];
    const int nchan = s.nchan, M = s.Mp;
    int rc;
    int Kt = M;
    {
        if ((rc = c->misc.reserve(256))) return rc;
        HIP_TRY(hipMemsetAsync(c->misc.p, 0, sizeof(int), c->stream));
        const double eps2 = c->harm_eps > 0.0 ? c->harm_eps * c->harm_eps : -1.0;
        hipLaunchKernelGGL(k_model_kcut, dim3(nchan), dim3(64), 0, c->stream, s.mft.as<cplx>(), s.mmax.as<double>(),
                           nchan, M, eps2, s.kt.as<int>(), c->misc.as<int>());
        HIP_TRY(hipGetLastError());
        HIP_TRY(hipMemcpyAsync(&Kt, c->misc.p, sizeof(int), hipMemcpyDeviceToHost, c->stream));
        HIP_TRY(hipStreamSynchronize(c->stream));
        Kt = std::min(M, std::max(64, Kt));
    }
    s.set = true; s.Kt = Kt;
    void* ptrs[5] = {s.mft.p, s.msum.p, s.kt.p, s.mdc.p, s.msq.p};
    DevBuf* tables[5] = {&c->mft_table, &c->msum_table, &c->kt_table, &c->mdc_table, &c->msq_table};
    for (int j = 0; j < 5; ++j)
        HIP_TRY(hipMemcpy((char*)tables[j]->p + sizeof(void*) * slot, &ptrs[j], sizeof(void*), hipMemcpyHostToDevice));
    return PP_OK;
}

extern "C" int pp_model_set(pp_ctx* c, int slot, const void* portrait, int dtype, int on_device, int nchan,
                            int nbin) {
    if (int busy_ = ctx_busy(c, "pp_model_set")) return busy_;
    if (!c || !portrait) return fail(PP_EINVAL, "pp_model_set: null argument");
    if (slot < 0 || slot >= PP_MAX_SLOTS) return fail(PP_EINVAL, "pp_model_set: slot %d", slot);
    if (!nbin_any_ok(nbin))
        return fail(PP_EINVAL, "pp_model_set: nbin %d must be a power of two in [32, 8192] or even in [8, 4096]", nbin);
    if (nchan < 1) return fail(PP_EINVAL, "pp_model_set: nchan %d", nchan);
    if (dtype != PP_F64 && dtype != PP_F32) return fail(PP_EINVAL, "pp_model_set: dtype %d", dtype);
    HIP_TRY(hipSetDevice(c->device));
    const bool anyb = !nbin_ok(nbin);
    const int M = nbin / 2, Mp = anyb ? ((M + 63) / 64) * 64 : M;
    const size_t esz = dtype == PP_F64 ? 8 : 4;
    ModelSlot& s = c->slots[slot];
    int rc;
    if ((rc = s.mft.reserve((size_t)nchan * Mp * sizeof(cplx)))) return rc;
    if ((rc = s.msum.reserve((size_t)nchan * sizeof(double)))) return rc;
    if ((rc = s.mmax.reserve((size_t)nchan * sizeof(double)))) return rc;
    if ((rc = s.mdc.reserve((size_t)nchan * sizeof(double)))) return rc;
    if ((rc = s.kt.reserve((size_t)nchan * sizeof(int)))) return rc;
    if ((rc = s.msq.reserve((size_t)nchan * Mp * sizeof(double)))) return rc;
    const void* dport = portrait;
    if (!on_device) {
        if ((rc = c->data.reserve((size_t)nchan * nbin * esz))) return rc;
        HIP_TRY(hipMemcpyAsync(c->data.p, portrait, (size_t)nchan * nbin * esz, hipMemcpyHostToDevice, c->stream));
        dport = c->data.p;
    }
    if (anyb) {
        if ((rc = c->X.reserve((size_t)nchan * (M + 1) * sizeof(cplx)))) return rc;
        Prof pr(c, KF_MODEL);
        if ((rc = harmonics_any(c, dport, dtype, 1, nchan, nbin, c->X.as<cplx>()))) return rc;
        hipLaunchKernelGGL(k_model_from_harm, dim3(nchan), dim3(64), 0, c->stream, (const cplx*)c->X.p, M, Mp,
                           s.mft.as<cplx>(), s.msq.as<double>(), s.msum.as<double>(), s.mmax.as<double>(), s.mdc.as<double>());
        HIP_TRY(hipGetLastError());
        s.nchan = nchan; s.nbin = nbin; s.Mp = Mp;
        return model_publish(c, slot);
    }
    const cplx* tw = nullptr;
    if ((rc = get_twiddles(c, nbin, &tw))) return rc;
    ModelFftArgs a{dport, s.mft.as<cplx>(), s.msum.as<double>(), s.mmax.as<double>(), s.mdc.as<double>(),
                   s.msq.as<double>(), tw, nchan};
    {
        Prof pr(c, KF_MODEL);
        PP_DISPATCH_M(M, {
            const int T = FftPlan<MM>::T;
            with_dtype(dtype, [&](auto t) { hipLaunchKernelGGL((k_model_fft<MM, decltype(t)>), dim3(fft_grid(T, nchan)), dim3(T), 0, c->stream, a); });
        });
    }
    HIP_TRY(hipGetLastError());
    s.nchan = nchan; s.nbin = nbin; s.Mp = M;
    return model_publish(c, slot);
}

extern "C" int pp_model_dc(pp_ctx* c, int slot, double* dc) {
    if (!c || !dc || slot < 0 || slot >= PP_MAX_SLOTS || !c->slots[slot].set) return fail(PP_ESTATE, "slot not set");
    HIP_TRY(hipSetDevice(c->device));
    HIP_TRY(hipMemcpyAsync(dc, c->slots[slot].mdc.p, (size_t)c->slots[slot].nchan * sizeof(double),
                           hipMemcpyDeviceToHost, c->stream));
    HIP_TRY(hipStreamSynchronize(c->stream));
    return PP_OK;
}

extern "C" int pp_model_shape(pp_ctx* c, int slot, int* nchan, int* nbin) {
    if (!c || !nchan || !nbin) return fail(PP_EINVAL, "pp_model_shape: null argument");
    if (slot < 0 || slot >= PP_MAX_SLOTS || !c->slots[slot].set) return fail(PP_ESTATE, "pp_model_shape: slot %d not set", slot);
    *nchan = c->slots[slot].nchan;
    *nbin = c->slots[slot].nbin;
    return PP_OK;
}

extern "C" int pp_model_nharm(pp_ctx* c, int slot) {
    if (!c || slot < 0 || slot >= PP_MAX_SLOTS || !c->slots[slot].set) return fail(PP_ESTATE, "slot not set");
    return c->slots[slot].Kt;
}

static int rows_harmonics(pp_ctx* c, const void* rows, int dtype, int nrows, int nbin, cplx* hout) {
    if (!nbin_ok(nbin)) return harmonics_any(c, rows, dtype, 1, nrows, nbin, hout);
    const cplx* tw = nullptr;
    int rc;
    if ((rc = get_twiddles(c, nbin, &tw))) return rc;
    PP_DISPATCH_M(nbin / 2, {
        const int T = FftPlan<MM>::T;
        if (dtype == PP_F64) hipLaunchKernelGGL((k_rfft_rows<MM, double>), dim3(fft_grid(T, nrows)), dim3(T), 0, c->stream, rows, hout, tw, nrows);
        else hipLaunchKernelGGL((k_rfft_rows<MM, float>), dim3(fft_grid(T, nrows)), dim3(T), 0, c->stream, rows, hout, tw, nrows);
    });
    HIP_TRY(hipGetLastError());
    return PP_OK;
}

extern "C" int pp_rfft_rows(pp_ctx* c, const void* rows, int dtype, int nrows, int nbin, double* out) {
    if (int busy_ = ctx_busy(c, "pp_rfft_rows")) return busy_;
    if (!c || !rows || !out) return fail(PP_EINVAL, "pp_rfft_rows: null argument");
    if (!nbin_any_ok(nbin) || nrows < 1) return fail(PP_EINVAL, "pp_rfft_rows: bad shape %d x %d", nrows, nbin);
    HIP_TRY(hipSetDevice(c->device));
    const size_t in_b = (size_t)nrows * nbin * (dtype == PP_F64 ? 8 : 4), out_b = (size_t)nrows * (nbin / 2 + 1) * sizeof(cplx);
    int rc;
    if ((rc = c->data.reserve(in_b))) return rc;
    if ((rc = c->X.reserve(out_b))) return rc;
    HIP_TRY(hipMemcpyAsync(c->data.p, rows, in_b, hipMemcpyHostToDevice, c->stream));
    if ((rc = rows_harmonics(c, c->data.p, dtype, nrows, nbin, c->X.as<cplx>()))) return rc;
    HIP_TRY(hipMemcpyAsync(out, c->X.p, out_b, hipMemcpyDeviceToHost, c->stream));
    HIP_TRY(hipStreamSynchronize(c->stream));
    return PP_OK;
}

static int upload(pp_ctx* c, DevBuf& b, const void* src, size_t bytes) {
    int rc = b.reserve(bytes);
    if (rc) return rc;
    HIP_TRY(hipMemcpyAsync(b.p, src, bytes, hipMemcpyHostToDevice, c->stream));
    return PP_OK;
}

template <typename K>
static int resident_grid(pp_ctx* c, K kernel, int T, long long nrows, int fallback) {
    const void* key = reinterpret_cast<const void*>(kernel);
    auto it = c->occ_cache.find(key);
    int per_cu = 0;
    if (it != c->occ_cache.end()) per_cu = it->second;
    else {
        if (hipOccupancyMaxActiveBlocksPerMultiprocessor(&per_cu, kernel, T, 0) != hipSuccess || per_cu < 1) {
            (void)hipGetLastError();
            per_cu = 0;
        }
        c->occ_cache[key] = per_cu;
    }
    if (!c->ncu) {
        hipDeviceProp_t prop;
        c->ncu = (hipGetDeviceProperties(&prop, c->device) == hipSuccess && prop.multiProcessorCount > 0)
                     ? prop.multiProcessorCount : 256;
    }
    const long long g = per_cu > 0 ? (long long)per_cu * c->ncu : (long long)fallback;
    return (int)std::max(1LL, std::min(nrows, g));
}

static void draw_tickets(pp_ctx* c, XspecArgs& x, long long nrows, bool advance = true) {
    x.ticket = c->ticket.as<unsigned>();
    x.ticket_base = c->ticket_base;
    if (advance) c->ticket_base += (unsigned)((nrows + PP_ROW_CHUNK - 1) / PP_ROW_CHUNK);
}

template <int MM, typename TIN>
static void launch_xspec(pp_ctx* c, const XspecArgs& xa_in, bool tail, int mode) {
    const int T = FftPlan<MM>::T;
    const long long nrows = (long long)xa_in.nsub * xa_in.nchan;
    XspecArgs xa = xa_in;
    draw_tickets(c, xa, nrows, T == 64);
    auto launch = [&](auto kernel) {
        const dim3 grid(resident_grid(c, kernel, T, nrows, fft_grid(T, nrows)));
        hipLaunchKernelGGL(kernel, grid, dim3(T), 0, c->stream, xa);
    };
    if constexpr (MM == 1024) {
        if (c->one_exchange && mode == 2 && 2 * xa.Kt < MM)
            return with_flag(tail, [&](auto TL) { launch(k_xspec_q1024<TIN, decltype(TL)::value>); });
        if (c->one_exchange && mode == 3)
            return with_flag(tail, [&](auto TL) { launch(k_xspec_qf<1024, TIN, decltype(TL)::value>); });
    }
    if constexpr (MM == 512) {
        if (c->one_exchange && (mode == 2 || mode == 3))
            return with_flag(tail, [&](auto TL) { launch(k_xspec_qf<512, TIN, decltype(TL)::value>); });
    }
    if constexpr (MM == 1024 && sizeof(TIN) == 4) {
        if (c->paired_split && 2 * xa.Kt < MM && mode <= 2 && !xa.act && xa.cstep == 1)
            return with_flag(tail, [&](auto TL) {
                with_mode<2>(mode, [&](auto MD) { launch(k_xspec_p1024<TIN, decltype(TL)::value, decltype(MD)::value>); });
            });
    }
    with_flag(tail, [&](auto TL) { with_mode<3>(mode, [&](auto MD) { launch(k_xspec<MM, TIN, decltype(TL)::value, decltype(MD)::value>); }); });
}

struct OutBlock {
    double *params, *errs, *nu, *cov, *chi2, *rchi2, *snr, *seed_phase;
    int32_t *nfev, *rc, *npass, *unfinished;
    static size_t bytes(size_t ns) { return (ns * 340 + 8 + 7) & ~(size_t)7; }
    static size_t staged_bytes(size_t ns) { return bytes(ns) + ns * 8; }
    OutBlock(const void* base, size_t ns) {
        double* d = params = reinterpret_cast<double*>(const_cast<void*>(base));
        errs = d + ns * 5; nu = d + ns * 10; cov = d + ns * 13; chi2 = d + ns * 38; rchi2 = d + ns * 39; snr = d + ns * 40;
        nfev = reinterpret_cast<int32_t*>(d + ns * 41); rc = nfev + ns; npass = rc + ns; unfinished = npass + ns;
        seed_phase = reinterpret_cast<double*>(reinterpret_cast<char*>(d) + bytes(ns));
    }
};
static void unpack_stage(const void* o_host, pp_fit_out* out, int s0, int ns) {
    const OutBlock h(o_host, ns);
    const struct { void* dst; const void* src; size_t bytes; } part[] = {
        {out->params, h.params, 40}, {out->param_errs, h.errs, 40}, {out->nu_refs, h.nu, 24}, {out->cov, h.cov, 200}, {out->chi2, h.chi2, 8},
        {out->red_chi2, h.rchi2, 8}, {out->snr, h.snr, 8}, {out->nfeval, h.nfev, 4}, {out->return_code, h.rc, 4}, {out->npass, h.npass, 4}};
    for (const auto& q : part) if (q.dst) memcpy((char*)q.dst + (size_t)s0 * q.bytes, q.src, (size_t)ns * q.bytes);
}
static void unpack_seed_phases(const void* o_host, const pp_fit_in* in, int s0, int ns) {
    if (in->ref_seed && in->ref_seed->seed_phase)
        memcpy(in->ref_seed->seed_phase + s0, OutBlock(o_host, ns).seed_phase, (size_t)ns * 8);
}
static int unfinished_in_stage(const void* o_host, int ns) { return *OutBlock(o_host, ns).unfinished; }

struct InBlock { double *freqs, *P, *x0, *nufit, *nuout, *rs_mprof, *rs_numean, *rs_xs; int* slot; };
struct InLayout {
    size_t ns, B, nfreq, rs_nprof, rs_on;
    InLayout(const pp_fit_in* in, int ns_)
        : ns(ns_), B(in->nbin), nfreq(in->freqs_stride ? (size_t)ns_ * in->nchan : (size_t)in->nchan),
          rs_nprof(in->ref_seed ? (in->ref_seed->model_prof_stride ? (size_t)ns_ : 1) : 0), rs_on(in->ref_seed ? 1 : 0) {}
    size_t bytes() const {
        return ((nfreq + ns * (1 + 5 + 3 + 3) + rs_nprof * B + rs_on * ns * (1 + 5)) * 8 + ns * 4 + 7) & ~(size_t)7;
    }
    InBlock at(void* base) const {
        InBlock b;
        b.freqs = reinterpret_cast<double*>(base);
        b.P = b.freqs + nfreq; b.x0 = b.P + ns; b.nufit = b.x0 + ns * 5; b.nuout = b.nufit + ns * 3;
        b.rs_mprof = b.nuout + ns * 3; b.rs_numean = b.rs_mprof + rs_nprof * B; b.rs_xs = b.rs_numean + rs_on * ns;
        b.slot = reinterpret_cast<int*>(b.rs_xs + rs_on * ns * 5);
        return b;
    }
};

static int solve_threads_for(const pp_ctx* c, int C) { return c->solve_threads > 0 ? c->solve_threads : (C <= 512 ? 64 : C <= 1024 ? 128 : 256); }
static bool solve_rows_in_turn(const pp_ctx* c, int C, int solve_nt) { return solve_nt == 256 && C > 2048 && c->solve_prefetch <= 0; }
static void solve_launch(pp_ctx* c, FitArgs& fa, int ns, int C, int solve_nt, hipStream_t sp) {
    size_t lds = (size_t)fa.solve_cache * 32;
    if (lds > 48 * 1024 && !c->solve_lds_attr) {
        const void* fns[9] = {(const void*)k_taylor_solve<64>, (const void*)k_taylor_solve<128>, (const void*)k_taylor_solve<256>,
                              (const void*)k_taylor_solve<256, 0>, (const void*)k_taylor_solve<512>,
                              (const void*)k_taylor_solve_v<128>, (const void*)k_taylor_solve_v<256>,
                              (const void*)k_taylor_solve_v<256, 0>, (const void*)k_taylor_solve_v<512>};
        bool ok = true;
        for (const void* fn : fns)
            ok = (hipFuncSetAttribute(fn, hipFuncAttributeMaxDynamicSharedMemorySize, PP_SOLVE_CACHE_MAX * 32) == hipSuccess) && ok;
        if (!ok) {
            (void)hipGetLastError();
            c->solve_cache = 0;
        }
        c->solve_lds_attr = true;
    }
    if (lds > 48 * 1024 && c->solve_cache == 0) { fa.solve_cache = 0; lds = 0; }
    const bool in_turn = solve_rows_in_turn(c, C, solve_nt);
    const bool virt = c->tail_virtual && solve_nt > 64;
    void (*kernel)(FitArgs);
    if (solve_nt == 64) kernel = k_taylor_solve<64>;
    else if (solve_nt == 128) kernel = virt ? k_taylor_solve_v<128> : k_taylor_solve<128>;
    else if (solve_nt == 512) kernel = virt ? k_taylor_solve_v<512> : k_taylor_solve<512>;
    else if (in_turn) kernel = virt ? k_taylor_solve_v<256, 0> : k_taylor_solve<256, 0>;
    else kernel = virt ? k_taylor_solve_v<256> : k_taylor_solve<256>;
    const int threads = virt ? 64 : (solve_nt == 64 || solve_nt == 128 || solve_nt == 512) ? solve_nt : 256;
    hipLaunchKernelGGL(kernel, dim3(ns), dim3(threads), lds, sp, fa);
}
static int finalize_threads_for(const pp_ctx* c, const FitArgs& ff, int C) {
    return (ff.ncs != 3 || C > 4096 || !c->finalize_regs) ? 0
           : c->finalize_regs > 1 ? c->finalize_regs : C <= 512 ? 64 : C <= 1024 ? 128 : C <= 2048 ? 256 : 512;
}
static int finalize_width_taken(const pp_ctx* c, const FitArgs& ff, int C) {
    const int fnt = finalize_threads_for(c, ff, C);
    return (fnt == 64 && C <= 512) ? 64 : (fnt == 128 && C <= 1024) ? 128 : (fnt == 256 && C <= 2048) ? 256 : fnt == 512 ? 512 : 0;
}
static void finalize_launch(pp_ctx* c, const FitArgs& ff, int ns, int C, hipStream_t sp) {
    const int fnt = finalize_threads_for(c, ff, C), w = finalize_width_taken(c, ff, C);
    const bool virt = c->tail_virtual && fnt > 64 && C <= 8 * fnt;
    void (*kernel)(FitArgs);
    if (virt && fnt == 128) kernel = k_finalize_v<128>;
    else if (virt && fnt == 256) kernel = k_finalize_v<256>;
    else if (virt) kernel = k_finalize_v<512>;
    else if (w == 64) kernel = k_finalize<8, 64>;
    else if (w == 128) kernel = k_finalize<8, 128>;
    else if (w == 256) kernel = k_finalize<8, 256>;
    else if (w == 512) kernel = k_finalize<8, 512>;
    else kernel = k_finalize<0, 256>;
    hipLaunchKernelGGL(kernel, dim3(ns), dim3(virt ? 64 : w ? w : 256), 0, sp, ff);
}
static int queue_outputs(pp_ctx* c, int stage, const pp_fit_out* out, int s0, int ns, int C, bool chan_dev, size_t copy_bytes,
                         hipStream_t sp) {
    pp_ctx::Stage& sg = c->stage[stage];
    pp_ctx::WorkSet& W = c->work[stage];
    const size_t nc = (size_t)ns * C;
    int rc;
#define PP_D2H(dst, buf, off, bytes) \
    if (dst) HIP_TRY(hipMemcpyAsync((char*)(dst) + (off), (buf).p, (bytes), hipMemcpyDeviceToHost, sp))
    if ((rc = staged_copy(c, sg.o_host, W.o_pack.p, copy_bytes, hipMemcpyDeviceToHost, sp))) return fail(rc, "output block copy failed");
    if (!chan_dev) {
        PP_D2H(out->scales, W.o_scales, (size_t)s0 * C * 8, nc * 8);
        PP_D2H(out->scale_errs, W.o_serrs, (size_t)s0 * C * 8, nc * 8);
        PP_D2H(out->channel_snrs, W.o_csnr, (size_t)s0 * C * 8, nc * 8);
    }
    PP_D2H(out->obj_f, W.o_f0, (size_t)s0 * 8, (size_t)ns * 8);
    PP_D2H(out->obj_grad, W.o_g0, (size_t)s0 * 40, (size_t)ns * 40);
    PP_D2H(out->obj_hess, W.o_H0, (size_t)s0 * 200, (size_t)ns * 200);
#undef PP_D2H
    return PP_OK;
}
static int queue_refseed_finish(pp_ctx* c, const RefTailArgs& r, int ns, cplx* dspec, cplx* xwork, hipStream_t st, bool span_to_end) {
    constexpr int M = 1024;
    const size_t H = (size_t)M + 1;
    FpsArgs f = r.fps;
    f.spec = dspec; f.specm = r.mspec; f.mstride = r.mstride;
    auto start = [&]() {
        hipLaunchKernelGGL(k_refseed_start, dim3((ns + 63) / 64), dim3(64), 0, st, (const double*)r.fps.out7, ns, r.xs, r.seed_phase);
    };
    {
        Prof pr(c, KF_FPS, st);
        hipLaunchKernelGGL(k_refseed_finish, dim3((unsigned)((H + 255) / 256), ns), dim3(256), 0, st, r.part, r.ncc, r.delta, r.wsum,
                           ns, dspec, r.mws);
        hipLaunchKernelGGL(k_fps, dim3(ns), dim3(256), 0, st, f, xwork);
        if (span_to_end) start();
    }
    HIP_TRY(hipGetLastError());
    if (!span_to_end) { start(); HIP_TRY(hipGetLastError()); }
    return PP_OK;
}
static int flush_tail_queue(pp_ctx* c, pp_ctx::PendingTail& t) {
    int rc;
// ... 883 lines not shown
```

pulseportraiture_amd/csrc/pp_xspec1024q.h:

```cpp
#pragma once
#include "pp_fftq.h"


namespace pp {

constexpr unsigned PP_TICKET_WINDOW_NUM = 3u, PP_TICKET_WINDOW_DEN = 4u;
__device__ __forceinline__ int ticket_moment(const long long nrows) {
    const unsigned share = (unsigned)(nrows / (long long)gridDim.x) + 1u;
    return 1 + (int)(((blockIdx.x * 2654435761u) >> 8) % (share * PP_TICKET_WINDOW_NUM / PP_TICKET_WINDOW_DEN + 1u));
}

template <int M, typename Tin>
__device__ __forceinline__ const Tin* next_row_of(const XspecArgs& a, const unsigned more_nx, const int i_nx, const int n_nx,
                                                  const size_t rc) {
    const size_t rn = more_nx ? (size_t)sub_of(a.act, i_nx) * a.nchan_full + (a.coff + n_nx * a.cstep) : rc;
    return reinterpret_cast<const Tin*>(a.data) + rn * (2 * M);
}

constexpr int FFTQ_FREE_ELEM0 = 3 * 272 + 16, FFTQ_FREE_PITCH = 17;

template <int M, bool TAIL, bool ONE = true, bool LEAN = false>
__device__ __forceinline__ void store_row_results(const XspecArgs& a, const size_t rc, const int tid, double tv) {
    constexpr int H = M + 1, kc = (int)(0.75 * H);
  if constexpr (ONE && LEAN) {
    static_assert(!TAIL && PP_TJ == 10 && PP_TSTRIDE == 12, "sign pattern of totals 0..11; S_d in the quads behind them");
    const unsigned q = (unsigned)wave_reduce16_index(tid);
    const double th = 0.5 * tv;
    double val = __hiloint2double((int)((unsigned)__double2hiint(th) + (((q + 1u) >> 1) << 31)), __double2loint(th));
    double* dst = a.tay + tay_idx(rc, 0) + q;
    if (q >= (unsigned)PP_TSTRIDE) { val = tv; dst = a.sdraw + rc; }
    typedef double __attribute__((address_space(1)))* gdp_t;
    *(gdp_t)(uintptr_t)dst = val;
  } else if constexpr (ONE) {
    const int q = wave_reduce16_index(tid);
    const double th = 0.5 * tv;
    double val = (q <= PP_TJ && ((q & 3) == 1 || (q & 3) == 2)) ? -th : th;
    double* dst = a.tay + tay_idx(rc, q < PP_TSTRIDE ? q : 0);
    if (q >= PP_TSTRIDE) { val = tv; dst = a.sdraw + rc; }
    if (TAIL) {
        const double nz = sqrt(tv / (2.0 * M) / (double)(H - kc));
        if (q > PP_TSTRIDE) { val = nz; dst = a.noise + rc; }
    }
    typedef double __attribute__((address_space(1)))* gdp_t;
    *(gdp_t)(uintptr_t)dst = val;
  } else {
    if ((tid & 3) == 0) {
        const int q = wave_reduce16_index(tid);
        if (q < PP_TSTRIDE) {
            tv *= 0.5;
            a.tay[tay_idx(rc, q)] = (q <= PP_TJ && ((q & 3) == 1 || (q & 3) == 2)) ? -tv : tv;
        }
    }
    if (tid == 4 * PP_TSTRIDE) a.sdraw[rc] = tv;
    if (TAIL && tid == 4 * (PP_TSTRIDE + 1)) a.noise[rc] = sqrt(tv / (2.0 * M) / (double)(H - kc));
  }
}

__device__ __forceinline__ void first_row_landed() { __builtin_amdgcn_s_waitcnt(0x0F70); }

constexpr int Q_PREFETCH_F64 = 1, Q_PREFETCH_F32 = 0;
template <typename Tin, bool TAIL>
__global__ __launch_bounds__(64, 2) void k_xspec_q1024(XspecArgs a) {
    constexpr int M = 1024, T = 64, R1 = 16, PER1 = 1;
    constexpr int NSL = 7;
    typedef typename RawOf<Tin>::type Raw;
    constexpr int NRED = PP_TSTRIDE + (TAIL ? 2 : 1);
    static_assert(NRED <= 16, "wave_reduce_lds takes 16 values");
    constexpr int WRED = PP_WRED_DOUBLES(NRED) / 2;
    constexpr int LDSN = WRED > FFTQ_LDS_ELEMS ? WRED : FFTQ_LDS_ELEMS;
    static_assert(2 * LDSN >= PP_TAIL_LDS_DOUBLES, "tail_work's layout of this kernel's LDS");
    constexpr bool F64 = sizeof(Tin) == 8;
    constexpr int NML = (F64 && TAIL) ? 2 : 0;
    constexpr bool TWL = F64 && !TAIL, TWR = F64 && TAIL;
    constexpr bool ROWTOP = !TAIL;
    constexpr int NTW = TWL ? 2 : 0;
    __shared__ cplx lds[LDSN + 64 * (NML + NTW)];
    static_assert(sizeof(lds) <= 19456, "eight workgroups per CU");
    static_assert(FFTQ_FREE_ELEM0 + 15 * FFTQ_FREE_PITCH < FFTQ_LDS_ELEMS && FFTQ_FREE_ELEM0 >= 64 * (TAIL ? 12 : 7) &&
                  2 * FFTQ_FREE_ELEM0 >= PP_WRED_DOUBLES(NRED), "t2's elements are outside everything a row writes");
    cplx* const ldsm = lds + LDSN + threadIdx.x;
    int tid = threadIdx.x;
    const long long nrows = (long long)a.nsub * a.nchan;
    Raw cur[PER1][R1];
    cplx t1 = a.twB[2 * tid], t2 = a.twB[32 * (tid & 15)];
    const int lam0 = fftq_lambda(tid);
    cplx wb0 = a.twB[lam0 ? lam0 : 64];
    const cplx wbT = a.twB[64];
    cplx* const ldt2 = lds + FFTQ_FREE_ELEM0;
    cplx* const ldtw = lds + LDSN + 64 * NML;
    auto put_lane_consts = [&](const cplx p1, const cplx p2, const cplx pb) {
        if (!TWL) return;
        ldt2[FFTQ_FREE_PITCH * (tid & 15)] = p2;
        ldtw[tid] = p1;
        ldtw[64 + tid] = pb;
        lds_sync<T>();
    };
    put_lane_consts(t1, t2, wb0);
    int tail_after = 0x7fffffff;
    if (a.tail) tail_after = ticket_moment(nrows);
    RowWalk<true> rw;
    rw.start(nrows, a.mwords, a.ticket, a.ticket_base);
    long long row = rw.row;
    int n = 0, i = 0;
    if (rw.more) {
        n = __builtin_amdgcn_readfirstlane((int)(row / a.nsub));
        i = __builtin_amdgcn_readfirstlane((int)(row % a.nsub));
        const size_t rc = (size_t)sub_of(a.act, i) * a.nchan_full + (a.coff + n * a.cstep);
        stage_load_global<M, T, R1>(cur, reinterpret_cast<const Tin*>(a.data) + rc * (2 * M), tid);
    }
    cplx mv2[NSL];
    const cplx* mheld = nullptr;
    const cplx* mrow = nullptr;
    int n_held = -1, ktn = 0;
    int i_nx = i, n_nx = n;
    constexpr bool FASTROW = TWL;
    if (ROWTOP) first_row_landed();
#pragma unroll 1
    for (int phase = 0; phase < 2; ++phase) {
    if (phase == 1) {
        if (!a.tail) break;
        tail_work(a.tail, reinterpret_cast<double*>(lds), 2 * (LDSN + 64 * NML), tid, 1);
        tail_after = 0x7fffffff;
        if (TWL) {
            const int lamr = fftq_lambda(tid);
            put_lane_consts(as_global(a.twB)[2 * tid], as_global(a.twB)[32 * (tid & 15)], as_global(a.twB)[lamr ? lamr : 64]);
        }
    }
    unsigned fast_left = 0u;
    size_t rc_prev = 0;
    unsigned lanepk = 0u;
    if (TWL) {
        const int lamp = fftq_lambda(tid);
        lanepk = 16u * (unsigned)fftq_lane_of((64 - lamp) & 63) | (unsigned)(lamp ? lamp : 64) << 10;
    }
    for (; rw.more && tail_after != 0; rw.advance(), row = rw.row, i = i_nx, n = n_nx, --tail_after) {
        if (!FASTROW) {
            rw.draw(a.ticket);
            rw.peek(nrows, a.ticket_base, a.mwords);
        }
        asm volatile("" : "+v"(tid));
        if (TWL) {
            asm volatile("" : "+v"(lanepk));
            __builtin_assume((unsigned)tid < 64u);
        }
        const int lam = TWL ? 0 : fftq_lambda(tid);
        const bool l0 = TWL ? (tid == 0) : (lam == 0);
        const int kb = TWL ? (int)(lanepk >> 10) : (l0 ? 64 : lam);
        if (TWR) {
            t1 = as_global(a.twB)[2 * tid];
            t2 = as_global(a.twB)[32 * (tid & 15)];
            wb0 = as_global(a.twB)[kb];
        } else if (!TWL) {
            asm volatile("" : "+v"(t1.x), "+v"(t1.y), "+v"(t2.x), "+v"(t2.y), "+v"(wb0.x), "+v"(wb0.y));
        }
        size_t rc;
        const Tin* nxrow = nullptr;
        if (FASTROW && fast_left != 0u) {
            --fast_left;
            rc = rc_prev + (size_t)(unsigned)a.nchan_full;
            rw.row_nx = rw.row + 1u;
            rw.bits &= rw.bits - 1u;
            i_nx = i + 1;
// ... 263 lines not shown
```

Measured before the change: 77600.

## Add per-wave independent row walker kernel for 1024-point cross-spectrum with wave-local tail

```diff
diff --git a/pulseportraiture_amd/csrc/pp_common.h b/pulseportraiture_amd/csrc/pp_common.h
--- a/pulseportraiture_amd/csrc/pp_common.h
+++ b/pulseportraiture_amd/csrc/pp_common.h
@@ -172,6 +172,15 @@
 }
 #define PP_WRED_DOUBLES(NS) ((NS) * 68)
 
+template <bool WV>
+__device__ __forceinline__ void team_sync() {
+    if constexpr (WV) {
+        __builtin_amdgcn_fence(__ATOMIC_RELEASE, "workgroup");
+        __builtin_amdgcn_wave_barrier();
+        __builtin_amdgcn_fence(__ATOMIC_ACQUIRE, "workgroup");
+    } else __syncthreads();
+}
+
 template <int NV>
 __device__ inline void block_sum(double (&v)[NV], double* scratch) {
     const int lane = threadIdx.x & 63, wid = threadIdx.x >> 6, nw = blockDim.x >> 6;
diff --git a/pulseportraiture_amd/csrc/pp_extra.h b/pulseportraiture_amd/csrc/pp_extra.h
--- a/pulseportraiture_amd/csrc/pp_extra.h
+++ b/pulseportraiture_amd/csrc/pp_extra.h
@@ -797,7 +797,7 @@
 }
 
 #define PP_FPS_LDS 2048
-template <int NV, int NVW, typename F>
+template <int NV, int NVW, bool WV = false, typename F>
 __device__ __forceinline__ void fps_bsum(double (&out)[NV], double* scratch, int tid, F&& part) {
     if constexpr (NVW == 1) {
         part(tid, out);
@@ -816,14 +816,14 @@
                 for (int q = 0; q < NV; ++q) scratch[vw * NV + q] = v[q];
             }
         }
-        __syncthreads();
+        team_sync<WV>();
 #pragma unroll
         for (int q = 0; q < NV; ++q) {
             double t = 0.0;
             for (int w = 0; w < NVW; ++w) t += scratch[w * NV + q];
             out[q] = t;
         }
-        __syncthreads();
+        team_sync<WV>();
     }
 }
 
@@ -867,13 +867,13 @@
     return sim0;
 }
 
-template <int NVW, typename DF>
+template <int NVW, bool WV = false, typename DF>
 __device__ __forceinline__ void fps_body(const FpsArgs& a, const int i, const int tid, const int M, DF&& dspec,
                                          const cplx* m, cplx* X, double* scratch, double* shv, int* shj) {
     constexpr int RT = 256 / NVW;
     const int H = M + 1, kc = (int)(0.75 * H);
     double v[3];
-    fps_bsum<3, NVW>(v, scratch, tid, [&](const int vt, double (&u)[3]) __attribute__((always_inline)) {
+    fps_bsum<3, NVW, WV>(v, scratch, tid, [&](const int vt, double (&u)[3]) __attribute__((always_inline)) {
         u[0] = u[1] = u[2] = 0.0;
         for (int k = 1 + vt; k <= M; k += 256) {
             const cplx dk = dspec(k), mk = m[k];
@@ -913,7 +913,7 @@
     double phi = (Ns > 1) ? add_rn(mul_rn((double)best, h), a.lo) : a.lo;
     double f = 0.0, f2 = 0.0;
     auto sums_at = [&](double x, double (&s)[3]) __attribute__((always_inline)) {
-        fps_bsum<3, NVW>(s, scratch, tid, [&](const int vt, double (&u)[3]) __attribute__((always_inline)) {
+        fps_bsum<3, NVW, WV>(s, scratch, tid, [&](const int vt, double (&u)[3]) __attribute__((always_inline)) {
             fps_sums(X, M, x, vt, 256, u[0], u[1], u[2]);
         });
     };
diff --git a/pulseportraiture_amd/csrc/pp_fftq.h b/pulseportraiture_amd/csrc/pp_fftq.h
--- a/pulseportraiture_amd/csrc/pp_fftq.h
+++ b/pulseportraiture_amd/csrc/pp_fftq.h
@@ -25,11 +25,26 @@
 
 constexpr int FFTQ_LDS_ELEMS = 4 * 272;
 
-template <int WHEN = 0, bool LEAN = false, typename T1, typename T2, typename Mid>
+template <int WHEN = 0, bool LEAN = false, bool TAB = false, typename T1, typename T2, typename Mid>
 __device__ __forceinline__ void fftq1024_from(cplx (&v)[16], cplx* lds, T1 get_t1, T2 get_t2, int tid,
                                               double* power, Mid mid) {
     dft16_first(v);
     if (WHEN == 0) mid();
+    if constexpr (TAB) {
+        constexpr int AHEAD = 8;
+        cplx wq[16];
+#pragma unroll
+        for (int j = 1; j <= AHEAD; ++j) wq[j] = get_t1(j);
+        __builtin_amdgcn_sched_barrier(0);
+        dft16_second(v);
+#pragma unroll
+        for (int j = 1; j < 16; ++j) {
+            __builtin_amdgcn_sched_barrier(0);
+            if (j + AHEAD < 16) wq[j + AHEAD] = get_t1(j + AHEAD);
+            v[j] = cmul(v[j], wq[j]);
+        }
+        __builtin_amdgcn_sched_barrier(0);
+    } else {
     const cplx t1 = get_t1();
     dft16_second(v);
     {
@@ -44,6 +59,7 @@
         }
 #pragma unroll
         for (int j = 1; j < 16; ++j) v[j] = cmul(v[j], wq[j]);
+    }
     }
     if (WHEN == 1) mid();
     const cplx t2 = get_t2();
diff --git a/pulseportraiture_amd/csrc/pp_kernels.h b/pulseportraiture_amd/csrc/pp_kernels.h
--- a/pulseportraiture_amd/csrc/pp_kernels.h
+++ b/pulseportraiture_amd/csrc/pp_kernels.h
@@ -17,7 +17,14 @@
 struct TailArgs;
 #define PP_TAIL_LDS_DOUBLES 2176
 #define PP_TAIL_CACHE ((PP_TAIL_LDS_DOUBLES - 536) / 4)
-__device__ void tail_work(const TailArgs* t, double* lds, int nlds, int tid, int max_tickets);
+template <bool WV>
+__device__ void tail_work_as(const TailArgs* t, double* lds, int nlds, int tid, int max_tickets);
+__device__ __forceinline__ void tail_work(const TailArgs* t, double* lds, int nlds, int tid, int max_tickets) {
+    tail_work_as<false>(t, lds, nlds, tid, max_tickets);
+}
+__device__ __forceinline__ void tail_work_wave(const TailArgs* t, double* lds, int nlds, int tid, int max_tickets) {
+    tail_work_as<true>(t, lds, nlds, tid, max_tickets);
+}
 
 struct XspecArgs {
     const void* data;
@@ -175,8 +182,14 @@
 }
 
 constexpr int PP_ROW_CHUNK = 32;
-template <bool DYN>
+template <bool DYN, bool CU = false>
 struct RowWalk {
+    static __device__ __forceinline__ unsigned me() {
+        if constexpr (CU) return 8u * blockIdx.x + (unsigned)__builtin_amdgcn_readfirstlane((int)(threadIdx.x >> 6));
+        else return blockIdx.x;
+    }
+    static __device__ __forceinline__ unsigned walkers() { if constexpr (CU) return 8u * gridDim.x; else return gridDim.x; }
+    static __device__ __forceinline__ unsigned lane() { if constexpr (CU) return threadIdx.x & 63u; else return threadIdx.x; }
     unsigned row, row_nx;
     unsigned bits;
     unsigned wnx, cnx;
@@ -193,10 +206,10 @@
     static __device__ __forceinline__ unsigned chunk_after(unsigned c, unsigned* ticket, unsigned base) {
         if (DYN) {
             unsigned t = 0;
-            if (threadIdx.x == 0) t = atomicAdd(ticket, 1u);
-            return gridDim.x + (__builtin_amdgcn_readfirstlane(t) - base);
-        }
-        return c + gridDim.x;
+            if (lane() == 0u) t = atomicAdd(ticket, 1u);
+            return walkers() + (__builtin_amdgcn_readfirstlane(t) - base);
+        }
+        return c + walkers();
     }
     __device__ __forceinline__ void enter(unsigned c, unsigned w, unsigned nrows) {
         more_nx = (c * PP_ROW_CHUNK < nrows) ? 1u : 0u;
@@ -208,7 +221,7 @@
         static_assert(PP_ROW_CHUNK == 32, "one 32-bit word per chunk");
         const unsigned nrows = (unsigned)nrows_;
         wnx = 0; cnx = 0; have_wnx = 0u;
-        unsigned c = blockIdx.x;
+        unsigned c = me();
         unsigned w = word_of(mw, c, nrows);
         while (w == 0u && c * PP_ROW_CHUNK < nrows) {
             c = chunk_after(c, ticket, base);
@@ -216,15 +229,15 @@
         }
         enter(c, __builtin_amdgcn_readfirstlane(w), nrows);
         row = row_nx; more = more_nx;
-        tick = threadIdx.x;
+        tick = lane();
         fresh = 1u;
     }
     __device__ __forceinline__ void draw(unsigned* ticket) {
-        if (DYN && fresh && threadIdx.x == 0) tick = atomicAdd(ticket, 1u);
+        if (DYN && fresh && lane() == 0u) tick = atomicAdd(ticket, 1u);
     }
     __device__ __forceinline__ void peek(long long nrows_, unsigned base, const unsigned* mw) {
         if (mw && !fresh && !have_wnx) {
-            cnx = DYN ? gridDim.x + (__builtin_amdgcn_readfirstlane(tick) - base) : (row >> 5) + gridDim.x;
+            cnx = DYN ? walkers() + (__builtin_amdgcn_readfirstlane(tick) - base) : (row >> 5) + walkers();
             wnx = word_of(mw, cnx, (unsigned)nrows_);
             have_wnx = 1u;
         }
@@ -244,7 +257,7 @@
         unsigned c, w;
         if (have_wnx) { c = cnx; w = wnx; have_wnx = 0u; }
         else {
-            c = DYN ? gridDim.x + (__builtin_amdgcn_readfirstlane(tick) - base) : (row >> 5) + gridDim.x;
+            c = DYN ? walkers() + (__builtin_amdgcn_readfirstlane(tick) - base) : (row >> 5) + walkers();
             w = word_of(mw, c, nrows);
         }
         while (w == 0u && c * PP_ROW_CHUNK < nrows) {
@@ -266,7 +279,7 @@
             more_nx = 1u;
             return;
         }
-        unsigned c = DYN ? gridDim.x + (__builtin_amdgcn_readfirstlane(tick) - base) : (row >> 5) + gridDim.x;
+        unsigned c = DYN ? walkers() + (__builtin_amdgcn_readfirstlane(tick) - base) : (row >> 5) + walkers();
         unsigned w = word_of(mw, c, nrows);
         while (w == 0u && c * PP_ROW_CHUNK < nrows) {
             c = chunk_after(c, ticket, base);
@@ -1344,7 +1357,7 @@
 #define PP_SOLVE_CACHE_MAX 4096
 constexpr int PP_SOLVE_PF = 2;
 constexpr int PP_TAYLOR_WAVES = 2;
-template <int NV, int NVMAX, int NT, int NVW, typename F>
+template <int NV, int NVMAX, int NT, int NVW, bool WV = false, typename F>
 __device__ __forceinline__ void vblock_sum(double (&out)[NV], double* scratch, int& flip, double* mx, int tid, F&& accumulate) {
     static_assert(NV <= NVMAX, "scratch sized for NVMAX values");
     constexpr int NWV = NT / 64, RT = NT / NVW;
@@ -1367,7 +1380,7 @@
 #pragma unroll 1
         for (int k = 0; k < NVW; ++k) one_wave(rw + (RT / 64) * k);
     }
-    __syncthreads();
+    team_sync<WV>();
 #pragma unroll
     for (int i = 0; i < NV; ++i) out[i] = 0.0;
 #pragma unroll 1
@@ -1383,7 +1396,7 @@
     }
 }
 
-template <int NT, int PF, int NVW>
+template <int NT, int PF, int NVW, bool WV = false>
 __device__ __forceinline__ void taylor_solve_body(const FitArgs& a, const int i, const int tid, double* scratch, double* inv_lds) {
     constexpr int RT = NT / NVW;
     static_assert(NT % 64 == 0 && RT % 64 == 0 && NT % RT == 0, "whole waves");
@@ -1415,7 +1428,7 @@
             phase_geom(freqs[n], P, nuDM, nuGM, p1, p2);
             inv_w[n] = wts[n]; inv_p1[n] = p1; inv_p2[n] = p2; inv_S[n] = msum[n];
         }
-        __syncthreads();
+        team_sync<WV>();
     }
     auto chan_inv = [&](int n, double& w, double& p1, double& p2, double& S0) {
         if (n < ncache) { w = inv_w[n]; p1 = inv_p1[n]; p2 = inv_p2[n]; S0 = inv_S[n]; }
@@ -1467,7 +1480,7 @@
     auto evalm = [&](const double* dx, double& f, double* g, double* H, bool at_origin = false) -> double {
         double acc[10];
         double dmax = 0.0;
-        vblock_sum<10, 10, NT, NVW>(acc, scratch, flip, &dmax, tid, [&](const int vt, double (&ac)[10], double& dm) __attribute__((always_inline)) {
+        vblock_sum<10, 10, NT, NVW, WV>(acc, scratch, flip, &dmax, tid, [&](const int vt, double (&ac)[10], double& dm) __attribute__((always_inline)) {
             auto add = [&](double w, double p1, double p2, double S0, double A0, double A1, double A2) {
                 const bool in = (w != 0.0);
                 const double r = A0 / S0;
@@ -1603,7 +1616,7 @@
         double ev[4];
         double jf = 1.0;
         for (int j = 2; j <= PP_TJ; ++j) jf *= (double)j;
-        vblock_sum<4, 10, NT, NVW>(ev, scratch, flip, nullptr, tid, [&](const int vt, double (&e4)[4], double&) __attribute__((always_inline)) {
+        vblock_sum<4, 10, NT, NVW, WV>(ev, scratch, flip, nullptr, tid, [&](const int vt, double (&e4)[4], double&) __attribute__((always_inline)) {
             for_channels(vt, [&](int n, const double (&t)[PP_TSTRIDE]) {
                 double w, p1, p2, S0;
                 chan_inv(n, w, p1, p2, S0);
@@ -1927,7 +1940,7 @@
     return x;
 }
 
-template <int CPT, int NT, int NVW>
+template <int CPT, int NT, int NVW, bool WV = false>
 __device__ __forceinline__ void finalize_body(const FitArgs& a, const int i, const int tid, double* scratch, double* sh) {
     static_assert(NVW == 1 || CPT == 0, "channels held in registers belong to real threads");
     constexpr int RT = NT / NVW;
@@ -1987,7 +2000,7 @@
         }
     };
     double v3[3];
-    vblock_sum<3, 31, NT, NVW>(v3, scratch, flip, nullptr, tid, [&](const int vt, double (&u3)[3], double&) __attribute__((always_inline)) {
+    vblock_sum<3, 31, NT, NVW, WV>(v3, scratch, flip, nullptr, tid, [&](const int vt, double (&u3)[3], double&) __attribute__((always_inline)) {
         for_channels(vt, [&](int n, int q) {
             const double w = wt_of(n, q);
             double sd;
@@ -2006,7 +2019,7 @@
     double nzDM = nfDM, nzGM = nfGM, nztau = nftau;
     if (need_zero) {
         double v[20];
-        vblock_sum<20, 31, NT, NVW>(v, scratch, flip, nullptr, tid, [&](const int vt, double (&v)[20], double&) __attribute__((always_inline)) {
+        vblock_sum<20, 31, NT, NVW, WV>(v, scratch, flip, nullptr, tid, [&](const int vt, double (&v)[20], double&) __attribute__((always_inline)) {
         for_channels(vt, [&](int n, int q) {
             const double w = wt_of(n, q);
             if (w == 0.0) return;
@@ -2089,9 +2102,9 @@
                 const double A = v[0], B = v[1], C = v[2], D = v[3], E = v[4], F = v[3], G = v[5], Hh = v[1];
                 double co[4] = {A * C - E * G, E * Hh - A * D, F * G - B * C, B * D - F * Hh};
                 if (tid == 0) sh[0] = pick_poly_root(co, 3, fmean, true);
-                __syncthreads();
+                team_sync<WV>();
                 nzDM = nzGM = sh[0];
-                __syncthreads();
+                team_sync<WV>();
             }
             break;
         case 0x1B: {
@@ -2126,9 +2139,9 @@
                     deg = 4;
                 }
                 if (tid == 0) sh[0] = pick_poly_root(co, deg, fmean, true);
-                __syncthreads();
+                team_sync<WV>();
                 nzDM = nzGM = sh[0];
-                __syncthreads();
+                team_sync<WV>();
             }
             break;
         default: break;
@@ -2148,7 +2161,7 @@
     const double phi_out = py_wrap_half(phi_inf + k1 * DM / (noDM * noDM) + k2 * GM / (noGM * noGM * noGM * noGM));
     const double tau_out = tau * pow(notau / nftau, alpha);
     double m[31];
-    vblock_sum<31, 31, NT, NVW>(m, scratch, flip, nullptr, tid, [&](const int vt, double (&m)[31], double&) __attribute__((always_inline)) {
+    vblock_sum<31, 31, NT, NVW, WV>(m, scratch, flip, nullptr, tid, [&](const int vt, double (&m)[31], double&) __attribute__((always_inline)) {
     for_channels(vt, [&](int n, int q) {
         const double w = wt_of(n, q);
         if (w == 0.0) return;
diff --git a/pulseportraiture_amd/csrc/pp_tail.h b/pulseportraiture_amd/csrc/pp_tail.h
--- a/pulseportraiture_amd/csrc/pp_tail.h
+++ b/pulseportraiture_amd/csrc/pp_tail.h
@@ -27,6 +27,7 @@
     RefTailArgs rs;
 };
 
+template <bool WV = false>
 __device__ __forceinline__ void refseed_ticket(const RefTailArgs& r, const int nsub, const int i, const int tid, double* lds) {
     constexpr int M = 1024;
     static_assert(128 + 2 * M <= PP_TAIL_LDS_DOUBLES, "the fit's cross-spectrum in the carrying kernel's image");
@@ -67,16 +68,17 @@
             if (k > 448) X[k - 1] = make_double2(0.0, 0.0);
         }
     }
-    __syncthreads();
+    team_sync<WV>();
     const cplx* m = r.mspec + (size_t)i * r.mstride;
     auto dv = [&](const int k) __attribute__((always_inline)) { return X[k - 1]; };
-    fps_body<4>(r.fps, i, tid, M, dv, m, X, lds, nullptr, nullptr);
-    __syncthreads();
+    fps_body<4, WV>(r.fps, i, tid, M, dv, m, X, lds, nullptr, nullptr);
+    team_sync<WV>();
     if (tid == 0) refseed_start_one(r.fps.out7, i, r.xs, r.seed_phase);
-    __syncthreads();
+    team_sync<WV>();
 }
 
-__device__ __noinline__ void tail_work(const TailArgs* t, double* lds, int nlds, int tid, int max_tickets) {
+template <bool WV>
+__device__ __noinline__ void tail_work_as(const TailArgs* t, double* lds, int nlds, int tid, int max_tickets) {
     TailArgs* tw = const_cast<TailArgs*>(t);
     const int nsub = t->nsub;
     for (int round = 0; round < max_tickets; ++round) {
@@ -90,19 +92,19 @@
         double* sh = lds + 528;
         double* inv = lds + 536;
         (void)nlds;
-        if (t->rs.on) refseed_ticket(t->rs, nsub, i, tid, lds);
+        if (t->rs.on) refseed_ticket<WV>(t->rs, nsub, i, tid, lds);
         const int snt = t->solve_nt, spf = t->solve_pf, fnt = t->fin_nt;
-        if (snt == 64) taylor_solve_body<64, PP_SOLVE_PF, 1>(a, i, tid, scratch, inv);
-        else if (snt == 128) taylor_solve_body<128, PP_SOLVE_PF, 2>(a, i, tid, scratch, inv);
-        else if (snt == 512) taylor_solve_body<512, PP_SOLVE_PF, 8>(a, i, tid, scratch, inv);
-        else if (spf == 0) taylor_solve_body<256, 0, 4>(a, i, tid, scratch, inv);
-        else taylor_solve_body<256, PP_SOLVE_PF, 4>(a, i, tid, scratch, inv);
-        __syncthreads();
-        if (fnt == 64) finalize_body<8, 64, 1>(a, i, tid, scratch, sh);
-        else if (fnt == 128) finalize_body<0, 128, 2>(a, i, tid, scratch, sh);
-        else if (fnt == 512) finalize_body<0, 512, 8>(a, i, tid, scratch, sh);
-        else finalize_body<0, 256, 4>(a, i, tid, scratch, sh);
-        __syncthreads();
+        if (snt == 64) taylor_solve_body<64, PP_SOLVE_PF, 1, WV>(a, i, tid, scratch, inv);
+        else if (snt == 128) taylor_solve_body<128, PP_SOLVE_PF, 2, WV>(a, i, tid, scratch, inv);
+        else if (snt == 512) taylor_solve_body<512, PP_SOLVE_PF, 8, WV>(a, i, tid, scratch, inv);
+        else if (spf == 0) taylor_solve_body<256, 0, 4, WV>(a, i, tid, scratch, inv);
+        else taylor_solve_body<256, PP_SOLVE_PF, 4, WV>(a, i, tid, scratch, inv);
+        team_sync<WV>();
+        if (fnt == 64) finalize_body<8, 64, 1, WV>(a, i, tid, scratch, sh);
+        else if (fnt == 128) finalize_body<0, 128, 2, WV>(a, i, tid, scratch, sh);
+        else if (fnt == 512) finalize_body<0, 512, 8, WV>(a, i, tid, scratch, sh);
+        else finalize_body<0, 256, 4, WV>(a, i, tid, scratch, sh);
+        team_sync<WV>();
         if (tid == 0) {
             __threadfence();
             const unsigned d = atomicAdd(&tw->done, 1u);
diff --git a/pulseportraiture_amd/csrc/pp_toas.hip b/pulseportraiture_amd/csrc/pp_toas.hip
--- a/pulseportraiture_amd/csrc/pp_toas.hip
+++ b/pulseportraiture_amd/csrc/pp_toas.hip
@@ -187,6 +187,9 @@
     int fps_finish = 0;
     int paired_split = 1;
     int one_exchange = 1;
+    int cu_tables = 1;
+    int cu_grid_cap = 0;
+    bool cu_ready = false;
     int seed_chan_stride = 16;
     int tail_virtual = 0;
     int refseed_stride = 0;
@@ -279,6 +282,9 @@
 extern "C" int pp_abi_version(void) { return PP_ABI_VERSION; }
 extern "C" const char* pp_last_error(void) { return g_err.c_str(); }
 
+extern "C" __attribute__((visibility("hidden"))) int pp_cu1024_prepare(void);
+extern "C" __attribute__((visibility("hidden"))) void pp_cu1024_launch(const void* xspec_args, long long nrows, int ncu, hipStream_t stream);
+
 static int ctx_init(pp_ctx* c) {
     HIP_TRY(hipStreamCreateWithFlags(&c->stream, hipStreamNonBlocking));
     {
@@ -304,6 +310,8 @@
     int rc = c->ticket.reserve(64);
     if (rc) return rc;
     HIP_TRY(hipMemset(c->ticket.p, 0, 64));
+    c->cu_ready = pp_cu1024_prepare() == (int)hipSuccess;
+    if (!c->cu_ready) (void)hipGetLastError();
     return PP_OK;
 }
 
@@ -397,7 +405,8 @@
         {"solve_threads", 'i', &c->solve_threads, 0}, {"copy_kernels", 'i', &c->copy_kernels, INT32_MIN},
         {"solve_prefetch", 'i', &c->solve_prefetch, INT32_MIN}, {"overlap_post", 'i', &c->overlap_post, INT32_MIN},
         {"refseed_stride", 'i', &c->refseed_stride, 0}, {"tail_virtual", 'i', &c->tail_virtual, INT32_MIN},
-        {"fuse_tail", 'i', &c->fuse_tail, INT32_MIN},
+        {"fuse_tail", 'i', &c->fuse_tail, INT32_MIN}, {"cu_tables", 'i', &c->cu_tables, INT32_MIN},
+        {"cu_grid_cap", 'i', &c->cu_grid_cap, 0},
     };
     for (const OptRef& o : tab)
         if (n == o.name) { *out = o; return true; }
@@ -753,6 +762,14 @@
     return PP_OK;
 }
 
+static int cu_count(pp_ctx* c) {
+    if (!c->ncu) {
+        hipDeviceProp_t prop;
+        c->ncu = (hipGetDeviceProperties(&prop, c->device) == hipSuccess && prop.multiProcessorCount > 0)
+                     ? prop.multiProcessorCount : 256;
+    }
+    return c->ncu;
+}
 template <typename K>
 static int resident_grid(pp_ctx* c, K kernel, int T, long long nrows, int fallback) {
     const void* key = reinterpret_cast<const void*>(kernel);
@@ -766,12 +783,7 @@
         }
         c->occ_cache[key] = per_cu;
     }
-    if (!c->ncu) {
-        hipDeviceProp_t prop;
-        c->ncu = (hipGetDeviceProperties(&prop, c->device) == hipSuccess && prop.multiProcessorCount > 0)
-                     ? prop.multiProcessorCount : 256;
-    }
-    const long long g = per_cu > 0 ? (long long)per_cu * c->ncu : (long long)fallback;
+    const long long g = per_cu > 0 ? (long long)per_cu * cu_count(c) : (long long)fallback;
     return (int)std::max(1LL, std::min(nrows, g));
 }
 
@@ -792,8 +804,15 @@
         hipLaunchKernelGGL(kernel, grid, dim3(T), 0, c->stream, xa);
     };
     if constexpr (MM == 1024) {
-        if (c->one_exchange && mode == 2 && 2 * xa.Kt < MM)
+        if (c->one_exchange && mode == 2 && 2 * xa.Kt < MM) {
+            if constexpr (sizeof(TIN) == 8) {
+                if (c->cu_tables && c->cu_ready && !tail && !xa.mwords && !xa.act && !xa.slot) {
+                    const int ncu = cu_count(c);
+                    return pp_cu1024_launch(&xa, nrows, c->cu_grid_cap > 0 ? std::min(ncu, c->cu_grid_cap) : ncu, c->stream);
+                }
+            }
             return with_flag(tail, [&](auto TL) { launch(k_xspec_q1024<TIN, decltype(TL)::value>); });
+        }
         if (c->one_exchange && mode == 3)
             return with_flag(tail, [&](auto TL) { launch(k_xspec_qf<1024, TIN, decltype(TL)::value>); });
     }
diff --git a/pulseportraiture_amd/csrc/pp_xspec1024cu.h b/pulseportraiture_amd/csrc/pp_xspec1024cu.h
--- /dev/null
+++ b/pulseportraiture_amd/csrc/pp_xspec1024cu.h
@@ -0,0 +1,191 @@
+#pragma once
+#include "pp_xspec1024q.h"
+
+namespace pp {
+
+constexpr int CU_WAVES = 8, CU_NT1 = 15, CU_NWB = 7;
+constexpr int CU_IMAGE_ELEMS = FFTQ_LDS_ELEMS;
+constexpr int CU_LDS_BYTES = (CU_WAVES * CU_IMAGE_ELEMS + 64 * (CU_NT1 + CU_NWB)) * (int)sizeof(cplx);
+static_assert(CU_LDS_BYTES == 161792 && CU_LDS_BYTES <= 163840, "one workgroup per CU, the whole LDS");
+static_assert(2 * CU_IMAGE_ELEMS >= PP_TAIL_LDS_DOUBLES, "tail_work's layout of a wave's image");
+
+template <typename Tin>
+__global__ __launch_bounds__(64 * CU_WAVES, 2) void k_xspec_cu1024(XspecArgs a) {
+    constexpr int M = 1024, T = 64, R1 = 16, PER1 = 1;
+    constexpr int NSL = CU_NWB;
+    typedef typename RawOf<Tin>::type Raw;
+    static_assert(sizeof(Tin) == 8, "f64 rows");
+    constexpr int NRED = PP_TSTRIDE + 1;
+    constexpr int LDSN = CU_IMAGE_ELEMS;
+    static_assert(PP_WRED_DOUBLES(NRED) / 2 <= LDSN, "the reduction inside the image");
+    static_assert(FFTQ_FREE_ELEM0 + 15 * FFTQ_FREE_PITCH < FFTQ_LDS_ELEMS && FFTQ_FREE_ELEM0 >= 64 * 7 &&
+                  2 * FFTQ_FREE_ELEM0 >= PP_WRED_DOUBLES(NRED), "t2's elements are outside everything a row writes");
+    extern __shared__ cplx cu_lds[];
+    const int wave = __builtin_amdgcn_readfirstlane((int)(threadIdx.x >> 6));
+    int tid = threadIdx.x & 63;
+    cplx* const lds = cu_lds + wave * LDSN;
+    cplx* const tab1 = cu_lds + CU_WAVES * LDSN;
+    cplx* const tabw = tab1 + 64 * CU_NT1;
+    const long long nrows = (long long)a.nsub * a.nchan;
+    Raw cur[PER1][R1];
+    if (wave == 0) {
+        cplx wq[16];
+        wq[1] = a.twB[2 * tid];
+#pragma unroll
+        for (int j = 2; j < 16; ++j) {
+            if (j % 2 == 0) {
+                const cplx h = wq[j / 2];
+                wq[j] = make_double2(fma(h.x, h.x, -h.y * h.y), 2.0 * h.x * h.y);
+            } else wq[j] = cmul(wq[j - 1], wq[1]);
+        }
+#pragma unroll
+        for (int j = 1; j < 16; ++j) tab1[64 * (j - 1) + tid] = wq[j];
+        const int lamf = fftq_lambda(tid);
+        cplx wb = a.twB[lamf ? lamf : 64];
+        const cplx wbT = a.twB[64];
+#pragma unroll
+        for (int j = 0; j < CU_NWB; ++j) {
+            tabw[64 * j + tid] = wb;
+            wb = cmul(wb, wbT);
+        }
+    }
+    cplx* const ldt2 = lds + FFTQ_FREE_ELEM0;
+    auto put_lane_consts = [&](const cplx p2) {
+        ldt2[FFTQ_FREE_PITCH * (tid & 15)] = p2;
+        lds_sync<T>();
+    };
+    put_lane_consts(a.twB[32 * (tid & 15)]);
+    __syncthreads();
+    int tail_after = 0x7fffffff;
+    if (a.tail) tail_after = ticket_moment<true>(nrows);
+    RowWalk<true, true> rw;
+    rw.start(nrows, a.mwords, a.ticket, a.ticket_base);
+    long long row = rw.row;
+    int n = 0, i = 0;
+    if (rw.more) {
+        n = __builtin_amdgcn_readfirstlane((int)(row / a.nsub));
+        i = __builtin_amdgcn_readfirstlane((int)(row % a.nsub));
+        const size_t rc = (size_t)sub_of(a.act, i) * a.nchan_full + (a.coff + n * a.cstep);
+        stage_load_global<M, T, R1>(cur, reinterpret_cast<const Tin*>(a.data) + rc * (2 * M), tid);
+    }
+    cplx mv2[NSL];
+    const cplx* mheld = nullptr;
+    const cplx* mrow = nullptr;
+    int n_held = -1, ktn = 0;
+    int i_nx = i, n_nx = n;
+    first_row_landed();
+#pragma unroll 1
+    for (int phase = 0; phase < 2; ++phase) {
+    if (phase == 1) {
+        if (!a.tail) break;
+        tail_work_wave(a.tail, reinterpret_cast<double*>(lds), 2 * LDSN, tid, 1);
+        tail_after = 0x7fffffff;
+        put_lane_consts(as_global(a.twB)[32 * (tid & 15)]);
+    }
+    unsigned fast_left = 0u;
+    size_t rc_prev = 0;
+    unsigned lanepk = 0u;
+    {
+        const int lamp = fftq_lambda(tid);
+        lanepk = 16u * (unsigned)fftq_lane_of((64 - lamp) & 63) | (unsigned)(lamp ? lamp : 64) << 10;
+    }
+    for (; rw.more && tail_after != 0; rw.advance(), row = rw.row, i = i_nx, n = n_nx, --tail_after) {
+        asm volatile("" : "+v"(tid));
+        asm volatile("" : "+v"(lanepk));
+        __builtin_assume((unsigned)tid < 64u);
+        const bool l0 = (tid == 0);
+        const int kb = (int)(lanepk >> 10);
+        size_t rc;
+        const Tin* nxrow = nullptr;
+        if (fast_left != 0u) {
+            --fast_left;
+            rc = rc_prev + (size_t)(unsigned)a.nchan_full;
+            rw.row_nx = rw.row + 1u;
+            rw.bits &= rw.bits - 1u;
+            i_nx = i + 1;
+            nxrow = reinterpret_cast<const Tin*>(a.data) + (rc + (size_t)(unsigned)a.nchan_full) * (2 * M);
+        } else {
+            rw.draw(a.ticket);
+            rw.peek(nrows, a.ticket_base, a.mwords);
+            const int ia = sub_of(a.act, i), ne = a.coff + n * a.cstep;
+            rc = (size_t)ia * a.nchan_full + ne;
+            if (channel_lookup(a, ia, n, ne, M, n_held, mrow, ktn) && mrow != mheld) {
+#pragma unroll
+                for (int j = 0; j < NSL; ++j) mv2[j] = mrow[kb + 64 * j - 1];
+                mheld = mrow;
+            }
+            const bool first_of_chunk = rw.fresh != 0u;
+            rw.next(i, n, i_nx, n_nx, nrows, a.nsub, a.ticket_base, a.ticket, a.mwords);
+            nxrow = next_row_of<M, Tin>(a, rw.more_nx, i_nx, n_nx, rc);
+            const bool whole = first_of_chunk && rw.bits == 0xfffffffcu && i + (PP_ROW_CHUNK - 1) < a.nsub &&
+                               !a.mwords && !a.act && !a.slot;
+            fast_left = (unsigned)__builtin_amdgcn_readfirstlane(whole ? PP_ROW_CHUNK - 2 : 0);
+        }
+        rc_prev = rc;
+        const double phin = load_uniform(a.ph0 + rc);
+        double sd = 0.0;
+        cplx v[R1];
+#pragma unroll
+        for (int k = 0; k < R1; ++k) v[k] = to_cplx(cur[0][k]);
+        auto load_some = [&](int k0, int k1) { load_row_pieces<Raw, R1, true>(cur, nxrow, tid, k0, k1); };
+        auto prefetch = [&]() {
+            __builtin_amdgcn_sched_barrier(0);
+            load_some(0, R1 / 2);
+            __builtin_amdgcn_sched_barrier(0);
+        };
+        fftq1024_from<Q_PREFETCH_F64, true, true>(
+            v, lds, [&](const int j) { return tab1[64 * (j - 1) + tid]; }, [&]() { return ldt2[FFTQ_FREE_PITCH * (tid & 15)]; },
+            tid, &sd, prefetch);
+        __builtin_amdgcn_sched_barrier(0);
+        {
+            cplx* pub = lds + tid;
+#pragma unroll
+            for (int r = 0; r < NSL; ++r) pub[64 * r] = v[9 + r];
+            lds_sync<T>();
+        }
+        cplx wbq[2];
+        wbq[0] = tabw[tid];
+        __builtin_amdgcn_sched_barrier(0);
+        load_some(R1 / 2, R1);
+        __builtin_amdgcn_sched_barrier(0);
+        const cplx* pc = reinterpret_cast<const cplx*>(reinterpret_cast<const char*>(lds) + (lanepk & 0x3ffu));
+        const cplx el = unit_phasor<true, true>((double)kb, phin);
+        const cplx wst = make_double2(bcast_lane0(el.x), bcast_lane0(el.y));
+        cplx e = el;
+        const int ktu = __builtin_amdgcn_readfirstlane(ktn);
+        const double kap0 = PP_TWO_PI * (double)kb;
+        double tm[PP_TSTRIDE];
+        cplx zq[2];
+        zq[0] = pc[64 * 6];
+#pragma unroll
+        for (int j = 0; j < NSL; ++j) {
+            if (j > 0 && !(64 * j < ktu)) break;
+            const cplx zc = zq[j & 1];
+            const cplx wb = wbq[j & 1];
+            if (j + 1 < NSL && 64 * (j + 1) < ktu) {
+                zq[(j + 1) & 1] = pc[64 * (5 - j)];
+                wbq[(j + 1) & 1] = tabw[64 * (j + 1) + tid];
+            }
+            if (j == 0 || 64 * j < ktu) {
+                const cplx dd = split_pair(csel(l0, v[j + 1], v[j]), zc, wb);
+                const cplx x = cmulc(dd, mv2[j]);
+                const cplx z = cmul(x, e);
+                const double kap = j == 0 ? kap0 : kap0 + kconst<true>(PP_TWO_PI * (double)(64 * j));
+                taylor_terms(j == 0, tm, x, z, kap);
+            }
+            if (j + 1 < NSL && 64 * (j + 1) < ktu) e = cmul(e, wst);
+        }
+        double tr[NRED];
+#pragma unroll
+        for (int j = 0; j < PP_TSTRIDE; ++j) tr[j] = tm[j];
+        tr[PP_TSTRIDE] = sd;
+        lds_sync<T>();
+        double tv = wave_reduce_lds<NRED, true>(tr, tid, reinterpret_cast<double*>(lds));
+        store_row_results<M, false, true, true>(a, rc, tid, tv);
+        lds_sync<T>();
+    }
+    }
+    if (a.tail) tail_work_wave(a.tail, reinterpret_cast<double*>(lds), 2 * LDSN, tid, 1 << 30);
+}
+
+}
diff --git a/pulseportraiture_amd/csrc/pp_xspec1024q.h b/pulseportraiture_amd/csrc/pp_xspec1024q.h
--- a/pulseportraiture_amd/csrc/pp_xspec1024q.h
+++ b/pulseportraiture_amd/csrc/pp_xspec1024q.h
@@ -5,9 +5,10 @@
 namespace pp {
 
 constexpr unsigned PP_TICKET_WINDOW_NUM = 3u, PP_TICKET_WINDOW_DEN = 4u;
+template <bool CU = false>
 __device__ __forceinline__ int ticket_moment(const long long nrows) {
-    const unsigned share = (unsigned)(nrows / (long long)gridDim.x) + 1u;
-    return 1 + (int)(((blockIdx.x * 2654435761u) >> 8) % (share * PP_TICKET_WINDOW_NUM / PP_TICKET_WINDOW_DEN + 1u));
+    const unsigned share = (unsigned)(nrows / (long long)RowWalk<true, CU>::walkers()) + 1u;
+    return 1 + (int)(((RowWalk<true, CU>::me() * 2654435761u) >> 8) % (share * PP_TICKET_WINDOW_NUM / PP_TICKET_WINDOW_DEN + 1u));
 }
 
 template <int M, typename Tin>
diff --git a/pulseportraiture_amd/csrc/pp_xspec_cu.hip b/pulseportraiture_amd/csrc/pp_xspec_cu.hip
--- /dev/null
+++ b/pulseportraiture_amd/csrc/pp_xspec_cu.hip
@@ -0,0 +1,23 @@
+#include "../../include/pp_toas.h"
+
+#include <hip/hip_runtime.h>
+#include <stdint.h>
+#include <type_traits>
+
+#define pp pp_cu_unit
+#include "pp_tail.h"
+#include "pp_xspec1024cu.h"
+#undef pp
+
+extern "C" __attribute__((visibility("hidden"))) int pp_cu1024_prepare(void) {
+    return (int)hipFuncSetAttribute(reinterpret_cast<const void*>(&pp_cu_unit::k_xspec_cu1024<double>),
+                                    hipFuncAttributeMaxDynamicSharedMemorySize, pp_cu_unit::CU_LDS_BYTES);
+}
+
+extern "C" __attribute__((visibility("hidden"))) void pp_cu1024_launch(const void* xspec_args, long long nrows, int ncu, hipStream_t stream) {
+    const pp_cu_unit::XspecArgs& xa = *static_cast<const pp_cu_unit::XspecArgs*>(xspec_args);
+    const long long want = (nrows + pp_cu_unit::CU_WAVES - 1) / pp_cu_unit::CU_WAVES;
+    const dim3 grid((unsigned)(want < 1 ? 1 : want > ncu ? ncu : want));
+    hipLaunchKernelGGL(pp_cu_unit::k_xspec_cu1024<double>, grid, dim3(64 * pp_cu_unit::CU_WAVES), pp_cu_unit::CU_LDS_BYTES,
+                       stream, xa);
+}
```

New measurement: 78840, median of 6. 1.02x the previous value.
